# LitLeo/3m-asr-inference

Hardware: AMD Instinct MI355X
Metric: encoder frames/sec, 18Lx32e Conformer-MoE, 206-frame utterance (higher is better)
Workload: dtype f32; 1 GPU; 18-layer 32-expert fp32 (v_mfma_f32_16x16x4_f32), batch=1x206 frames per GPU, all experts local (BASELINE.json configs[1]); layers=18, experts=32, frames=206, batch_per_gpu=1, parallelism=replicas x1, streams_per_gpu=4, hip_graph=True, kernels_per_forward=262, fold_pos_proj=True, routing=balanced, route_mode=staged, packed_rows=False, fork_embed=auto

## Files before the change

### 3m-asr-inference_amd/csrc/conv.hip

```cpp
#include "common.h"
#include "kernels.h"

namespace m3 {

struct DwCausal {
  int causal = 0;
  const float* left = nullptr;
  long left_b_stride = 0; int left_t_stride = 0;
  const int32_t* step = nullptr;
  long half = 0;
  const int32_t* chunk_len = nullptr;
  int max_chunks = 0;
};

template <int KT, bool CAUSAL, bool SLOTS = false, bool GLU_IN = false>
__device__ __forceinline__ void dwconv_ln_silu_body(const float* __restrict__ z, const float* __restrict__ w_kc,
                                                    const float* __restrict__ bias, const float* __restrict__ gamma,
                                                    const float* __restrict__ beta, float eps, int T, int D, int K,
                                                    float* __restrict__ out, int out_bf16, const int32_t* __restrict__ pad_of,
                                                    const int32_t* __restrict__ row0, const int32_t* __restrict__ row_len,
                                                    int n_rows, const DwCausal& cs, const int row, const int ldz = 0) {
  static_assert(!GLU_IN || (!CAUSAL && !SLOTS), "GLU on load: the symmetric conv only");
  __shared__ float red[2][16];
  asm volatile("" ::"s"(z), "s"(w_kc), "s"(bias), "s"(gamma), "s"(beta), "s"(eps), "s"(T), "s"(D), "s"(K), "s"(out), "s"(out_bf16),
               "s"(pad_of), "s"(row0), "s"(row_len), "s"(n_rows));
  const int c = threadIdx.x * 4;
  const bool live = c < D;
  const size_t zs = GLU_IN ? (size_t)ldz : (size_t)D;
  const float* leftp = cs.left;
  if (CAUSAL && cs.step != nullptr) {
    int par;
    if (SLOTS) {
      const int sb = row >= n_rows ? (row - n_rows) / (K - 1) : row / T;
      const int pos = cs.step[sb];
      if (row >= n_rows && !stream_slot_live(cs.chunk_len[sb], pos, cs.max_chunks)) return;
      par = pos & 1;
    } else {
      par = *cs.step & 1;
    }
    leftp = cs.left + (size_t)par * cs.half;
    if (row >= n_rows) {
      const int i = row - n_rows, b = i / (K - 1), ci = i - b * (K - 1);
      const int s = ci + min(max(cs.chunk_len[b], 0), T);
      const float* src = s < K - 1 ? leftp + (size_t)b * cs.left_b_stride + (size_t)s * cs.left_t_stride
                                   : z + ((size_t)b * T + (s - (K - 1))) * D;
      float* dst = const_cast<float*>(cs.left) + (size_t)(par ^ 1) * cs.half + (size_t)b * cs.left_b_stride + (size_t)ci * cs.left_t_stride;
      if (live) stg4(dst + c, ldg4(src + c));
      return;
    }
  }
  int b = row / T, t = row % T, len = T;
  size_t r0 = (size_t)b * T, rpad = 0;
  if (pad_of != nullptr) {
    const int pr = pad_of[row];
    if (pr < 0) return;
    b = pr / T;
    t = pr - b * T;
    len = row_len[b];
    r0 = (size_t)row0[b];
    rpad = (size_t)row0[n_rows / T];
  }
  const int pad = CAUSAL ? K - 1 : (K - 1) / 2;
  if (CAUSAL) leftp += (size_t)b * cs.left_b_stride + (size_t)(K - 1) * cs.left_t_stride;
  const int lane = threadIdx.x & 63, wave = threadIdx.x >> 6, nwaves = (blockDim.x + 63) >> 6;
  f32x4 v = f32x4{0.f, 0.f, 0.f, 0.f};
  if (live) {
    v = ldg4(bias + c);
    for (int k0 = 0; k0 < K; k0 += KT) {
      f32x4 zz[KT], ww[KT], gg[GLU_IN ? KT : 1];
      float on[KT];
#pragma unroll
      for (int kk = 0; kk < KT; ++kk) {
        const int k = min(k0 + kk, K - 1);
        const int tt = t + k - pad;
        const int tc = min(max(tt, 0), T - 1);
        const float* src = z + (tc < len ? r0 + tc : rpad) * zs;
        if (CAUSAL) {
          on[kk] = (k0 + kk < K) ? 1.f : 0.f;
          if (tt < 0) src = leftp + (long)tt * cs.left_t_stride;
        } else {
          on[kk] = (k0 + kk < K && tt >= 0 && tt < T) ? 1.f : 0.f;
        }
        zz[kk] = ldg4(src + c);
        if (GLU_IN) gg[kk] = ldg4(src + D + c);
        ww[kk] = ldg4(w_kc + (size_t)k * D + c);
      }
      if (GLU_IN) {
        __builtin_amdgcn_sched_barrier(0);
#pragma unroll
        for (int kk = 0; kk < KT; ++kk)
#pragma unroll
          for (int j = 0; j < 4; ++j) zz[kk][j] = zz[kk][j] * sigmoidf(gg[kk][j]);
      }
#pragma unroll
      for (int kk = 0; kk < KT; ++kk)
#pragma unroll
        for (int j = 0; j < 4; ++j) v[j] = fmaf(zz[kk][j] * on[kk], ww[kk][j], v[j]);
    }
  }
  if (gamma != nullptr) {
    float s = live ? (v[0] + v[1]) + (v[2] + v[3]) : 0.f;
    s = wave_sum(s);
    if (lane == 0) red[0][wave] = s;
    __syncthreads();
    float tot = 0.f;
    for (int w = 0; w < nwaves; ++w) tot += red[0][w];
    const float mean = tot / (float)D;
    float q = 0.f;
    if (live) {
#pragma unroll
      for (int j = 0; j < 4; ++j) {
        const float d = v[j] - mean;
        q += d * d;
      }
    }
    q = wave_sum(q);
    if (lane == 0) red[1][wave] = q;
    __syncthreads();
    float qt = 0.f;
    for (int w = 0; w < nwaves; ++w) qt += red[1][w];
    const float rstd = rsqrtf(qt / (float)D + eps);
    if (live) {
      const f32x4 g = ldg4(gamma + c), be = ldg4(beta + c);
#pragma unroll
      for (int j = 0; j < 4; ++j) v[j] = (v[j] - mean) * rstd * g[j] + be[j];
    }
  }
  if (live) {
#pragma unroll
    for (int j = 0; j < 4; ++j) v[j] = silu(v[j]);
    if (out_bf16) {
      bf16x4 h;
#pragma unroll
      for (int j = 0; j < 4; ++j) h[j] = (bf16_t)v[j];
      *reinterpret_cast<bf16x4*>(reinterpret_cast<bf16_t*>(out) + (size_t)row * D + c) = h;
    } else {
      stg4(out + (size_t)row * D + c, v);
    }
  }
}

template <int KT, bool CAUSAL, bool SLOTS = false, bool GLU_IN = false>
__global__ __launch_bounds__(GLU_IN ? 256 : 1024) void dwconv_ln_silu_kernel(const float* __restrict__ z, const float* __restrict__ w_kc,
                                                              const float* __restrict__ bias,
                                                              const float* __restrict__ gamma,
                                                              const float* __restrict__ beta, float eps, int T,
                                                              int D, int K, float* __restrict__ out, int out_bf16,
                                                              const int32_t* __restrict__ pad_of,
                                                              const int32_t* __restrict__ row0,
                                                              const int32_t* __restrict__ row_len, int n_rows, DwCausal cs, int ldz) {
  dwconv_ln_silu_body<KT, CAUSAL, SLOTS, GLU_IN>(z, w_kc, bias, gamma, beta, eps, T, D, K, out, out_bf16, pad_of, row0, row_len, n_rows, cs,
                                                 (int)blockIdx.x, ldz);
}
struct DwKernArgs {
  const float *z, *w_kc, *bias, *gamma, *beta; float eps; int T, D, K; float* out; int out_bf16;
  const int32_t *pad_of, *row0, *row_len; int n_rows; DwCausal cs; int ldz;
};
template <int KT, bool CAUSAL, bool GLU_IN = false>
__global__ __launch_bounds__(GLU_IN ? 256 : 1024) void dwconv_ln_silu_dual_kernel(const DwKernArgs a, const DwKernArgs b) {
  if ((int)blockIdx.x < a.n_rows)
    dwconv_ln_silu_body<KT, CAUSAL, false, GLU_IN>(a.z, a.w_kc, a.bias, a.gamma, a.beta, a.eps, a.T, a.D, a.K, a.out, a.out_bf16, a.pad_of, a.row0,
                                                   a.row_len, a.n_rows, a.cs, (int)blockIdx.x, a.ldz);
  else
    dwconv_ln_silu_body<KT, CAUSAL, false, GLU_IN>(b.z, b.w_kc, b.bias, b.gamma, b.beta, b.eps, b.T, b.D, b.K, b.out, b.out_bf16, b.pad_of, b.row0,
                                                   b.row_len, b.n_rows, b.cs, (int)blockIdx.x - a.n_rows, b.ldz);
}

static int launch_dwconv_impl(const float* z, const float* w_kc, const float* bias, const float* gamma, const float* beta, float eps,
                              int B, int T, int D, int K, float* out, hipStream_t stream, int out_bf16, const int32_t* pad_of,
                              const int32_t* row0, const int32_t* row_len, const DwCausal& cs, bool slots = false, int glu_ldz = 0) {
  M3_REQUIRE(glu_ldz == 0 || dwconv_glu_in_supports(D, K, cs.causal != 0 || slots, out_bf16, glu_ldz),
             "dwconv (GLU on load): needs the symmetric fp32 conv, K <= 15, 256 <= channels <= 1024, ldz=%d a multiple of 4 and >= %d", glu_ldz, 2 * D);
  M3_REQUIRE(!slots || (cs.causal && cs.step != nullptr && cs.max_chunks > 0), "dwconv (slot mode): needs the streaming causal form");
  M3_REQUIRE((D & 3) == 0 && D <= 4096, "dwconv: channels=%d must be a multiple of 4 (<=4096)", D);
  M3_REQUIRE(cs.causal || (K & 1) == 1, "dwconv: kernel size %d must be odd (non-causal)", K);
  M3_REQUIRE(!cs.causal || (cs.left != nullptr && K >= 2), "dwconv (causal): the frames left of frame 0 must be supplied (left_fill / cache)");
  const int rows = B * T;
  if (rows == 0) return 0;
  const int threads = (int)align_up(D / 4, 64);
  const int grid = rows + (cs.step != nullptr ? B * (K - 1) : 0);
#define M3_DW_CASE(KT_, C_)                                                                                                  \
  hipLaunchKernelGGL((dwconv_ln_silu_kernel<KT_, C_>), dim3(grid), dim3(threads), 0, stream, z, w_kc, bias, gamma, beta, eps, T, \
                     D, K, out, out_bf16, pad_of, row0, row_len, rows, cs, 0)
#define M3_DW_SLOTS(KT_)                                                                                                        \
  hipLaunchKernelGGL((dwconv_ln_silu_kernel<KT_, true, true>), dim3(grid), dim3(threads), 0, stream, z, w_kc, bias, gamma, beta, eps, \
                     T, D, K, out, out_bf16, pad_of, row0, row_len, rows, cs, 0)
  if (glu_ldz)
    hipLaunchKernelGGL((dwconv_ln_silu_kernel<15, false, false, true>), dim3(grid), dim3(threads), 0, stream, z, w_kc, bias, gamma, beta, eps, T,
                       D, K, out, out_bf16, pad_of, row0, row_len, rows, cs, glu_ldz);
  else if (slots) { if (K <= 15) M3_DW_SLOTS(15); else M3_DW_SLOTS(8); }
  else if (K <= 15) { if (cs.causal) M3_DW_CASE(15, true); else M3_DW_CASE(15, false); }
  else { if (cs.causal) M3_DW_CASE(8, true); else M3_DW_CASE(8, false); }
#undef M3_DW_SLOTS
#undef M3_DW_CASE
  M3_LAUNCH_CHECK();
  return 0;
}

int launch_dwconv_ln_silu(const float* z, const float* w_kc, const float* bias, const float* gamma,
                          const float* beta, float eps, int B, int T, int D, int K, float* out, hipStream_t stream, int out_bf16,
                          const int32_t* pad_of, const int32_t* row0, const int32_t* row_len, const float* causal_left_fill) {
  DwCausal cs;
  if (causal_left_fill != nullptr) { cs.causal = 1; cs.left = causal_left_fill; }
  return launch_dwconv_impl(z, w_kc, bias, gamma, beta, eps, B, T, D, K, out, stream, out_bf16, pad_of, row0, row_len, cs);
}

bool dwconv_glu_in_supports(int D, int K, bool causal_or_stream, int out_bf16, int ldz) {
  return !causal_or_stream && !out_bf16 && (K & 1) == 1 && K <= 15 && D >= 256 && D <= 1024 && (D & 3) == 0 && ldz >= 2 * D && (ldz & 3) == 0;
}

int launch_dwconv_ln_silu_args(const DwArgs& a, hipStream_t stream) {
  if (a.glu_ldz) {
    M3_REQUIRE(a.causal_left_fill == nullptr, "dwconv (GLU on load): the symmetric conv only");
    return launch_dwconv_impl(a.z, a.w_kc, a.bias, a.gamma, a.beta, a.eps, a.B, a.T, a.D, a.K, a.out, stream, a.out_bf16, a.pad_of, a.row0, a.row_len,
                              DwCausal{}, false, a.glu_ldz);
  }
  return launch_dwconv_ln_silu(a.z, a.w_kc, a.bias, a.gamma, a.beta, a.eps, a.B, a.T, a.D, a.K, a.out, stream, a.out_bf16, a.pad_of, a.row0,
                               a.row_len, a.causal_left_fill);
}
bool dwconv_dual_fusable(const DwArgs& a, const DwArgs& b) {
  if ((a.glu_ldz != 0) != (b.glu_ldz != 0)) return false;
  if (a.glu_ldz && !(dwconv_glu_in_supports(a.D, a.K, a.causal_left_fill != nullptr, a.out_bf16, a.glu_ldz) &&
                     dwconv_glu_in_supports(b.D, b.K, b.causal_left_fill != nullptr, b.out_bf16, b.glu_ldz)))
    return false;
  return a.D == b.D && a.K == b.K && (a.causal_left_fill != nullptr) == (b.causal_left_fill != nullptr) && a.B * a.T > 0 && b.B * b.T > 0 &&
         (a.D & 3) == 0 && a.D <= 4096 && (a.causal_left_fill != nullptr || (a.K & 1) == 1);
}
int launch_dwconv_ln_silu_dual(const DwArgs& a, const DwArgs& b, hipStream_t stream) {
  M3_REQUIRE(dwconv_dual_fusable(a, b), "dwconv dual: the two problems do not share an instantiation");
  auto pack = [](const DwArgs& q) {
    DwKernArgs k;
    k.z = q.z; k.w_kc = q.w_kc; k.bias = q.bias; k.gamma = q.gamma; k.beta = q.beta; k.eps = q.eps; k.T = q.T; k.D = q.D; k.K = q.K;
    k.out = q.out; k.out_bf16 = q.out_bf16; k.pad_of = q.pad_of; k.row0 = q.row0; k.row_len = q.row_len; k.n_rows = q.B * q.T;
    if (q.causal_left_fill != nullptr) { k.cs.causal = 1; k.cs.left = q.causal_left_fill; }
    k.ldz = q.glu_ldz;
    return k;
  };
  const DwKernArgs ka = pack(a), kb = pack(b);
  const int threads = (int)align_up(a.D / 4, 64), grid = ka.n_rows + kb.n_rows;
  const bool causal = a.causal_left_fill != nullptr;
#define M3_DWD_CASE(KT_, C_) hipLaunchKernelGGL((dwconv_ln_silu_dual_kernel<KT_, C_>), dim3(grid), dim3(threads), 0, stream, ka, kb)
  if (a.glu_ldz) hipLaunchKernelGGL((dwconv_ln_silu_dual_kernel<15, false, true>), dim3(grid), dim3(threads), 0, stream, ka, kb);
  else if (a.K <= 15) { if (causal) M3_DWD_CASE(15, true); else M3_DWD_CASE(15, false); }
  else { if (causal) M3_DWD_CASE(8, true); else M3_DWD_CASE(8, false); }
#undef M3_DWD_CASE
  M3_LAUNCH_CHECK();
  return 0;
}

int launch_dwconv_ln_silu_stream(const float* z, const float* w_kc, const float* bias, const float* gamma, const float* beta,
                                 float eps, int B, int T, int D, int K, float* out, float* cache_pair, const int32_t* step,
                                 const int32_t* chunk_len, hipStream_t stream, int out_bf16, int slot_max_chunks) {
  M3_REQUIRE(cache_pair && step && chunk_len, "dwconv (stream): null state");
  DwCausal cs;
  cs.causal = 1; cs.left = cache_pair; cs.left_b_stride = (long)(K - 1) * D; cs.left_t_stride = D;
  cs.step = step; cs.half = (long)B * (K - 1) * D; cs.chunk_len = chunk_len;
  cs.max_chunks = slot_max_chunks > 0 ? slot_max_chunks : 0;
  return launch_dwconv_impl(z, w_kc, bias, gamma, beta, eps, B, T, D, K, out, stream, out_bf16, nullptr, nullptr, nullptr, cs,
                            slot_max_chunks >= 0);
}

__device__ __forceinline__ void conv1_relu_body(const float* __restrict__ feat, const float* __restrict__ w9c,
                                                const float* __restrict__ bias, const float* __restrict__ cmvn_mean,
                                                const float* __restrict__ cmvn_istd, int T, int idim, int T1, int F1, int C,
                                                float* __restrict__ out, int relu, int out_bf16, const int32_t* __restrict__ feat_len,
                                                int32_t* __restrict__ lens_out, int B, const int row) {
  extern __shared__ float xs[];
  if (feat_len != nullptr && row == 0 && blockIdx.y == 0)
    for (int i = threadIdx.x; i < B; i += blockDim.x) lens_out[i] = ((feat_len[i] - 3) / 2 + 1 - 3) / 2 + 1;
  const int b = row / T1, t1 = row - b * T1;
  const float* src = feat + ((size_t)b * T + 2 * t1) * idim;
  for (int i = threadIdx.x; i < 3 * idim; i += blockDim.x) {
    float xv = src[i];
    if (cmvn_mean != nullptr) {
      const int f = i % idim;
      xv = (xv - cmvn_mean[f]) * cmvn_istd[f];
    }
    xs[i] = xv;
  }
  const int c = threadIdx.x * 4;
  const bool live = c < C;
  f32x4 w[9], bv = f32x4{0.f, 0.f, 0.f, 0.f};
  if (live) {
    bv = ldg4(bias + c);
#pragma unroll
    for (int k = 0; k < 9; ++k) w[k] = ldg4(w9c + (size_t)k * C + c);
  }
  __syncthreads();
  if (!live) return;
  const size_t obase = (size_t)row * F1 * C + c;
  const int fchunk = (F1 + gridDim.y - 1) / gridDim.y;
  const int f_lo = blockIdx.y * fchunk, f_hi = min(F1, f_lo + fchunk);
  for (int f1 = f_lo; f1 < f_hi; ++f1) {
    f32x4 acc = bv;
#pragma unroll
    for (int kh = 0; kh < 3; ++kh)
#pragma unroll
      for (int kw = 0; kw < 3; ++kw) {
        const float xv = xs[kh * idim + 2 * f1 + kw];
#pragma unroll
        for (int j = 0; j < 4; ++j) acc[j] = fmaf(xv, w[kh * 3 + kw][j], acc[j]);
      }
#pragma unroll
    for (int j = 0; j < 4; ++j) acc[j] = relu ? fmaxf(acc[j], 0.f) : acc[j];
    if (out_bf16) {
      bf16x4 h;
#pragma unroll
      for (int j = 0; j < 4; ++j) h[j] = (bf16_t)acc[j];
      *reinterpret_cast<bf16x4*>(reinterpret_cast<bf16_t*>(out) + obase + (size_t)f1 * C) = h;
    } else {
      stg4(out + obase + (size_t)f1 * C, acc);
    }
  }
}

__global__ __launch_bounds__(256) void conv1_relu_kernel(const float* __restrict__ feat, const float* __restrict__ w9c,
                                                         const float* __restrict__ bias,
                                                         const float* __restrict__ cmvn_mean,
                                                         const float* __restrict__ cmvn_istd, int T, int idim, int T1,
                                                         int F1, int C, float* __restrict__ out, int relu, int out_bf16,
                                                         const int32_t* __restrict__ feat_len, int32_t* __restrict__ lens_out, int B) {
  conv1_relu_body(feat, w9c, bias, cmvn_mean, cmvn_istd, T, idim, T1, F1, C, out, relu, out_bf16, feat_len, lens_out, B, (int)blockIdx.x);
}
struct Conv1KernArgs {
  const float *feat, *w9c, *bias, *cmvn_mean, *cmvn_istd; int C; float* out; int relu, out_bf16; const int32_t* feat_len; int32_t* lens_out;
};
__global__ __launch_bounds__(256) void conv1_relu_dual_kernel(const Conv1KernArgs a, const Conv1KernArgs b, int T, int idim, int T1, int F1,
                                                              int B, int rows, int n0) {
  const int id = (int)blockIdx.x;
  if (id < n0) {
    if (id < rows)
      conv1_relu_body(a.feat, a.w9c, a.bias, a.cmvn_mean, a.cmvn_istd, T, idim, T1, F1, a.C, a.out, a.relu, a.out_bf16, a.feat_len, a.lens_out, B, id);
  } else {
    conv1_relu_body(b.feat, b.w9c, b.bias, b.cmvn_mean, b.cmvn_istd, T, idim, T1, F1, b.C, b.out, b.relu, b.out_bf16, b.feat_len, b.lens_out, B, id - n0);
  }
}

static int conv1_fsplit(int rows) { return rows >= 2048 ? 1 : (rows >= 512 ? 2 : 5); }

int launch_conv1_relu(const float* feat, const float* w9c, const float* bias, const float* cmvn_mean,
                      const float* cmvn_istd, int B, int T, int idim, int C, float* out, hipStream_t stream, int relu, int out_bf16,
                      const int32_t* feat_len, int32_t* lens_out) {
  M3_REQUIRE(T >= 3 && idim >= 3, "subsampling: input (T=%d, idim=%d) shorter than the 3x3 kernel", T, idim);
  M3_REQUIRE((C & 3) == 0 && C <= 1024, "subsampling: channels=%d must be a multiple of 4 (<= 1024)", C);
  const int T1 = (T - 3) / 2 + 1, F1 = (idim - 3) / 2 + 1;
  if (B * T1 == 0) return 0;
  const int threads = (int)align_up(C / 4, 64);
  const int fsplit = conv1_fsplit(B * T1);
  hipLaunchKernelGGL(conv1_relu_kernel, dim3(B * T1, fsplit), dim3(threads), 3 * idim * sizeof(float), stream,
                     feat, w9c, bias, cmvn_mean, cmvn_istd, T, idim, T1, F1, C, out, relu, out_bf16, feat_len, lens_out, B);
  M3_LAUNCH_CHECK();
  return 0;
}

int launch_conv1_relu_args(const Conv1Args& a, hipStream_t stream) {
  return launch_conv1_relu(a.feat, a.w9c, a.bias, a.cmvn_mean, a.cmvn_istd, a.B, a.T, a.idim, a.C, a.out, stream, a.relu, a.out_bf16, a.feat_len,
                           a.lens_out);
}
bool conv1_dual_fusable(const Conv1Args& a, const Conv1Args& b) {
  auto ok = [](const Conv1Args& q) { return q.T >= 3 && q.idim >= 3 && (q.C & 3) == 0 && q.C > 0 && q.C <= 1024; };
  return ok(a) && ok(b) && a.B == b.B && a.T == b.T && a.idim == b.idim && a.B * ((a.T - 3) / 2 + 1) > 0 && a.out != b.out;
}
int launch_conv1_relu_dual(const Conv1Args& a, const Conv1Args& b, hipStream_t stream) {
  M3_REQUIRE(conv1_dual_fusable(a, b), "subsampling conv1 dual: the two problems do not share an input shape");
  const int T1 = (a.T - 3) / 2 + 1, F1 = (a.idim - 3) / 2 + 1, rows = a.B * T1;
  auto pack = [](const Conv1Args& q) {
    return Conv1KernArgs{q.feat, q.w9c, q.bias, q.cmvn_mean, q.cmvn_istd, q.C, q.out, q.relu, q.out_bf16, q.feat_len, q.lens_out};
  };
  const int threads = (int)align_up((a.C > b.C ? a.C : b.C) / 4, 64);
  const int n0 = (int)align_up((size_t)rows, 8);
  hipLaunchKernelGGL(conv1_relu_dual_kernel, dim3(n0 + rows, conv1_fsplit(rows)), dim3(threads), 3 * a.idim * sizeof(float), stream, pack(a), pack(b),
                     a.T, a.idim, T1, F1, a.B, rows, n0);
  M3_LAUNCH_CHECK();
  return 0;
}

__global__ void depthwise_conv1d_nct_kernel(const float* __restrict__ x, const float* __restrict__ w,
                                            const float* __restrict__ bias, int C, int T, int To, int K, int pad,
                                            float* __restrict__ y, size_t n) {
  for (size_t i = (size_t)blockIdx.x * blockDim.x + threadIdx.x; i < n; i += (size_t)gridDim.x * blockDim.x) {
    const int t = (int)(i % To);
    const size_t bc = i / To;
    const int c = (int)(bc % C);
    const float* xr = x + bc * T;
    float acc = bias ? bias[c] : 0.f;
    for (int k = 0; k < K; ++k) {
      const int tt = t + k - pad;
      if (tt >= 0 && tt < T) acc = fmaf(xr[tt], w[(size_t)c * K + k], acc);
    }
    y[i] = acc;
  }
}

int launch_depthwise_conv1d_nct(const float* x, const float* w, const float* bias, int B, int C, int T, int K,
                                int pad, float* y, hipStream_t stream) {
// ... 31 lines not shown
```

### 3m-asr-inference_amd/csrc/engine.hip

```cpp
#include <assert.h>
#include <math.h>
#include <stdlib.h>
#include <string.h>

#include <functional>
#include <memory>
#include <string>
#include <unordered_map>
#include <vector>

#include "../../include/m3asr.h"
#include "common.h"
#include "kernels.h"

namespace m3 {
struct MoeWorkspace {
  int32_t* mapping; int32_t* acc; int32_t* pos; float* slab; size_t bytes;
};
MoeWorkspace carve_moe_workspace(void* base, int S, int E, int D, int F);
}

using namespace m3;

namespace {

struct Norm { const float* g = nullptr; const float* b = nullptr; };
struct Lin { const float* w = nullptr; const float* b = nullptr; const float* wsum = nullptr; const float* wbeta = nullptr; };

struct BlockW {
  Norm n_ffm, n_mha, n_conv, n_ff, n_final, n_cnn;
  Lin mac1, mac2, qkv, pos, out, pw1, pw2, ff1, ff2;
  const float* pos_u = nullptr; const float* pos_v = nullptr;
  const float* dw_w = nullptr; const float* dw_b = nullptr;
  const float* left_fill = nullptr;
  Lin router;
  Lin router_x;
  const float *ew1 = nullptr, *eb1 = nullptr, *ew2 = nullptr, *eb2 = nullptr;
  const float *es1 = nullptr, *es2 = nullptr;
  float h_scale = 0.f;
};

struct SubW { const float* c1w; const float* c1b; const float* c2w; const float* c2b; Lin out; };

enum class FuseKind { None, Gemm, Dwconv, Attention, Conv1, SplitK };

struct Stage {
  std::string name;
  std::function<int(hipStream_t)> run;
  m3_stage_info info;
  bool reads_embed = false;
  FuseKind fuse_kind = FuseKind::None;
  GemmParams gemm; GemmPlan gemm_plan; float* gemm_ws = nullptr;
  Conv1Args c1;
  DwArgs dw;
  AttArgs att;
};

m3_stage_info stage_info(const char* kernel, int launches, double bytes, double flops, bool per_row = true) {
  m3_stage_info i;
  i.kernel = kernel; i.launches = launches; i.per_row = per_row ? 1 : 0; i.alg_bytes = bytes; i.flops = flops;
  return i;
}

struct Buf { void* ptr; size_t bytes; };

struct BindKey {
  int B = 0, T = 0;
  const float* feat = nullptr; const int32_t* feat_len = nullptr; float* logits = nullptr;
  void* ws = nullptr; size_t ws_bytes = 0;
  int ep_cap = 0;
  void* sstate = nullptr; int s_hist = 0, s_maxf = 0;
  bool s_slots = false;
  bool operator==(const BindKey& o) const {
    return B == o.B && T == o.T && feat == o.feat && feat_len == o.feat_len && logits == o.logits && ws == o.ws &&
           ws_bytes == o.ws_bytes && ep_cap == o.ep_cap && sstate == o.sstate && s_hist == o.s_hist && s_maxf == o.s_maxf &&
           s_slots == o.s_slots;
  }
};

}

struct m3_engine {
  m3_engine_config cfg;
  std::unordered_map<std::string, m3_weight_entry> table;
  std::vector<std::string> names;
  SubW sub_e, sub_m;
  std::vector<BlockW> eblocks, mblocks;
  Norm e_after, m_after;
  Lin out_linear;
  const float* pe = nullptr;
  int64_t pe_rows = 0;
  const float* pos_all = nullptr;
  const float* cmvn_mean = nullptr; const float* cmvn_istd = nullptr;
  const float* output_bias = nullptr;
  const float* router_e_all = nullptr;

  struct Bound {
    BindKey key;
    int Tp = 0, S = 0;
    bool a16 = false;
    bool dma = false;
    bool packed = false;
    bool xn_skipped = false;
    int fork_first = -1, fork_mid = -1, join_at = -1;
    std::shared_ptr<float> pfold;
    std::vector<Stage> stages;
    std::unordered_map<std::string, Buf> buffers;
    int n_kernels = 0;
    hipGraphExec_t graph_exec = nullptr;
    bool graph_valid = false;
    uint64_t last_use = 0;
    bool matches(const BindKey& k) const { return !stages.empty() && key == k; }
  };
  Bound cur;
  std::vector<Bound> parked;
  uint64_t use_clock = 0;
  int n_captures = 0;
  int ep_capacity = 0;
  hipStream_t side = nullptr;
  hipEvent_t ev_fork = nullptr, ev_join = nullptr;
  std::unordered_map<int, std::weak_ptr<float>> pfold_by_tp;
};

namespace {

struct Switches {
  int gate_index_max_rows;
  bool self_route;
  bool hfuse;
  int router_min_rows;
  bool router_xq;
  bool router_skip_xn;
  bool fused8_adapt;
  bool glu_defer;
  bool front_pair;
};
const Switches& switches() {
  static const Switches sw = [] {
    auto num = [](const char* name, int dflt) { const char* v = getenv(name); return v ? atoi(v) : dflt; };
    Switches w;
    w.gate_index_max_rows = num("M3_GATE_INDEX_MAX_ROWS", 512);
    w.self_route = num("M3_SELF_ROUTE", 1) != 0;
    w.hfuse = num("M3_HFUSE", 1) != 0;
    w.router_min_rows = num("M3_ROUTER_MIN_ROWS", 2048);
    w.router_xq = num("M3_ROUTER_XQ", 1) != 0;
    w.router_skip_xn = num("M3_ROUTER_SKIP_XN", 0) != 0;
    w.fused8_adapt = num("M3_FUSED8_ADAPT", 0) != 0;
    w.glu_defer = num("M3_GLU_DEFER", 1) != 0;
    w.front_pair = num("M3_FRONT_PAIR", 1) != 0;
    return w;
  }();
  return sw;
}

bool lookup(const m3_engine* e, const std::string& name, int64_t numel, const float** out, int dtype = M3_F32) {
  auto it = e->table.find(name);
  if (it == e->table.end()) {
    set_error("engine: weight '%s' missing from the plan", name.c_str());
    return false;
  }
  if (numel >= 0 && it->second.numel != numel) {
    set_error("engine: weight '%s' has %lld elements, expected %lld", name.c_str(), (long long)it->second.numel,
              (long long)numel);
    return false;
  }
  if (it->second.dtype != dtype) {
    set_error("engine: weight '%s' has dtype %d, the engine (weight_dtype=%d) expects %d", name.c_str(),
              (int)it->second.dtype, (int)e->cfg.weight_dtype, dtype);
    return false;
  }
  *out = (const float*)it->second.data;
  return true;
}

#define GET(dst, name, numel) \
  do { if (!lookup(e, (name), (numel), &(dst))) return false; } while (0)
#define GETW(dst, name, numel) \
  do { if (!lookup(e, (name), (numel), &(dst), e->cfg.weight_dtype == M3_F32 ? M3_F32 : M3_BF16)) return false; } while (0)
#define GETE(dst, name, numel) \
  do { if (!lookup(e, (name), (numel), &(dst), e->cfg.weight_dtype)) return false; } while (0)

bool load_norm(const m3_engine* e, const std::string& p, int d, Norm* n) {
  GET(n->g, p + "weight", d);
  GET(n->b, p + "bias", d);
  return true;
}
bool load_lin(const m3_engine* e, const std::string& p, int64_t n_out, int64_t n_in, bool bias, Lin* l) {
  GETW(l->w, p + "weight", n_out * n_in);
  if (bias) GET(l->b, p + "bias", n_out);
  return true;
}
bool load_lin_ln(const m3_engine* e, const std::string& p, int64_t n_out, int64_t n_in, bool wbeta, Lin* l,
                 bool fp32_only = false) {
  if (fp32_only) {
    GET(l->w, p + "ln.weight", n_out * n_in);
  } else {
    GETW(l->w, p + "ln.weight", n_out * n_in);
  }
  GET(l->b, p + "ln.bias", n_out);
  GET(l->wsum, p + "ln.wsum", n_out);
  if (wbeta) GET(l->wbeta, p + "ln.wbeta", n_out);
  return true;
}

bool load_block(const m3_engine* e, const std::string& p, int D, int F, int K, bool cnn_ln, bool moe, int De, BlockW* b, bool causal) {
  const m3_engine_config& c = e->cfg;
  if (!load_norm(e, p + "norm_final.", D, &b->n_final)) return false;
  if (moe && !load_norm(e, p + "norm_ff.", D, &b->n_ff)) return false;
  if (!load_lin_ln(e, p + "feed_forward_macaron.w_1.", F, D, false, &b->mac1) ||
      !load_lin(e, p + "feed_forward_macaron.w_2.", D, F, true, &b->mac2) ||
      !load_lin_ln(e, p + "self_attn.qkv.", 3 * D, D, false, &b->qkv) ||
      !load_lin(e, p + "self_attn.linear_out.", D, D, true, &b->out) ||
      !load_lin_ln(e, p + "conv_module.pointwise_conv1.", 2 * D, D, true, &b->pw1) ||
      !load_lin(e, p + "conv_module.pointwise_conv2.", D, D, true, &b->pw2))
    return false;
  GET(b->pos_u, p + "self_attn.pos_bias_u", D);
  GET(b->pos_v, p + "self_attn.pos_bias_v", D);
  GET(b->dw_w, p + "conv_module.depthwise_conv.weight_kc", (int64_t)K * D);
  GET(b->dw_b, p + "conv_module.depthwise_conv.bias", D);
  if (cnn_ln && !load_norm(e, p + "conv_module.norm.", D, &b->n_cnn)) return false;
  if (causal) GET(b->left_fill, p + "conv_module.left_fill", D);
  if (!moe) {
    if (!load_lin_ln(e, p + "feed_forward.w_1.", F, D, false, &b->ff1) ||
        !load_lin(e, p + "feed_forward.w_2.", D, F, true, &b->ff2))
      return false;
  } else {
    const int world = c.ep_world_size > 0 ? c.ep_world_size : 1;
    const int64_t Etot = (int64_t)c.num_experts * world;
    GET(b->router.w, p + "feed_forward.router_weights_t", Etot * (D + De));
    if (c.router_with_bias) GET(b->router.b, p + "feed_forward.router_bias", Etot);
    if (c.fuse_route && !load_lin_ln(e, p + "feed_forward.router_x.", Etot, D, false, &b->router_x, true)) return false;
    const int64_t E = c.num_experts;
    GETE(b->ew1, p + "feed_forward.experts.w_1.weight", E * F * D);
    if (c.weight_dtype == M3_FP8) {
      GET(b->es1, p + "feed_forward.experts.w_1.scale", E * F);
      GET(b->es2, p + "feed_forward.experts.w_2.scale", E * D);
      if (c.fp8_activations) {
        const float* hs = nullptr;
        GET(hs, p + "feed_forward.experts.h_scale", 1);
        if (hipMemcpy(&b->h_scale, hs, sizeof(float), hipMemcpyDeviceToHost) != hipSuccess || !(b->h_scale > 0.f)) {
          set_error("engine: '%sfeed_forward.experts.h_scale' must hold one positive number", p.c_str());
          return false;
        }
      }
    }
    GET(b->eb1, p + "feed_forward.experts.w_1.bias", E * F);
    GETE(b->ew2, p + "feed_forward.experts.w_2.weight_sliced", E * D * F);
    GET(b->eb2, p + "feed_forward.experts.w_2.bias", E * D);
  }
  return true;
}

bool load_sub(const m3_engine* e, const std::string& p, int D, int idim, SubW* s) {
  const int F2 = ((idim - 1) / 2 - 1) / 2;
  GET(s->c1w, p + "conv.0.weight_9c", 9 * (int64_t)D);
  GET(s->c1b, p + "conv.0.bias", D);
  GETW(s->c2w, p + "conv.2.weight_ohwi", 9 * (int64_t)D * D);
  GET(s->c2b, p + "conv.2.bias", D);
  return load_lin(e, p + "out.0.", D, (int64_t)D * F2, true, &s->out);
}
#undef GET
#undef GETW
#undef GETE

inline int sub_len(int t) { return ((t - 3) / 2 + 1 - 3) / 2 + 1; }

struct Carver {
  char* base; size_t off = 0;
  explicit Carver(void* b) : base((char*)b) {}
  template <typename T> T* take(size_t n) {
    T* p = (T*)(base ? base + off : nullptr);
    off += align_up(n * sizeof(T), 256);
    return p;
  }
};

struct Plan {
  int32_t* lens;
  float *c1, *c2, *x, *emb, *h1, *qkv, *pbuf, *ctx, *glu, *dw, *xn, *rl, *eall;
  void* xb;
  int32_t* moe_fs;
  unsigned char* xq; float* xq_scale;
  float* xstats;
  int32_t* gate_idx; float* gate_val;
  void* moe_ws; size_t moe_ws_bytes;
  float* splitk; size_t splitk_bytes;
  float* taps;
  float* pfold;
  int32_t *row0, *pad_of; float* xpad; void* xbpad; float* lpk;
  int32_t *ep_acc, *ep_mapping, *ep_pos, *ep_map_send, *ep_gate_recv, *ep_overflow; float *wire_a, *wire_b; int ep_cap, ep_rows;
  bool fork;
  bool hfuse;
  float *e_c1, *e_c2, *e_x, *e_h1, *e_qkv, *e_ctx, *e_glu, *e_dw, *e_xpad, *e_splitk, *e_xstats; void *e_xb, *e_xbpad;
  size_t bytes;
};

bool use_fork_embed(const m3_engine_config& c, int B, int S) { return c.fork_embed > 0 && !c.debug_taps; }
bool use_packed_rows(const m3_engine_config& c, int B) {
  if (c.packed_rows < 0 || (c.packed_rows == 0 && B <= 1)) return false;
  return !c.debug_taps && c.fuse_route == 0 && B <= 1024;
}

bool use_hfuse(const m3_engine_config& c, int B, int S) {
  return switches().hfuse && !c.debug_taps && c.weight_dtype == M3_F32 && c.embed_blocks > 0 && c.num_blocks > 0 && S <= 128 && c.fork_embed <= 0 &&
         !use_packed_rows(c, B);
}

Plan make_plan(const m3_engine_config& c, void* base, int B, int T, int ep_capacity = 0) {
  Plan p;
  Carver cv(base);
  const int Tp = sub_len(T), S = B * Tp;
  const int T1 = (T - 3) / 2 + 1, F1 = (c.input_dim - 3) / 2 + 1, F2 = (F1 - 3) / 2 + 1;
  const int D = c.attention_dim > c.embed_dim ? c.attention_dim : c.embed_dim;
  const int F = c.hidden_units > c.embed_linear_units ? c.hidden_units : c.embed_linear_units;
  const int world = c.ep_world_size > 0 ? c.ep_world_size : 1;
  const int Etot = c.num_experts * world;
  p.lens = cv.take<int32_t>(B);
  p.c1 = cv.take<float>((size_t)B * T1 * F1 * D);
  p.c2 = cv.take<float>((size_t)S * F2 * D);
  p.x = cv.take<float>((size_t)S * D);
  p.emb = cv.take<float>((size_t)S * D);
  p.xb = cv.take<uint16_t>((size_t)S * D);
  p.xstats = cv.take<float>((size_t)S * 2 * kXbStatParts);
  p.h1 = cv.take<float>((size_t)S * F);
  p.qkv = cv.take<float>((size_t)S * 3 * D);
  p.pbuf = cv.take<float>((size_t)Tp * D * (c.num_blocks + c.embed_blocks));
  p.ctx = cv.take<float>((size_t)S * D);
  const size_t glu_floats = (size_t)S * D * (switches().glu_defer && c.weight_dtype == M3_F32 && D >= 256 ? 2 : 1);
  p.glu = cv.take<float>(glu_floats);
  p.dw = cv.take<float>((size_t)S * D);
  p.xn = cv.take<float>((size_t)S * D);
  p.xq = nullptr; p.xq_scale = nullptr; p.moe_fs = nullptr;
  if (c.weight_dtype == M3_FP8) p.moe_fs = cv.take<int32_t>(64);
  if (c.weight_dtype == M3_FP8 && D == 512) {
    p.xq = cv.take<unsigned char>((size_t)S * D);
    p.xq_scale = cv.take<float>((size_t)S);
  }
  p.rl = cv.take<float>((size_t)S * Etot);
  p.eall = cv.take<float>((size_t)S * Etot * c.num_blocks);
  p.gate_idx = cv.take<int32_t>((size_t)c.num_blocks * S);
  p.gate_val = cv.take<float>((size_t)c.num_blocks * S);
  const bool ep = world > 1 || c.ep_stages > 0;
  p.ep_cap = ep ? (ep_capacity > 0 ? ep_capacity : S) : 0;
  p.ep_rows = ep ? world * (p.ep_cap + 1) : 0;
  p.moe_ws_bytes = carve_moe_workspace(nullptr, ep ? p.ep_rows : S, c.num_experts, c.attention_dim, c.hidden_units).bytes;
  p.moe_ws = cv.take<char>(p.moe_ws_bytes * (size_t)(c.debug_taps ? c.num_blocks : 1));
  p.ep_acc = p.ep_mapping = p.ep_pos = p.ep_map_send = p.ep_gate_recv = p.ep_overflow = nullptr; p.wire_a = p.wire_b = nullptr;
  if (ep) {
    p.ep_overflow = cv.take<int32_t>(64);
    p.ep_acc = cv.take<int32_t>((size_t)Etot + 1);
    p.ep_mapping = cv.take<int32_t>(S);
    p.ep_pos = cv.take<int32_t>(S);
    p.ep_map_send = cv.take<int32_t>(S);
    p.ep_gate_recv = cv.take<int32_t>(p.ep_rows);
    p.wire_a = cv.take<float>((size_t)p.ep_rows * c.attention_dim);
    p.wire_b = cv.take<float>((size_t)p.ep_rows * c.attention_dim);
  }
  {
    size_t n1 = 0, n2 = 0;
    if (c.weight_dtype == M3_F32) {
      GemmParams g;
      g.mode = GEMM_A_CONV3X3S2; g.lda = 4; g.conv_C = D; g.M = S * F2; g.N = D; g.K = 9 * D; g.ldy = D;
      n1 = plan_gemm(g, SIZE_MAX).ws_bytes;
      GemmParams l;
      l.lda = F2 * D; l.M = S; l.N = D; l.K = F2 * D; l.ldy = D;
      n2 = plan_gemm(l, SIZE_MAX).ws_bytes;
    }
    p.splitk_bytes = n1 > n2 ? n1 : n2;
    p.splitk = p.splitk_bytes ? cv.take<float>(p.splitk_bytes / sizeof(float)) : nullptr;
  }
  p.taps = c.debug_taps ? cv.take<float>((size_t)(c.num_blocks + c.embed_blocks) * S * D) : nullptr;
  p.pfold = nullptr;
  p.row0 = p.pad_of = nullptr; p.xpad = p.lpk = nullptr; p.xbpad = nullptr;
  if (use_packed_rows(c, B)) {
    p.row0 = cv.take<int32_t>(B + 1);
    p.pad_of = cv.take<int32_t>(S);
    p.xpad = cv.take<float>((size_t)S * D);
    p.xbpad = cv.take<uint16_t>((size_t)S * D);
    p.lpk = cv.take<float>((size_t)S * c.output_dim);
  }
  p.fork = use_fork_embed(c, B, S);
  p.hfuse = !p.fork && use_hfuse(c, B, S);
  p.e_c1 = p.c1; p.e_c2 = p.c2; p.e_x = p.x; p.e_h1 = p.h1; p.e_qkv = p.qkv; p.e_ctx = p.ctx; p.e_glu = p.glu; p.e_dw = p.dw;
  p.e_xb = p.xb; p.e_xpad = p.xpad; p.e_xbpad = p.xbpad; p.e_splitk = p.splitk; p.e_xstats = p.xstats;
  if (p.fork || p.hfuse) {
    p.e_c1 = cv.take<float>((size_t)B * T1 * F1 * D);
    p.e_c2 = cv.take<float>((size_t)S * F2 * D);
    p.e_x = cv.take<float>((size_t)S * D);
    p.e_xb = cv.take<uint16_t>((size_t)S * D);
    p.e_xstats = cv.take<float>((size_t)S * 2 * kXbStatParts);
    p.e_h1 = cv.take<float>((size_t)S * F);
    p.e_qkv = cv.take<float>((size_t)S * 3 * D);
    p.e_ctx = cv.take<float>((size_t)S * D);
    p.e_glu = cv.take<float>(glu_floats);
    p.e_dw = cv.take<float>((size_t)S * D);
    if (p.splitk_bytes) p.e_splitk = cv.take<float>(p.splitk_bytes / sizeof(float));
    if (use_packed_rows(c, B)) {
      p.e_xpad = cv.take<float>((size_t)S * D);
      p.e_xbpad = cv.take<uint16_t>((size_t)S * D);
    }
  }
  p.bytes = cv.off;
  return p;
}

struct StreamState {
  int32_t* step = nullptr;
  std::vector<float*> kv, conv;
  int32_t *slot_pos = nullptr, *slot_status = nullptr, *slot_frames = nullptr;
  size_t bytes = 0;
};
StreamState carve_stream_state(const m3_engine_config& c, void* base, int B, int hist) {
  Carver cv(base);
  StreamState st;
  st.step = cv.take<int32_t>(64);
  const int nb = c.embed_blocks + c.num_blocks, D = c.attention_dim, K = c.cnn_module_kernel;
  for (int i = 0; i < nb; ++i) st.kv.push_back(cv.take<float>((size_t)B * hist * 2 * D));
  for (int i = 0; i < nb; ++i) st.conv.push_back(cv.take<float>((size_t)2 * B * (K - 1) * D));
  st.slot_pos = cv.take<int32_t>((size_t)3 * B);
  st.slot_status = st.slot_pos ? st.slot_pos + B : nullptr;
  st.slot_frames = st.slot_pos ? st.slot_pos + 2 * B : nullptr;
  st.bytes = cv.off;
  return st;
}

Plan embed_view(const Plan& pl) {
  Plan q = pl;
  q.c1 = pl.e_c1; q.c2 = pl.e_c2; q.x = pl.e_x; q.h1 = pl.e_h1; q.qkv = pl.e_qkv; q.ctx = pl.e_ctx; q.glu = pl.e_glu; q.dw = pl.e_dw;
  q.xb = pl.e_xb; q.xpad = pl.e_xpad; q.xbpad = pl.e_xbpad; q.splitk = pl.e_splitk; q.xstats = pl.e_xstats;
  return q;
}

enum class RouterForm {
  Gemm,
  Kernel,
  Fused,
  Split,
};
enum class GateForm {
  RouterTail,
  GateIndex,
  Top1Index,
  InExpert,
  InRoute,
};
struct MoeRoute {
  RouterForm router = RouterForm::Gemm;
  GateForm gate = GateForm::Top1Index;
  bool ep = false;
  bool router_top1 = false;
  bool use_xq = false;
  bool skip_xn = false;
  bool fs_dev = false;
  bool needs_e_all = false;
  bool norm_in_expert() const { return router == RouterForm::Fused || router == RouterForm::Split; }
};

static ExpertWeights expert_weights(const m3_engine_config& c, const BlockW& w) {
  if (c.weight_dtype == M3_F32) return ExpertWeights::F32;
  if (c.weight_dtype == M3_BF16) return ExpertWeights::BF16;
  return w.h_scale > 0.f ? ExpertWeights::FP8A8 : ExpertWeights::FP8;
}

MoeRoute choose_moe_route(const m3_engine_config& c, int S, const BlockW& w, const Plan& pl) {
  const Switches& sw = switches();
  const int world = c.ep_world_size > 0 ? c.ep_world_size : 1;
  const int E = c.num_experts, Etot = E * world, D = c.attention_dim, De = c.embed_dim, F = c.hidden_units;
  const bool one_wg_experts = Etot == 8 || Etot == 16 || Etot == 32 || Etot == 64;
  const bool self_routing = sw.self_route && c.weight_dtype == M3_F32 && expert_ffn_f32_self_routing(S, Etot) &&
                            plan_expert_ffn(ExpertWeights::F32, S, E, D, F).kernel == ExpertKernel::SlabF32;
  MoeRoute r;
  r.ep = world > 1 || c.ep_stages > 0;
  if (c.fuse_route == 2 && world == 1 && S < 1024 && one_wg_experts) {
    r.router = RouterForm::Split;
    r.gate = self_routing ? GateForm::InExpert : GateForm::GateIndex;
  } else if (c.fuse_route == 1 && world == 1 && S <= 256 && (E == 16 || E == 32 || E == 64)) {
    r.router = RouterForm::Fused;
    r.gate = GateForm::InRoute;
  } else {
    r.router = moe_router_supports(De, D, Etot) && S >= sw.router_min_rows ? RouterForm::Kernel : RouterForm::Gemm;
    r.router_top1 = r.router == RouterForm::Kernel && moe_router_fuses_top1(Etot) && S > sw.gate_index_max_rows;
    if (self_routing && c.fuse_route == 0 && !r.ep) r.gate = GateForm::InExpert;
    else if (S <= sw.gate_index_max_rows && one_wg_experts) r.gate = GateForm::GateIndex;
    else r.gate = r.router_top1 ? GateForm::RouterTail : GateForm::Top1Index;
  }
  const bool fused8 = !r.ep && plan_expert_ffn(expert_weights(c, w), S, E, D, F).kernel == ExpertKernel::FusedFp8;
  r.use_xq = r.router == RouterForm::Kernel && sw.router_xq && fused8 && pl.xq != nullptr;
  r.skip_xn = r.use_xq && sw.router_skip_xn && !c.debug_taps;
  r.fs_dev = sw.fused8_adapt && fused8 && pl.moe_fs != nullptr && !c.debug_taps;
  r.needs_e_all = r.norm_in_expert();
  return r;
}

struct StageBuilder {
  const m3_engine& eng;
  Plan pl;
  m3_engine::Bound& bd;
  StreamState st;
  bool lens_in_conv1 = false;
  const float *tail_ln_g = nullptr, *tail_ln_b = nullptr; float tail_ln_eps = 0.f; float* tail_ln_out = nullptr;
  float* splitk_ws = nullptr; size_t splitk_bytes = 0;
};

}

static void add_stage(StageBuilder& sb, const std::string& name, int kernels, std::function<int(hipStream_t)> fn,
                      m3_stage_info info = stage_info("", 0, 0.0, 0.0)) {
  info.launches = kernels;
  sb.bd.stages.push_back(Stage{name, std::move(fn), info});
  sb.bd.n_kernels += kernels;
}

static m3_stage_info gemm_info(const GemmParams& p, const GemmPlan& plan) {
  const bool glu = p.act == ACT_GLU;
  const double M = p.M, N = p.N, K = p.K, Nout = glu ? N / 2 : N;
  const double wsz = p.w_bf16 ? 2 : 4, asz = p.a_bf16 ? 2 : 4, ysz = p.y_bf16 ? 2 : 4;
  double a_bytes = M * K * asz;
  if (p.mode == GEMM_A_CONV3X3S2)
    a_bytes = (double)(p.M / (p.conv_T2 * p.conv_F2)) * p.conv_T1 * p.conv_F1 * p.conv_C * asz;
  double bytes = N * K * wsz + a_bytes + M * Nout * ysz;
  if (p.resid) bytes += M * Nout * 4;
  if (p.Yb) bytes += M * Nout * 2;
  if (p.ln_out) bytes += M * (K - p.K1) * 4;
  return stage_info(plan.label, 1, bytes, 2.0 * M * N * K, p.mode != GEMM_A_CONV3X3S2);
}

static void add_gemm(StageBuilder& sb, const std::string& name, GemmParams p, bool fp32_weights = false) {
  p.w_bf16 = (!fp32_weights && sb.eng.cfg.weight_dtype != M3_F32) ? 1 : 0;
  float* ws = sb.splitk_ws;
  const GemmPlan plan = plan_gemm(p, ws != nullptr ? sb.splitk_bytes : 0);
  add_stage(sb, name, plan.launches ? plan.launches : 1, [plan, p, ws](hipStream_t s) { return launch_gemm(plan, p, ws, s); }, gemm_info(p, plan));
  if (plan.launches == 1) {
    sb.bd.stages.back().fuse_kind = FuseKind::Gemm;
    sb.bd.stages.back().gemm = p;
    sb.bd.stages.back().gemm_plan = plan;
  } else if (plan.kernel == GemmKernel::SplitKF32 && plan.launches == 2) {
    sb.bd.stages.back().gemm = p;
    sb.bd.stages.back().gemm_plan = plan;
    sb.bd.stages.back().gemm_ws = ws;
  }
}

static bool stages_fusable(const Stage& a, const Stage& b) {
  if (a.fuse_kind == FuseKind::None || a.fuse_kind != b.fuse_kind) return false;
  if (a.fuse_kind == FuseKind::Gemm) return gemm_dual_fusable(a.gemm_plan, b.gemm_plan);
  if (a.fuse_kind == FuseKind::Dwconv) return dwconv_dual_fusable(a.dw, b.dw);
  if (a.fuse_kind == FuseKind::Attention) return relpos_attention_dual_fusable(a.att, b.att);
  if (a.fuse_kind == FuseKind::Conv1) return conv1_dual_fusable(a.c1, b.c1);
  if (a.fuse_kind == FuseKind::SplitK) return gemm_splitk_dual_fusable(a.gemm_plan, b.gemm_plan) && a.gemm_ws != b.gemm_ws;
  return false;
}
static Stage fused_stage(const Stage& a, const Stage& b, bool reduce_half = false) {
  Stage d;
  d.name = reduce_half ? a.name + ".reduce+" + b.name + ".reduce" : a.name + "+" + b.name;
  const char* label = "";
  if (a.fuse_kind == FuseKind::Conv1) {
    const Conv1Args pa = a.c1, pb = b.c1;
    d.run = [pa, pb](hipStream_t s) { return launch_conv1_relu_dual(pa, pb, s); };
    label = "conv1_relu_dual_kernel";
  } else if (a.fuse_kind == FuseKind::SplitK) {
    const GemmParams pa = a.gemm, pb = b.gemm;
    const GemmPlan qa = a.gemm_plan, qb = b.gemm_plan;
    float* const wa = a.gemm_ws; float* const wb = b.gemm_ws;
    const int which = reduce_half ? 2 : 1;
    d.run = [qa, pa, wa, qb, pb, wb, which](hipStream_t s) { return launch_gemm_f32_splitk_dual(qa, pa, wa, qb, pb, wb, s, which); };
    label = "gemm_f32_splitk_dual_kernel";
  } else if (a.fuse_kind == FuseKind::Gemm) {
    const GemmParams pa = a.gemm, pb = b.gemm;
    const GemmPlan qa = a.gemm_plan, qb = b.gemm_plan;
    d.run = [qa, pa, qb, pb](hipStream_t s) { return launch_gemm_f32_dual(qa, pa, qb, pb, s); };
    label = "gemm_f32_dual_kernel";
  } else if (a.fuse_kind == FuseKind::Dwconv) {
    const DwArgs pa = a.dw, pb = b.dw;
    d.run = [pa, pb](hipStream_t s) { return launch_dwconv_ln_silu_dual(pa, pb, s); };
    label = "dwconv_ln_silu_dual_kernel";
  } else {
    const AttArgs pa = a.att, pb = b.att;
    d.run = [pa, pb](hipStream_t s) { return launch_relpos_attention_dual(pa, pb, s); };
    label = "relpos_attention_dual_kernel";
  }
  d.info = reduce_half ? stage_info(label, 1, 0.0, 0.0, a.info.per_row != 0)
                       : stage_info(label, 1, a.info.alg_bytes + b.info.alg_bytes, a.info.flops + b.info.flops, a.info.per_row != 0);
  return d;
}
static void fuse_independent_pairs(StageBuilder& sb, int first, int mid, int join) {
  if (first < 0 || mid <= first + 1 || join <= mid) return;
  std::vector<Stage>& st = sb.bd.stages;
  std::vector<Stage> out(st.begin(), st.begin() + first);
  std::vector<Stage> pending;
  int i = first, saved = 0;
  for (int m = mid; m < join; ++m) {
    assert(!st[m].reads_embed);
    int partner = -1;
    if (st[m].fuse_kind != FuseKind::None)
      for (int k = st[m].fuse_kind == FuseKind::Conv1 ? i : std::max(i, first + 1); k < mid; ++k)
        if (stages_fusable(st[k], st[m])) { partner = k; break; }
    if (partner < 0) { pending.push_back(st[m]); continue; }
    for (; i < partner; ++i) out.push_back(st[i]);
    for (Stage& q : pending) out.push_back(q);
    pending.clear();
    out.push_back(fused_stage(st[partner], st[m]));
    saved += st[partner].info.launches + st[m].info.launches - 1;
    if (st[m].fuse_kind == FuseKind::SplitK) {
      out.push_back(fused_stage(st[partner], st[m], true));
      saved -= 1;
    }
    i = partner + 1;
  }
  for (; i < mid; ++i) out.push_back(st[i]);
  for (Stage& q : pending) out.push_back(q);
  for (int k = join; k < (int)st.size(); ++k) out.push_back(st[k]);
  st.swap(out);
  sb.bd.n_kernels -= saved;
}

static int embed_join(const std::vector<Stage>& st, int from) {
  for (int i = from; i < (int)st.size(); ++i)
    if (st[i].reads_embed) return i;
  return -1;
}

static void build_subsample(StageBuilder& sb, const std::string& pfx, const SubW& w, int D, const Plan& pl, float* xout) {
  const m3_engine_config& c = sb.eng.cfg;
  const int B = sb.bd.key.B, T = sb.bd.key.T;
  const int T1 = (T - 3) / 2 + 1, F1 = (c.input_dim - 3) / 2 + 1, F2 = (F1 - 3) / 2 + 1, T2 = (T1 - 3) / 2 + 1;
  const float* feat = sb.bd.key.feat;
  float* c1 = pl.c1; float* c2 = pl.c2;
  const int idim = c.input_dim;
  const float* cm = sb.eng.cmvn_mean; const float* ci = sb.eng.cmvn_istd;
  const bool a16 = sb.bd.a16;
  const int32_t* flen = sb.lens_in_conv1 ? sb.bd.key.feat_len : nullptr;
  int32_t* lens_out = pl.lens;
  sb.lens_in_conv1 = false;
  Conv1Args ca;
  ca.feat = feat; ca.w9c = w.c1w; ca.bias = w.c1b; ca.cmvn_mean = cm; ca.cmvn_istd = ci; ca.B = B; ca.T = T; ca.idim = idim; ca.C = D; ca.out = c1;
  ca.relu = 1; ca.out_bf16 = a16; ca.feat_len = flen; ca.lens_out = lens_out;
  add_stage(sb, pfx + "conv1", 1, [ca](hipStream_t s) { return launch_conv1_relu_args(ca, s); },
            stage_info("conv1_relu_kernel", 1, (double)B * T * idim * 4 + (double)B * T1 * F1 * D * (a16 ? 2 : 4), 18.0 * B * T1 * F1 * D, false));
  const size_t conv1_at = sb.bd.stages.size() - 1;
  GemmParams g;
  g.a_bf16 = a16; g.y_bf16 = a16;
  g.mode = GEMM_A_CONV3X3S2; g.A = c1; g.lda = 4;
  g.conv_T1 = T1; g.conv_F1 = F1; g.conv_T2 = T2; g.conv_F2 = F2; g.conv_C = D;
  g.W = w.c2w; g.bias = w.c2b; g.Y = c2; g.ldy = D; g.M = B * T2 * F2; g.N = D; g.K = 9 * D; g.act = ACT_RELU;
  if (sb.bd.packed) g.conv_len = pl.lens;
  add_gemm(sb, pfx + "conv2", g);
  const bool pairable = switches().front_pair && !a16 && !sb.bd.packed && sb.bd.stages.back().gemm_plan.kernel == GemmKernel::SplitKF32 &&
                        sb.bd.stages.back().gemm_ws != nullptr;
  if (pairable) {
    sb.bd.stages[conv1_at].fuse_kind = FuseKind::Conv1;
    sb.bd.stages[conv1_at].c1 = ca;
    sb.bd.stages.back().fuse_kind = FuseKind::SplitK;
  }
  const bool packed = sb.bd.packed;
  GemmParams l;
  l.A = c2; l.lda = F2 * D; l.W = w.out.w; l.bias = w.out.b; l.Y = packed ? pl.xpad : xout; l.ldy = D;
  l.M = B * T2; l.N = D; l.K = F2 * D; l.alpha = sqrtf((float)D);
  l.a_bf16 = a16;
  if (a16) { l.Yb = packed ? pl.xbpad : pl.xb; l.ldyb = D; }
  add_gemm(sb, pfx + "linear", l);
  if (pairable && sb.bd.stages.back().gemm_ws != nullptr) sb.bd.stages.back().fuse_kind = FuseKind::SplitK;
  if (packed) {
    const float* xpad = pl.xpad; const void* xbpad = pl.xbpad; void* xb = pl.xb; const int32_t* pad_of = pl.pad_of;
    const int S = B * T2;
    add_stage(sb, pfx + "pack", a16 ? 2 : 1, [=](hipStream_t s) {
      if (int rc = launch_local_gather(xpad, pad_of, S, D * 4, xout, s)) return rc;
      return a16 ? launch_local_gather(xbpad, pad_of, S, D * 2, xb, s) : 0;
    }, stage_info("row_permute_kernel", 1, (double)S * D * (a16 ? 12 : 8) + 4.0 * S, 0.0));
  }
  if (sb.bd.dma) {
    const void* xbv = pl.xb; float* xs = pl.xstats;
    const int S = B * T2;
    add_stage(sb, pfx + "row_stats", 1, [=](hipStream_t s) { return launch_row_stats_bf16(xbv, S, D, xs, s); },
              stage_info("row_stats_bf16_kernel", 1, (double)S * D * 2 + 32.0 * S, 3.0 * S * D));
  }
}

struct MoeLayer {
  std::string pfx;
  const BlockW* w;
  int S, Tp, D, F, De, E, Etot, world;
  float eps;
  float *x, *xn, *rl;
  int32_t* gidx; float* gval;
  const float* gv;
  const int32_t *lens, *live_len; int live_rpb;
  const int32_t* pdev;
  const float* eall; int ld_eall;
  void* xb_out; float* xstats_out;
  void* ws; MoeWorkspace mw;
};

static void add_moe_router(StageBuilder& sb, const MoeLayer& m, const MoeRoute& r, const Plan& pl) {
  const BlockW& w = *m.w;
  const int S = m.S, D = m.D, De = m.De, E = m.E, Etot = m.Etot;
  if (r.router == RouterForm::Fused) {
    add_stage(sb, m.pfx + "moe_route", 1, [m](hipStream_t s) {
      const BlockW& w = *m.w;
      return launch_moe_route(m.x, m.D, m.D, w.router_x.w, w.router_x.wsum, w.router_x.b, m.eall, m.ld_eall, m.eps, m.lens, m.Tp,
                              m.S, m.E, m.gidx, m.gval, m.mw.mapping, m.mw.acc, m.mw.pos, s);
    }, stage_info("moe_route_kernel", 1, (double)E * D * 4 + (double)S * (D + E) * 4 + 16.0 * S, 2.0 * S * E * D));
  } else if (r.router == RouterForm::Kernel) {
    void* xq = r.use_xq ? pl.xq : nullptr; float* xqs = r.use_xq ? pl.xq_scale : nullptr;
    float* xn_out = r.skip_xn ? nullptr : m.xn;
    if (r.skip_xn) sb.bd.xn_skipped = true;
    int32_t* gidx = r.router_top1 ? m.gidx : nullptr; float* gval = r.router_top1 ? m.gval : nullptr;
    const float* emb = pl.emb;
    add_stage(sb, m.pfx + "moe_router", 1, [=](hipStream_t s) {
      const BlockW& w = *m.w;
      return launch_moe_router(emb, m.De, m.De, m.x, m.D, m.D, w.router.w, w.router.b, w.n_ff.g, w.n_ff.b, m.eps, xn_out, m.D, m.rl,
                               m.Etot, m.S, m.Etot, m.pdev, s, gidx, gval, m.live_len, m.live_rpb, xq, xqs);
    }, stage_info("moe_router_kernel", 1, (double)Etot * (De + D) * 4 + (double)S * (De + 2 * D + Etot) * 4, 2.0 * S * Etot * (De + D)));
  } else {
    GemmParams g;
    g.Y = m.rl; g.ldy = Etot; g.M = S; g.N = Etot; g.m_dev = m.pdev;
    if (r.router == RouterForm::Split) {
      g.A = m.x; g.lda = D; g.W = w.router_x.w; g.bias = w.router_x.b; g.ln_wsum = w.router_x.wsum; g.ln_eps = m.eps; g.K = D;
      g.resid = m.eall; g.ldr = m.ld_eall;
    } else {
      g.mode = GEMM_A_CONCAT2; g.A = pl.emb; g.lda = De; g.K1 = De; g.A2 = m.x; g.lda2 = D; g.K = De + D;
      g.W = w.router.w; g.bias = w.router.b;
      g.ln_gamma = w.n_ff.g; g.ln_beta = w.n_ff.b; g.ln_eps = m.eps; g.ln_on_a2 = 1; g.ln_out = m.xn; g.ld_ln_out = D;
    }
    add_gemm(sb, m.pfx + "moe_router", g, true);
  }
  sb.bd.stages.back().reads_embed = true;
}

static void add_moe_gate_index(StageBuilder& sb, const MoeLayer& m, int32_t* map, int32_t* acc, int32_t* pos) {
  add_stage(sb, m.pfx + "moe_gate_index", 1, [=](hipStream_t s) {
    return launch_moe_gate_index(m.rl, m.Etot, m.live_len, m.live_rpb, m.S, m.gidx, m.gval, map, acc, pos, s);
  }, stage_info("moe_index_kernel", 1, (double)m.S * (m.Etot * 4 + 16) + 4.0 * (m.Etot + 1), 0.0));
}

static void add_moe_top1(StageBuilder& sb, const MoeLayer& m) {
  add_stage(sb, m.pfx + "moe_top1", 1, [m](hipStream_t s) {
    return launch_softmax_top1(m.rl, m.Etot, m.live_len, m.live_rpb, m.S, m.Etot, m.gidx, m.gval, s);
  }, stage_info("softmax_top1_kernel", 1, (double)m.S * (m.Etot * 4 + 8), 0.0));
}

static void add_moe_local_index(StageBuilder& sb, const MoeLayer& m) {
  add_stage(sb, m.pfx + "moe_local.index", 1, [m](hipStream_t s) {
    return launch_moe_index(m.gidx, m.S, m.E, m.mw.mapping, m.mw.acc, m.mw.pos, s);
  }, stage_info("moe_index_kernel", 1, 12.0 * m.S + 4.0 * (m.E + 1), 0.0));
}

static ExpertFfnArgs expert_args(const BlockW& w, const float* x, const MoeWorkspace& mw, int D) {
  ExpertFfnArgs a{};
  a.x = x; a.ldx = D; a.pos = mw.pos; a.acc_hist = mw.acc; a.w1 = w.ew1; a.w2 = w.ew2; a.s1 = w.es1; a.s2 = w.es2; a.b1 = w.eb1;
  a.w2_sliced = 1; a.h_scale = w.h_scale; a.slab = mw.slab;
  return a;
}

static void add_moe_local_expert(StageBuilder& sb, const MoeLayer& m, const MoeRoute& r, const ExpertFfnPlan& f, const Plan& pl) {
  const bool norm = r.norm_in_expert();
  const float* xin = norm ? m.x : m.xn;
  const bool self_route = r.gate == GateForm::InExpert;
  const void* xq = r.use_xq ? pl.xq : nullptr; const float* xqs = r.use_xq ? pl.xq_scale : nullptr;
  int32_t* fs = r.fs_dev ? pl.moe_fs : nullptr;
  add_stage(sb, m.pfx + "moe_local.expert", f.launches, [=](hipStream_t s) {
    const BlockW& w = *m.w;
    const float* ln_g = norm ? w.n_ff.g : nullptr; const float* ln_b = norm ? w.n_ff.b : nullptr; const float ln_eps = norm ? m.eps : 0.f;
    if (self_route)
      return launch_expert_route_ffn_f32(xin, m.D, m.rl, m.live_len, m.live_rpb, m.S, m.E, m.D, m.F, w.ew1, w.eb1, w.ew2, 1, w.eb2,
                                         m.mw.slab, m.gidx, m.gval, m.mw.mapping, m.mw.acc, m.mw.pos, s, ln_g, ln_b, ln_eps);
    ExpertFfnArgs a = expert_args(w, xin, m.mw, m.D);
    a.ln_gamma = ln_g; a.ln_beta = ln_b; a.ln_eps = ln_eps; a.xq = xq; a.xq_scale = xqs; a.fs_dev = fs;
    return launch_expert_ffn(f, m.S, m.E, m.D, m.F, a, s);
  }, stage_info(f.label, 1, -1.0, 4.0 * m.D * m.F * m.S));
}

static void add_moe_local_combine(StageBuilder& sb, const MoeLayer& m, const MoeRoute& r, const ExpertFfnPlan& f, const Plan& pl) {
  const bool self_route = r.gate == GateForm::InExpert;
  const int32_t* cmap = self_route ? nullptr : m.mw.mapping;
  const float* cb2 = self_route ? nullptr : m.w->eb2;
  const int32_t* fs = r.fs_dev ? pl.moe_fs : nullptr;
  const double S = m.S, D = m.D;
  add_stage(sb, m.pfx + "moe_local.combine", 1, [=](hipStream_t s) {
    const BlockW& w = *m.w;
    return launch_moe_combine(f.rows(m.mw.slab), fs ? kExpertFusedFp8MaxSplit : f.slices, cmap, m.gidx, m.gv, cb2, m.x, 0.5f, w.n_final.g, w.n_final.b, m.eps, m.x,
                              m.S, m.D, s, m.xb_out, m.xstats_out, fs);
  }, stage_info("moe_combine_kernel", 1, S * D * 4 * (f.slices + 2) + (m.xb_out ? 2.0 * S * D : 0.0), S * D * (f.slices + 10)));
}

static void add_moe_ep(StageBuilder& sb, const MoeLayer& m, const MoeRoute& r, const Plan& pl) {
  const int S = m.S, E = m.E, Etot = m.Etot, D = m.D, F = m.F, world = m.world;
  const int cap = pl.ep_cap, R = pl.ep_rows;
  int32_t *g_acc = pl.ep_acc, *g_map = pl.ep_mapping, *g_pos = pl.ep_pos, *map_send = pl.ep_map_send, *gate_recv = pl.ep_gate_recv;
  int32_t* ep_overflow = pl.ep_overflow;
  float *wire_a = pl.wire_a, *wire_b = pl.wire_b;
  const MoeWorkspace rw = carve_moe_workspace(m.ws, R, E, D, F);
  if (r.gate == GateForm::GateIndex) add_moe_gate_index(sb, m, g_map, g_acc, g_pos);
  if (r.gate == GateForm::Top1Index) add_moe_top1(sb, m);
  const bool one_launch = r.gate == GateForm::GateIndex;
  const int32_t* gidx = m.gidx; const float* xn = m.xn;
  add_stage(sb, m.pfx + "moe_ep.send", one_launch ? 1 : 2, [=](hipStream_t s) {
    if (!one_launch)
      if (int rc = launch_moe_index(gidx, S, Etot, g_map, g_acc, g_pos, s)) return rc;
    return launch_ep_send_rows(gidx, g_map, g_acc, S, world, E, cap, map_send, xn, wire_a, D * 4, s, ep_overflow);
  }, stage_info("ep_send_rows_kernel", 1, (double)S * D * 8 + 24.0 * S, 0.0));
  auto exchange = [=, &sb](const char* name) {
    if (world == 1) add_stage(sb, m.pfx + name, 0, [=](hipStream_t s) {
      M3_CHECK_HIP(hipMemcpyAsync(wire_b, wire_a, (size_t)R * D * 4, hipMemcpyDeviceToDevice, s));
      return 0;
    });
  };
  exchange("moe_ep.exchange1");
  const ExpertFfnPlan f = plan_expert_ffn(expert_weights(sb.eng.cfg, *m.w), R, E, D, F, EXPERT_SCATTER_ROWS);
  const bool scatter2 = f.kernel == ExpertKernel::TiledBf16;
  const BlockW* wp = m.w;
  add_stage(sb, m.pfx + "moe_ep.expert", (scatter2 ? 2 : 3) + f.launches, [=](hipStream_t s) {
    const BlockW& w = *wp;
    if (int rc = launch_ep_recv_gate(wire_b, world, E, cap, D * 4, gate_recv, s)) return rc;
    if (int rc = launch_moe_index(gate_recv, R, E, rw.mapping, rw.acc, rw.pos, s)) return rc;
    ExpertFfnArgs a = expert_args(w, wire_b, rw, D);
    if (scatter2) { a.b2 = w.eb2; a.y_scatter = wire_a; }
    if (int rc = launch_expert_ffn(f, R, E, D, F, a, s)) return rc;
    if (scatter2) return 0;
    return launch_moe_combine(f.rows(rw.slab), f.slices, rw.mapping, gate_recv, nullptr, w.eb2, nullptr, 1.f, nullptr, nullptr, 0.f, wire_a, R, D, s);
  }, stage_info(f.label, 1, -1.0, 4.0 * D * F * S));
  exchange("moe_ep.exchange2");
  add_stage(sb, m.pfx + "moe_ep.combine", 1, [=](hipStream_t s) {
    const BlockW& w = *wp;
    return launch_moe_combine(wire_b, 1, map_send, nullptr, m.gv, nullptr, m.x, 0.5f, w.n_final.g, w.n_final.b, m.eps, m.x, S, D, s,
                              m.xb_out, m.xstats_out);
  }, stage_info("moe_combine_kernel", 1, (double)S * D * 12 + (m.xb_out ? 2.0 * S * D : 0.0), (double)S * D * 11));
  sb.bd.buffers["ep.wire_a"] = Buf{wire_a, (size_t)R * D * 4};
  sb.bd.buffers["ep.wire_b"] = Buf{wire_b, (size_t)R * D * 4};
}

static void build_block(StageBuilder& sb, const std::string& pfx, const BlockW& w, int D, int F, int H, int K, bool cnn_ln,
                        bool moe, int layer, int tap_index, const Plan& pl, bool causal) {
  auto add_gemm = [&](StageBuilder&, const std::string& name, GemmParams g, bool fp32_weights = false) {
    if (sb.bd.packed) g.m_dev = pl.row0 + sb.bd.key.B;
    ::add_gemm(sb, name, g, fp32_weights);
  };
  const m3_engine_config& c = sb.eng.cfg;
  const BindKey& key = sb.bd.key;
  const int B = key.B, Tp = sb.bd.Tp, S = sb.bd.S;
  const bool streaming = key.sstate != nullptr;
  const int32_t* step = key.s_slots ? sb.st.slot_pos : sb.st.step;
  const int slot_chunks = key.s_slots ? key.s_maxf / Tp : -1;
  float* x = pl.x;
  const int32_t* lens = pl.lens;
  const float eps = 1e-12f;

  const bool a16 = sb.bd.a16;
  void* xb = pl.xb;
  const bool dma = sb.bd.dma;
  float* xstats = pl.xstats;
  auto from_xb = [&](GemmParams& g) {
    if (a16) { g.A = (const float*)xb; g.a_bf16 = 1; }
    if (dma) { g.ln_stats = xstats; g.ln_stat_parts = kXbStatParts; }
  };
  auto also_xb = [&](GemmParams& g) {
    if (a16) { g.Yb = xb; g.ldyb = D; }
    if (dma) g.Yb_stats = xstats;
  };
  const bool packed = sb.bd.packed;
  const int32_t* row0 = packed ? pl.row0 : nullptr;
  const int32_t* pad_of = packed ? pl.pad_of : nullptr;
  const int32_t* pdev = packed ? pl.row0 + B : nullptr;
  const int32_t* live_len = packed ? pdev : lens;
  const int live_rpb = packed ? S : Tp;
  {
    GemmParams g;
    g.A = x; g.lda = D; g.W = w.mac1.w; g.bias = w.mac1.b; g.Y = pl.h1; g.ldy = F; g.M = S; g.N = F; g.K = D;
    g.ln_wsum = w.mac1.wsum; g.ln_eps = eps; g.act = ACT_SILU;
    from_xb(g); g.y_bf16 = a16;
    add_gemm(sb, pfx + "ffn_macaron.w1", g);
    GemmParams h;
    h.A = pl.h1; h.lda = F; h.W = w.mac2.w; h.bias = w.mac2.b; h.Y = x; h.ldy = D; h.M = S; h.N = D; h.K = F;
    h.alpha = 0.5f; h.resid = x; h.ldr = D;
    h.a_bf16 = a16; also_xb(h);
    add_gemm(sb, pfx + "ffn_macaron.w2", h);
  }
  {
    GemmParams g;
    g.A = x; g.lda = D; g.W = w.qkv.w; g.bias = w.qkv.b; g.Y = pl.qkv; g.ldy = 3 * D; g.M = S; g.N = 3 * D; g.K = D;
    g.ln_wsum = w.qkv.wsum; g.ln_eps = eps;
    from_xb(g);
    const bool att16 = a16 && relpos_attention_bf16_supports(Tp, D / H);
    g.y_bf16 = att16;
    add_gemm(sb, pfx + "att.qkv", g);
    const int ldp = (c.num_blocks + c.embed_blocks) * D;
    const float* pmat = pl.pbuf + (size_t)tap_index * D;
    const float* qkv = pl.qkv; float* ctx = pl.ctx;
    const float* pu = w.pos_u; const float* pv = w.pos_v;
    const int dk = D / H;
    const float scale = 1.f / sqrtf((float)dk);
    const int chunk = c.static_chunk_size, left_chunks = c.num_left_chunks;
    if (streaming) {
      float* hist = sb.st.kv[tap_index]; const int cap = key.s_hist;
      add_stage(sb, pfx + "att.core", 1, [=](hipStream_t s) {
        return launch_relpos_attention_stream(qkv, 3 * D, hist, cap, pmat, ldp, pu, pv, lens, step, B, Tp, H, dk, scale, ctx, D, left_chunks, s,
                                              slot_chunks);
      }, stage_info("relpos_attention_stream_kernel", 1, (double)S * D * 24 + (double)Tp * D * 4, 6.0 * Tp * D * S));
    } else
    {
    add_stage(sb, pfx + "att.core", 1, [=](hipStream_t s) {
      if (att16) return launch_relpos_attention_bf16(qkv, 3 * D, pmat, ldp, pu, pv, lens, B, Tp, H, dk, scale, ctx, D, s, row0, chunk, left_chunks);
      return launch_relpos_attention(qkv, 3 * D, pmat, ldp, pu, pv, lens, B, Tp, H, dk, scale, ctx, D, s, a16, row0, chunk, left_chunks);
    }, stage_info(att16 ? "relpos_attention_bf16_kernel" : "relpos_attention_kernel", 1,
                  (double)S * D * (att16 ? 8 : (12 + (a16 ? 2 : 4))) + (double)Tp * D * 4, 6.0 * Tp * D * S));
    if (!att16) {
      AttArgs aa;
      aa.qkv = qkv; aa.ldq = 3 * D; aa.pmat = pmat; aa.ldp = ldp; aa.pos_u = pu; aa.pos_v = pv; aa.row_len = lens; aa.B = B; aa.T = Tp; aa.H = H;
      aa.dk = dk; aa.scale = scale; aa.out = ctx; aa.ldo = D; aa.out_bf16 = a16; aa.row0 = row0; aa.chunk = chunk; aa.left_chunks = left_chunks;
      sb.bd.stages.back().fuse_kind = FuseKind::Attention;
      sb.bd.stages.back().att = aa;
    }
    }
    GemmParams o;
    o.A = pl.ctx; o.lda = D; o.W = w.out.w; o.bias = w.out.b; o.Y = x; o.ldy = D; o.M = S; o.N = D; o.K = D;
    o.resid = x; o.ldr = D;
    o.a_bf16 = a16; also_xb(o);
    add_gemm(sb, pfx + "att.out", o);
  }
  {
    GemmParams g;
    g.A = x; g.lda = D; g.W = w.pw1.w; g.bias = w.pw1.b; g.Y = pl.glu; g.ldy = D; g.M = S; g.N = 2 * D; g.K = D;
    g.ln_wsum = w.pw1.wsum; g.ln_wbeta = w.pw1.wbeta; g.ln_eps = eps; g.act = ACT_GLU;
    g.row_len = live_len; g.rows_per_batch = live_rpb; g.mask_in = 1;
    from_xb(g);
    bool glu_deferred = false;
    if (switches().glu_defer && c.weight_dtype == M3_F32 && !a16 && !causal && !streaming &&
        dwconv_glu_in_supports(D, K, false, 0, 2 * D)) {
      GemmParams r = g;
      r.act = ACT_NONE; r.ldy = 2 * D;
      const GemmPlan rp = plan_gemm(r, 0);
      if (rp.launches == 1 && rp.kernel == GemmKernel::SkinnyF32 && rp.mt == 1) { g = r; glu_deferred = true; }
    }
    add_gemm(sb, pfx + "conv.pw1_glu", g);
    const float* glu = pl.glu; float* dw = pl.dw;
    const float* dww = w.dw_w; const float* dwb = w.dw_b;
    const float* ng = cnn_ln ? w.n_cnn.g : nullptr; const float* nb = cnn_ln ? w.n_cnn.b : nullptr;
    const float* lfill = causal ? w.left_fill : nullptr;
    if (streaming) {
      float* cpair = sb.st.conv[tap_index];
      add_stage(sb, pfx + "conv.dw_ln_silu", 1, [=](hipStream_t s) {
        return launch_dwconv_ln_silu_stream(glu, dww, dwb, ng, nb, 1e-5f, B, Tp, D, K, dw, cpair, step, lens, s, a16, slot_chunks);
      }, stage_info("dwconv_ln_silu_kernel", 1, (double)S * D * 8 + (double)K * D * 4 + 8.0 * B * (K - 1) * D, 2.0 * K * D * S));
    } else
    {
      DwArgs da;
      da.z = glu; da.w_kc = dww; da.bias = dwb; da.gamma = ng; da.beta = nb; da.eps = 1e-5f; da.B = B; da.T = Tp; da.D = D; da.K = K;
      da.out = dw; da.out_bf16 = a16; da.pad_of = pad_of; da.row0 = row0; da.row_len = lens; da.causal_left_fill = lfill;
      da.glu_ldz = glu_deferred ? 2 * D : 0;
      add_stage(sb, pfx + "conv.dw_ln_silu", 1, [da](hipStream_t s) { return launch_dwconv_ln_silu_args(da, s); },
                stage_info("dwconv_ln_silu_kernel", 1, (double)S * D * ((glu_deferred ? 8 : 4) + (a16 ? 2 : 4)) + (double)K * D * 4, 2.0 * K * D * S));
      sb.bd.stages.back().fuse_kind = FuseKind::Dwconv;
      sb.bd.stages.back().dw = da;
    }
    GemmParams h;
    h.A = pl.dw; h.lda = D; h.W = w.pw2.w; h.bias = w.pw2.b; h.Y = x; h.ldy = D; h.M = S; h.N = D; h.K = D;
    h.row_len = live_len; h.rows_per_batch = live_rpb; h.mask_out = 1; h.resid = x; h.ldr = D;
    h.a_bf16 = a16; also_xb(h);
    add_gemm(sb, pfx + "conv.pw2", h);
  }
  if (!moe) {
    GemmParams g;
    g.A = x; g.lda = D; g.W = w.ff1.w; g.bias = w.ff1.b; g.Y = pl.h1; g.ldy = F; g.M = S; g.N = F; g.K = D;
    g.ln_wsum = w.ff1.wsum; g.ln_eps = eps; g.act = ACT_SILU;
    from_xb(g); g.y_bf16 = a16;
    add_gemm(sb, pfx + "ffn.w1", g);
    GemmParams h;
    h.A = pl.h1; h.lda = F; h.W = w.ff2.w; h.bias = w.ff2.b; h.Y = x; h.ldy = D; h.M = S; h.N = D; h.K = F;
    h.alpha = 0.5f; h.resid = x; h.ldr = D;
    h.a_bf16 = a16;
    add_gemm(sb, pfx + "ffn.w2", h);
    const float* fg = w.n_final.g; const float* fb = w.n_final.b;
    void* xbo = a16 ? xb : nullptr;
    float* xso = dma ? xstats : nullptr;
    const float* g2 = sb.tail_ln_g; const float* b2 = sb.tail_ln_b; float* y2 = sb.tail_ln_out;
    const float eps2 = sb.tail_ln_eps;
    sb.tail_ln_g = nullptr;
    add_stage(sb, pfx + "norm_final", 1, [=](hipStream_t s) { return launch_layernorm(x, fg, fb, eps, x, S, D, s, xbo, xso, g2, b2, eps2, y2); },
              stage_info("layernorm_kernel", 1, (double)S * D * (a16 ? 10 : 8) + (g2 ? 4.0 * S * D : 0.0), (g2 ? 16.0 : 8.0) * S * D));
  } else {
    MoeLayer m;
    m.pfx = pfx; m.w = &w; m.S = S; m.Tp = Tp; m.D = D; m.F = F; m.De = c.embed_dim; m.E = c.num_experts;
    m.world = c.ep_world_size > 0 ? c.ep_world_size : 1; m.Etot = m.E * m.world; m.eps = eps;
    m.x = x; m.xn = pl.xn; m.rl = pl.rl;
    m.gidx = pl.gate_idx + (size_t)layer * S; m.gval = pl.gate_val + (size_t)layer * S;
    m.gv = c.keep_expert_output ? nullptr : m.gval;
    m.lens = lens; m.live_len = live_len; m.live_rpb = live_rpb; m.pdev = pdev;
    m.eall = pl.eall + (size_t)layer * m.E; m.ld_eall = c.num_blocks * m.E;
    m.xb_out = a16 ? xb : nullptr; m.xstats_out = dma ? xstats : nullptr;
    m.ws = (char*)pl.moe_ws + (c.debug_taps ? (size_t)layer * pl.moe_ws_bytes : 0);
    m.mw = carve_moe_workspace(m.ws, S, m.E, D, F);
    const MoeRoute r = choose_moe_route(c, S, w, pl);
    add_moe_router(sb, m, r, pl);
    if (r.ep) {
      add_moe_ep(sb, m, r, pl);
    } else {
      if (r.gate == GateForm::GateIndex) add_moe_gate_index(sb, m, m.mw.mapping, m.mw.acc, m.mw.pos);
      if (r.gate == GateForm::Top1Index) add_moe_top1(sb, m);
      if (r.gate == GateForm::Top1Index || r.gate == GateForm::RouterTail) add_moe_local_index(sb, m);
      const ExpertFfnPlan f = plan_expert_ffn(expert_weights(c, w), S, m.E, D, F, r.norm_in_expert() ? EXPERT_NORM_IN_KERNEL : 0);
      add_moe_local_expert(sb, m, r, f, pl);
      add_moe_local_combine(sb, m, r, f, pl);
    }
    const std::string b = pfx.substr(0, pfx.size() - 1);
    sb.bd.buffers[b + ".gate_idx"] = Buf{m.gidx, (size_t)S * 4};
    sb.bd.buffers[b + ".gate_value"] = Buf{m.gval, (size_t)S * 4};
    sb.bd.buffers[b + ".mapping"] = Buf{m.mw.mapping, (size_t)S * 4};
    sb.bd.buffers[b + ".acc_histogram"] = Buf{m.mw.acc, (size_t)(m.E + 1) * 4};
  }
  if (c.debug_taps) {
    float* tap = pl.taps + (size_t)tap_index * S * D;
    add_stage(sb, pfx + "tap", 0, [=](hipStream_t s) {
      M3_CHECK_HIP(hipMemcpyAsync(tap, x, (size_t)S * D * sizeof(float), hipMemcpyDeviceToDevice, s));
      return 0;
    });
    sb.bd.buffers[pfx.substr(0, pfx.size() - 1) + ".out"] = Buf{tap, (size_t)S * D * 4};
  }
}

extern "C" {

int m3_engine_output_frames(int T) { return T >= 7 ? sub_len(T) : 0; }

m3_engine* m3_engine_create(const m3_engine_config* config, const m3_weight_entry* table, int n_entries) {
  if (!config || !table || n_entries <= 0) {
    set_error("engine_create: null config / weight table");
    return nullptr;
  }
  m3_engine* e = new m3_engine;
  e->cfg = *config;
  const m3_engine_config& c = e->cfg;
  auto fail = [&](const char* msg) -> m3_engine* {
    if (msg) set_error("%s", msg);
    delete e;
    return nullptr;
  };
  if (c.attention_dim % c.attention_heads || c.embed_dim % c.embed_heads) return fail("engine_create: dim % heads != 0");
  if (c.attention_dim % 16 || c.embed_dim % 16 || c.hidden_units % 64 || c.embed_linear_units % 16)
    return fail("engine_create: dims must be multiples of 16 (hidden_units of 64)");
  if (c.embed_dim != c.attention_dim) return fail("engine_create: embed_dim != attention_dim is not supported");
  if (c.weight_dtype != M3_F32 && c.weight_dtype != M3_BF16 && c.weight_dtype != M3_FP8)
    return fail("engine_create: weight_dtype must be f32, bf16 or fp8");
  if (c.weight_dtype == M3_FP8 && (c.attention_dim % 64 || c.hidden_units % 64))
    return fail("engine_create: fp8 experts need attention_dim and hidden_units that are multiples of 64");
  if (c.fp8_activations && c.weight_dtype != M3_FP8) return fail("engine_create: fp8_activations needs weight_dtype fp8");
  if (c.ep_stages > 0 && c.fuse_route) return fail("engine_create: ep_stages needs the staged route (fuse_route = 0)");
  if (c.ep_world_size > 1 && (c.ep_rank < 0 || c.ep_rank >= c.ep_world_size)) return fail("engine_create: ep_rank outside [0, ep_world_size)");
  if (c.weight_dtype != M3_F32) {
    if (c.fuse_route) return fail("engine_create: fuse_route is fp32-only");
    if (c.attention_dim % 32 || c.hidden_units % 64 || c.embed_linear_units % 32)
      return fail("engine_create: bf16 weights need dims that are multiples of 32");
  }
  e->names.reserve(n_entries);
  for (int i = 0; i < n_entries; ++i) {
    if (!table[i].name || !table[i].data) return fail("engine_create: null weight entry");
    e->names.emplace_back(table[i].name);
    m3_weight_entry w = table[i];
    w.name = nullptr;
    e->table[e->names.back()] = w;
  }
  const int D = c.attention_dim, De = c.embed_dim, K = c.cnn_module_kernel;
  if (!load_sub(e, "embed.subsampling.", De, c.input_dim, &e->sub_e) || !load_sub(e, "subsampling.", D, c.input_dim, &e->sub_m))
    return fail(nullptr);
  if (!load_norm(e, "embed.after_norm.", De, &e->e_after) ||
      !load_lin_ln(e, "out_linear.", c.output_dim, D, false, &e->out_linear))
    return fail(nullptr);
  {
    auto m = e->table.find("cmvn.mean"), v = e->table.find("cmvn.istd"), ob = e->table.find("output_bias");
    if ((m == e->table.end()) != (v == e->table.end())) return fail("engine_create: cmvn.mean and cmvn.istd go together");
    if (m != e->table.end()) {
      if (m->second.numel != c.input_dim || v->second.numel != c.input_dim) return fail("engine_create: cmvn vectors must have input_dim entries");
      e->cmvn_mean = (const float*)m->second.data;
      e->cmvn_istd = (const float*)v->second.data;
    }
    if (ob != e->table.end()) {
      if (ob->second.numel != c.output_dim) return fail("engine_create: output_bias must have output_dim entries");
      e->output_bias = (const float*)ob->second.data;
    }
  }
  {
    auto it = e->table.find("pe");
    if (it == e->table.end() || it->second.numel % D) return fail("engine_create: positional table 'pe' missing");
    e->pe = (const float*)it->second.data;
    e->pe_rows = it->second.numel / D;
  }
  if (!lookup(e, "pos_all.weight", (int64_t)(c.embed_blocks + c.num_blocks) * D * D, &e->pos_all,
              c.weight_dtype == M3_F32 ? M3_F32 : M3_BF16))
    return fail(nullptr);
  if (c.fuse_route && !lookup(e, "router_e_all.weight", (int64_t)c.num_blocks * c.num_experts * De, &e->router_e_all))
    return fail(nullptr);
  e->eblocks.resize(c.embed_blocks);
  for (int i = 0; i < c.embed_blocks; ++i)
    if (!load_block(e, "embed.blocks." + std::to_string(i) + ".", De, c.embed_linear_units, K, c.embed_cnn_layer_norm,
                    false, De, &e->eblocks[i], c.embed_causal > 0))
      return fail(nullptr);
  e->mblocks.resize(c.num_blocks);
  for (int i = 0; i < c.num_blocks; ++i)
    if (!load_block(e, "blocks." + std::to_string(i) + ".", D, c.hidden_units, K, c.cnn_layer_norm, true, De,
                    &e->mblocks[i], c.causal > 0))
      return fail(nullptr);
  return e;
}

void m3_engine_destroy(m3_engine* engine) {
  if (!engine) return;
  if (engine->ev_fork) (void)hipEventDestroy(engine->ev_fork);
  if (engine->ev_join) (void)hipEventDestroy(engine->ev_join);
  if (engine->side) (void)hipStreamDestroy(engine->side);
  if (engine->cur.graph_exec) (void)hipGraphExecDestroy(engine->cur.graph_exec);
  for (auto& b : engine->parked)
    if (b.graph_exec) (void)hipGraphExecDestroy(b.graph_exec);
  delete engine;
}

size_t m3_engine_workspace_size(const m3_engine* engine, int B, int T) {
  if (!engine || B <= 0 || T < 7) return 0;
  return make_plan(engine->cfg, nullptr, B, T, engine->ep_capacity).bytes;
}

static int init_engine_kernels() {
  int (*const inits[])() = {init_expert_ffn_kernels, init_expert_ffn_bf16_kernels, init_expert_ffn_w8_kernels, init_gemm_bf16_tiled_kernels,
                            init_expert_ffn_f32_tiled_kernels, init_expert_ffn_fused_fp8_kernels, init_gemm_f32_tiled_kernels,
                            init_gemm_bf16_dma_kernels, init_expert_gemm_g256_kernels, init_moe_router_kernels,
                            init_relpos_attention_bf16_kernels, init_gemm_f32_splitk_kernels};
  for (auto init : inits)
    if (int rc = init()) return rc;
  return 0;
}

static int build_binding(m3_engine* e, const BindKey& k, m3_engine::Bound& bd) {
  M3_REQUIRE(k.feat && k.feat_len && k.logits && k.ws, "engine_prepare: null argument");
  const int B = k.B, T = k.T;
  M3_REQUIRE(B > 0 && T >= 7, "engine_prepare: need B > 0 and T >= 7 frames (got B=%d T=%d)", B, T);
  const m3_engine_config& c = e->cfg;
  const int Tp = sub_len(T);
  M3_REQUIRE(Tp < e->pe_rows, "engine_prepare: T'=%d exceeds the positional table (%lld rows)", Tp,
             (long long)e->pe_rows);
  if (int rc = init_engine_kernels()) return rc;
  const bool streaming = k.sstate != nullptr;
  StageBuilder sb{*e, make_plan(c, k.ws, B, T, k.ep_cap), bd,
                  streaming ? carve_stream_state(c, k.sstate, B, k.s_hist) : StreamState()};
  Plan& pl = sb.pl;
  M3_REQUIRE(k.ws_bytes >= pl.bytes, "engine_prepare: workspace %zu bytes < required %zu", k.ws_bytes, pl.bytes);
  const int32_t* feat_len = k.feat_len; float* logits = k.logits;
  bd.key = k; bd.Tp = Tp; bd.S = B * Tp;
  sb.splitk_ws = pl.splitk; sb.splitk_bytes = pl.splitk_bytes;
  {
    GemmParams t;
    t.M = B * Tp; t.N = c.attention_dim; t.K = c.attention_dim; t.w_bf16 = 1;
    bd.a16 = c.weight_dtype != M3_F32 && c.bf16_activations >= 0 && !c.debug_taps && c.embed_dim == c.attention_dim &&
             (c.embed_linear_units % 128) == 0 && (c.hidden_units % 128) == 0 && plan_gemm(t, 0).kernel == GemmKernel::TiledBf16;
  }
  {
    GemmParams t;
    t.M = B * Tp; t.N = c.attention_dim; t.K = c.attention_dim; t.lda = c.attention_dim; t.w_bf16 = 1; t.a_bf16 = 1;
    bd.dma = bd.a16 && c.attention_dim == 128 * kXbStatParts && plan_gemm(t, 0).kernel == GemmKernel::DmaBf16;
  }
  bd.packed = use_packed_rows(c, B);
  if (streaming) {
    bd.a16 = bd.dma = bd.packed = false;
  }
  const int S = bd.S, D = c.attention_dim, De = c.embed_dim;

  if (pl.ep_overflow != nullptr) {
    int32_t* ovf = pl.ep_overflow;
    add_stage(sb, "ep.reset", 0, [=](hipStream_t s) {
      M3_CHECK_HIP(hipMemsetAsync(ovf, 0, sizeof(int32_t), s));
      return 0;
    });
    bd.buffers["ep.overflow"] = Buf{ovf, sizeof(int32_t)};
  }
  {
    int32_t* lens = pl.lens;
    if (bd.packed) {
      int32_t* row0 = pl.row0; int32_t* pad_of = pl.pad_of;
      add_stage(sb, "pack_plan", 1, [=](hipStream_t s) { return launch_pack_plan(lens, B, Tp, row0, pad_of, s, feat_len); },
                stage_info("pack_plan_kernel", 1, 12.0 * B + 4.0 * B * Tp, 0.0, false));
    } else if (pl.fork || (!c.fold_pos_proj && !streaming)) {
      add_stage(sb, "lens", 1, [=](hipStream_t s) { return launch_subsample_lens(feat_len, B, lens, s); },
                stage_info("subsample_lens_kernel", 1, 8.0 * B, 0.0, false));
    } else {
      sb.lens_in_conv1 = true;
    }
  }
  {
    const int nb = c.num_blocks + c.embed_blocks;
    GemmParams pp;
    const int Tpos = streaming ? k.s_maxf : Tp;
    pp.A = e->pe; pp.lda = D; pp.W = e->pos_all; pp.Y = pl.pbuf; pp.ldy = nb * D; pp.M = Tpos; pp.N = nb * D; pp.K = D;
    if (c.fold_pos_proj || streaming) {
      auto known = e->pfold_by_tp.find(Tpos);
      std::shared_ptr<float> pf = known != e->pfold_by_tp.end() ? known->second.lock() : nullptr;
      if (!pf) {
        float* dev = nullptr;
        M3_CHECK_HIP(hipMalloc((void**)&dev, (size_t)Tpos * nb * D * sizeof(float)));
        pf = std::shared_ptr<float>(dev, [](float* q) { (void)hipFree(q); });
        pp.Y = dev;
        pp.w_bf16 = c.weight_dtype != M3_F32;
        if (int rc = launch_gemm(plan_gemm(pp, 0), pp, nullptr, nullptr)) return rc;
        M3_CHECK_HIP(hipStreamSynchronize(nullptr));
        for (auto it = e->pfold_by_tp.begin(); it != e->pfold_by_tp.end();)
          it = it->second.expired() ? e->pfold_by_tp.erase(it) : std::next(it);
        e->pfold_by_tp[Tpos] = pf;
      }
      bd.pfold = pf;
      pl.pbuf = pf.get();
    } else {
      add_gemm(sb, "pos_all", pp);
    }
  }
  const Plan ple = embed_view(pl);
  const int embed_start = (int)bd.stages.size();
  sb.splitk_ws = ple.splitk;
  build_subsample(sb, "embed.subsample.", e->sub_e, De, ple, ple.x);
  for (int i = 0; i < c.embed_blocks; ++i) {
    if (i + 1 == c.embed_blocks) {
      sb.tail_ln_g = e->e_after.g; sb.tail_ln_b = e->e_after.b; sb.tail_ln_eps = 1e-12f; sb.tail_ln_out = pl.emb;
    }
    build_block(sb, "embed.blocks." + std::to_string(i) + ".", e->eblocks[i], De, c.embed_linear_units, c.embed_heads,
                c.cnn_module_kernel, c.embed_cnn_layer_norm, false, i, i, ple, c.embed_causal > 0);
  }
  sb.splitk_ws = pl.splitk;
  if (c.embed_blocks == 0) {
    float* x = ple.x; float* emb = pl.emb;
    const float* g = e->e_after.g; const float* b = e->e_after.b;
    add_stage(sb, "embed.after_norm", 1, [=](hipStream_t s) { return launch_layernorm(x, g, b, 1e-12f, emb, S, De, s); },
              stage_info("layernorm_kernel", 1, 8.0 * S * De, 8.0 * S * De));
  }
  if (choose_moe_route(c, S, e->mblocks.empty() ? BlockW() : e->mblocks[0], pl).needs_e_all) {
    GemmParams g;
    g.A = pl.emb; g.lda = De; g.W = e->router_e_all; g.Y = pl.eall; g.ldy = c.num_blocks * c.num_experts;
    g.M = S; g.N = c.num_blocks * c.num_experts; g.K = De;
    add_gemm(sb, "router_e_all", g, true);
    bd.stages.back().reads_embed = true;
  }
  const int main_start = (int)bd.stages.size();
  build_subsample(sb, "subsample.", e->sub_m, D, pl, pl.x);
  for (int i = 0; i < c.num_blocks; ++i)
    build_block(sb, "blocks." + std::to_string(i) + ".", e->mblocks[i], D, c.hidden_units, c.attention_heads,
                c.cnn_module_kernel, c.cnn_layer_norm, true, i, c.embed_blocks + i, pl, c.causal > 0);
  {
    GemmParams g;
    g.A = pl.x; g.lda = D; g.W = e->out_linear.w; g.bias = e->out_linear.b; g.Y = logits; g.ldy = c.output_dim;
    g.M = S; g.N = c.output_dim; g.K = D;
    g.ln_wsum = e->out_linear.wsum; g.ln_eps = 1e-12f;
    if (bd.a16) { g.A = (const float*)pl.xb; g.a_bf16 = 1; }
    if (bd.dma) { g.ln_stats = pl.xstats; g.ln_stat_parts = kXbStatParts; }
    float* lout = logits;
    if (bd.packed) {
      lout = pl.lpk;
      g.Y = lout;
      g.m_dev = pl.row0 + B;
    }
    add_gemm(sb, "logits", g);
    const float* ob = e->output_bias;
    const int V = c.output_dim;
    if (c.log_softmax_out) {
      add_stage(sb, "log_softmax", 1, [=](hipStream_t s) { return launch_log_softmax_bias(lout, ob, lout, (size_t)S, V, s); },
                stage_info("log_softmax_bias_kernel", 1, 8.0 * S * V, 4.0 * S * V));
    }
    if (bd.packed) {
      const int32_t* row0 = pl.row0;
      add_stage(sb, "unpack", 1, [=](hipStream_t s) { return launch_unpack_rows(lout, row0, B, Tp, V, logits, s); },
                stage_info("unpack_rows_kernel", 1, 8.0 * S * V, 0.0, false));
    }
  }
  const int join = embed_join(bd.stages, main_start);
  if (pl.fork && join >= 0 && c.num_blocks >= 1) {
    bd.fork_first = embed_start; bd.fork_mid = main_start; bd.join_at = join;
  }
  if (pl.hfuse && !streaming && join > 0) fuse_independent_pairs(sb, embed_start, main_start, join);
  if (streaming) {
    const StreamState& st = sb.st;
    int32_t* step = st.step;
    if (k.s_slots) {
      int32_t *pos = st.slot_pos, *status = st.slot_status, *frames = st.slot_frames;
      const int32_t* lens = pl.lens; const int max_chunks = k.s_maxf / Tp;
      add_stage(sb, "stream.advance", 1, [=](hipStream_t s) { return launch_advance_slots(pos, status, frames, lens, B, Tp, max_chunks, s); },
                stage_info("advance_slots_kernel", 1, 20.0 * B, 0.0, false));
    } else
    add_stage(sb, "stream.advance", 1, [=](hipStream_t s) { return launch_advance_counter(step, 1, s); },
              stage_info("advance_counter_kernel", 1, 8.0, 0.0, false));
  }
  bd.buffers["x"] = Buf{pl.x, (size_t)S * D * 4};
  bd.buffers["dw"] = Buf{pl.dw, (size_t)S * D * 4};
  if (!bd.xn_skipped) bd.buffers["xn"] = Buf{pl.xn, (size_t)S * D * 4};
  if (pl.xq != nullptr) {
    bd.buffers["xq"] = Buf{pl.xq, (size_t)S * D};
    bd.buffers["xq_scale"] = Buf{pl.xq_scale, (size_t)S * 4};
  }
  bd.buffers["embed"] = Buf{pl.emb, (size_t)S * De * 4};
  if (bd.a16) bd.buffers["xb"] = Buf{pl.xb, (size_t)S * D * 2};
  bd.buffers["lens"] = Buf{pl.lens, (size_t)B * 4};
  if (bd.packed) bd.buffers["row0"] = Buf{pl.row0, (size_t)(B + 1) * 4};
  if (pl.ep_rows) bd.buffers["ep.gate_recv"] = Buf{pl.ep_gate_recv, (size_t)pl.ep_rows * 4};
  bd.buffers["router_logits"] = Buf{pl.rl, (size_t)S * c.num_experts * (c.ep_world_size > 0 ? c.ep_world_size : 1) * 4};

  return 0;
}

static int find_parked(const m3_engine* e, const BindKey& k) {
  for (size_t i = 0; i < e->parked.size(); ++i)
    if (e->parked[i].matches(k)) return (int)i;
  return -1;
}

static int shape_cache_capacity(const m3_engine* e) { return e->cfg.shape_cache > 0 ? e->cfg.shape_cache : (e->cfg.shape_cache < 0 ? 0 : 7); }

static int park_victim(const m3_engine* e) {
  if (e->parked.empty() || (int)e->parked.size() < shape_cache_capacity(e)) return -1;
  size_t lru = 0;
  for (size_t i = 1; i < e->parked.size(); ++i)
    if (e->parked[i].last_use < e->parked[lru].last_use) lru = i;
  return (int)lru;
}

static void park_current(m3_engine* e) {
  if (e->cur.stages.empty()) return;
  if (shape_cache_capacity(e) > 0) {
    const int victim = park_victim(e);
    if (victim >= 0) {
      if (e->parked[victim].graph_exec) (void)hipGraphExecDestroy(e->parked[victim].graph_exec);
      e->parked.erase(e->parked.begin() + victim);
    }
    e->parked.push_back(std::move(e->cur));
  } else if (e->cur.graph_exec) {
    (void)hipGraphExecDestroy(e->cur.graph_exec);
  }
  e->cur = m3_engine::Bound();
}

static int bind(m3_engine* e, const BindKey& k) {
  if (!e->cur.matches(k)) {
    int hit = find_parked(e, k);
    if (hit >= 0 && !e->cur.stages.empty() && hit == park_victim(e)) hit = -1;
    m3_engine::Bound fresh;
    if (hit < 0)
      if (int rc = build_binding(e, k, fresh)) return rc;
    park_current(e);
    if (hit >= 0) {
      hit = find_parked(e, k);
      fresh = std::move(e->parked[hit]);
      e->parked.erase(e->parked.begin() + hit);
    }
    e->cur = std::move(fresh);
  }
  e->cur.last_use = ++e->use_clock;
  return 0;
}

static BindKey forward_key(const m3_engine* e, const float* feat, const int32_t* feat_len, int B, int T, float* logits,
                           void* workspace, size_t workspace_bytes) {
  BindKey k;
  k.B = B; k.T = T; k.feat = feat; k.feat_len = feat_len; k.logits = logits; k.ws = workspace; k.ws_bytes = workspace_bytes;
  k.ep_cap = e->ep_capacity;
  return k;
}

int m3_engine_prepare(m3_engine* e, const float* feat, const int32_t* feat_len, int B, int T, float* logits,
                      void* workspace, size_t workspace_bytes) {
  M3_REQUIRE(e != nullptr, "engine_prepare: null argument");
  if (int rc = bind(e, forward_key(e, feat, feat_len, B, T, logits, workspace, workspace_bytes))) return rc;
  return (int)e->cur.stages.size();
}

int m3_engine_set_ep_capacity(m3_engine* engine, int rows_per_chunk) {
  M3_REQUIRE(engine != nullptr && rows_per_chunk >= 0, "engine_set_ep_capacity: bad argument");
  engine->ep_capacity = rows_per_chunk;
  return 0;
}

int m3_engine_num_stages(const m3_engine* engine) { return engine ? (int)engine->cur.stages.size() : 0; }
const char* m3_engine_stage_name(const m3_engine* engine, int index) {
  if (!engine || index < 0 || index >= (int)engine->cur.stages.size()) return nullptr;
  return engine->cur.stages[index].name.c_str();
}
int m3_engine_num_captures(const m3_engine* engine) { return engine ? engine->n_captures : 0; }
int m3_engine_stage_info(const m3_engine* engine, int index, m3_stage_info* info) {
  M3_REQUIRE(engine && info, "engine_stage_info: null argument");
  M3_REQUIRE(index >= 0 && index < (int)engine->cur.stages.size(), "engine_stage_info: no stage %d", index);
  *info = engine->cur.stages[index].info;
  return 0;
}
int m3_engine_num_kernels(const m3_engine* engine) { return engine ? engine->cur.n_kernels : 0; }

int m3_engine_run(m3_engine* engine, int first_stage, int last_stage, m3_stream stream) {
  M3_REQUIRE(engine && !engine->cur.stages.empty(), "engine_run: engine not prepared");
  M3_REQUIRE(first_stage >= 0 && last_stage <= (int)engine->cur.stages.size() && first_stage <= last_stage,
             "engine_run: bad stage range [%d,%d)", first_stage, last_stage);
  for (int i = first_stage; i < last_stage; ++i)
    if (int rc = engine->cur.stages[i].run((hipStream_t)stream)) return rc;
  return 0;
}

int m3_engine_buffer(const m3_engine* engine, const char* name, void** ptr, size_t* bytes) {
  M3_REQUIRE(engine && name && ptr && bytes, "engine_buffer: null argument");
  auto it = engine->cur.buffers.find(name);
  M3_REQUIRE(it != engine->cur.buffers.end(), "engine_buffer: no buffer named '%s' for the bound shape", name);
  *ptr = it->second.ptr;
  *bytes = it->second.bytes;
  return 0;
}

static int capture_graph(m3_engine* e, hipStream_t stream, const char* who) {
  m3_engine::Bound& b = e->cur;
  M3_REQUIRE(stream != nullptr, "%s: graph capture needs a non-default stream", who);
  if (b.graph_exec) {
    (void)hipGraphExecDestroy(b.graph_exec);
    b.graph_exec = nullptr;
  }
  hipGraph_t graph = nullptr;
  const m3_stream stream_ = (m3_stream)stream;
  const int n_st = (int)b.stages.size();
  const bool fork = b.fork_first >= 0 && b.fork_mid > b.fork_first && b.join_at > b.fork_mid;
  if (fork && e->side == nullptr) {
    M3_CHECK_HIP(hipStreamCreateWithFlags(&e->side, hipStreamNonBlocking));
    M3_CHECK_HIP(hipEventCreateWithFlags(&e->ev_fork, hipEventDisableTiming));
    M3_CHECK_HIP(hipEventCreateWithFlags(&e->ev_join, hipEventDisableTiming));
  }
  M3_CHECK_HIP(hipStreamBeginCapture(stream, hipStreamCaptureModeThreadLocal));
  int rc = 0;
  if (!fork) {
    rc = m3_engine_run(e, 0, n_st, stream_);
  } else {
    hipError_t he = hipSuccess;
    rc = m3_engine_run(e, 0, b.fork_first, stream_);
    if (!rc && (he = hipEventRecord(e->ev_fork, stream)) != hipSuccess) rc = -1;
    if (!rc && (he = hipStreamWaitEvent(e->side, e->ev_fork, 0)) != hipSuccess) rc = -1;
    if (!rc) rc = m3_engine_run(e, b.fork_first, b.fork_mid, (m3_stream)e->side);
    if (!rc) rc = m3_engine_run(e, b.fork_mid, b.join_at, stream_);
    if (!rc && (he = hipEventRecord(e->ev_join, e->side)) != hipSuccess) rc = -1;
    if (!rc && (he = hipStreamWaitEvent(stream, e->ev_join, 0)) != hipSuccess) rc = -1;
    if (!rc) rc = m3_engine_run(e, b.join_at, n_st, stream_);
    if (he != hipSuccess) set_error("%s: forked capture failed: %s", who, hipGetErrorString(he));
  }
  hipError_t ce = hipStreamEndCapture(stream, &graph);
  if (rc) {
    if (graph) (void)hipGraphDestroy(graph);
    return rc;
  }
  M3_CHECK_HIP(ce);
  M3_CHECK_HIP(hipGraphInstantiate(&b.graph_exec, graph, nullptr, nullptr, 0));
  M3_CHECK_HIP(hipGraphDestroy(graph));
  b.graph_valid = true;
  ++e->n_captures;
  return 0;
}

static int run_current(m3_engine* e, int use_graph, m3_stream stream_, const char* who) {
  if (!use_graph) return m3_engine_run(e, 0, (int)e->cur.stages.size(), stream_);
  hipStream_t stream = (hipStream_t)stream_;
  if (!e->cur.graph_valid)
    if (int rc = capture_graph(e, stream, who)) return rc;
  M3_CHECK_HIP(hipGraphLaunch(e->cur.graph_exec, stream));
  return 0;
}

int m3_engine_forward(m3_engine* e, const float* feat, const int32_t* feat_len, int B, int T, float* logits,
                      void* workspace, size_t workspace_bytes, int use_graph, m3_stream stream_) {
  M3_REQUIRE(e != nullptr, "engine_forward: null engine");
  if (int rc = bind(e, forward_key(e, feat, feat_len, B, T, logits, workspace, workspace_bytes))) return rc;
  M3_REQUIRE(e->cfg.ep_world_size <= 1, "engine_forward: an expert-parallel engine (ep_world_size = %d) is run stage-wise, with the "
             "all-to-all between its moe_ep.* stages (m3asr/ep.py)", (int)e->cfg.ep_world_size);
  return run_current(e, use_graph, stream_, "engine_forward");
}


static int stream_check(const m3_engine* e, const m3_stream_desc* d) {
  M3_REQUIRE(e != nullptr && d != nullptr, "engine stream: null argument");
  const m3_engine_config& c = e->cfg;
  M3_REQUIRE(c.static_chunk_size > 0, "engine stream: the engine was built without static_chunk_size (the chunk length in output frames)");
  M3_REQUIRE(c.causal > 0 && c.embed_causal > 0, "engine stream: both encoders need causal conv modules (a symmetric depthwise conv "
             "looks %d frames into the future)", (int)(c.cnn_module_kernel - 1) / 2);
  M3_REQUIRE(c.ep_world_size <= 1 && c.ep_stages <= 0 && c.fork_embed <= 0, "engine stream: expert-parallel stages / forked capture are not available chunk by chunk");
  M3_REQUIRE(d->B > 0 && d->max_frames >= c.static_chunk_size && d->max_frames < e->pe_rows,
             "engine stream: need B > 0 and chunk <= max_frames < %lld positions (got B=%d max_frames=%d)", (long long)e->pe_rows, d->B, d->max_frames);
  const int need = c.num_left_chunks < 0 ? d->max_frames : (c.num_left_chunks + 1) * c.static_chunk_size;
  M3_REQUIRE(d->history_frames >= need, "engine stream: history_frames=%d < %d (%s)", d->history_frames, need,
             c.num_left_chunks < 0 ? "all left chunks are visible: the history must hold the whole stream" : "(num_left_chunks + 1) chunks");
  return 0;
}

static int stream_state(const m3_engine* e, const m3_stream_desc* d, const void* state, size_t state_bytes, const char* who,
                        StreamState* st) {
  if (int rc = stream_check(e, d)) return rc;
  *st = carve_stream_state(e->cfg, const_cast<void*>(state), d->B, d->history_frames);
  M3_REQUIRE(state != nullptr && state_bytes >= st->bytes, "%s: state %zu bytes < required %zu", who, state_bytes, st->bytes);
  return 0;
}

int m3_engine_chunk_input_frames(const m3_engine* engine) {
  return engine && engine->cfg.static_chunk_size > 0 ? 4 * engine->cfg.static_chunk_size + 3 : 0;
}

size_t m3_engine_stream_state_size(const m3_engine* engine, const m3_stream_desc* desc) {
  if (stream_check(engine, desc)) return 0;
  return carve_stream_state(engine->cfg, nullptr, desc->B, desc->history_frames).bytes;
}

int m3_engine_stream_reset(m3_engine* e, const m3_stream_desc* desc, void* state, size_t state_bytes, m3_stream stream_) {
  StreamState st;
  if (int rc = stream_state(e, desc, state, state_bytes, "engine_stream_reset", &st)) return rc;
  const m3_engine_config& c = e->cfg;
  hipStream_t stream = (hipStream_t)stream_;
  M3_CHECK_HIP(hipMemsetAsync(st.step, 0, 64 * sizeof(int32_t), stream));
  M3_CHECK_HIP(hipMemsetAsync(st.slot_pos, 0, (size_t)3 * desc->B * sizeof(int32_t), stream));
  const int K = c.cnn_module_kernel, D = c.attention_dim, nb = c.embed_blocks + c.num_blocks;
  for (int i = 0; i < nb; ++i) {
    const BlockW& w = i < c.embed_blocks ? e->eblocks[i] : e->mblocks[i - c.embed_blocks];
    if (int rc = launch_fill_rows(w.left_fill, D, st.conv[i], (size_t)2 * desc->B * (K - 1), stream)) return rc;
  }
  return 0;
}

static int run_chunk(m3_engine* e, const m3_stream_desc* desc, void* state, const float* feat_chunk, const int32_t* chunk_feat_len,
                     float* logits, void* workspace, size_t workspace_bytes, bool slots, int use_graph, m3_stream stream_) {
  BindKey k = forward_key(e, feat_chunk, chunk_feat_len, desc->B, 4 * e->cfg.static_chunk_size + 3, logits, workspace, workspace_bytes);
  k.sstate = state; k.s_hist = desc->history_frames; k.s_maxf = desc->max_frames; k.s_slots = slots;
  if (int rc = bind(e, k)) return rc;
  return run_current(e, use_graph, stream_, "engine_forward_chunk");
}

int m3_engine_forward_chunk(m3_engine* e, const m3_stream_desc* desc, void* state, size_t state_bytes, const float* feat_chunk,
                            const int32_t* chunk_feat_len, float* logits, void* workspace, size_t workspace_bytes, int chunk_index,
                            int use_graph, m3_stream stream_) {
  StreamState st;
  if (int rc = stream_state(e, desc, state, state_bytes, "engine_forward_chunk", &st)) return rc;
  M3_REQUIRE(chunk_index >= 0 && (long)(chunk_index + 1) * e->cfg.static_chunk_size <= desc->max_frames,
             "engine_forward_chunk: chunk %d ends past max_frames=%d (the stream is longer than the state was sized for)", chunk_index, desc->max_frames);
  return run_chunk(e, desc, state, feat_chunk, chunk_feat_len, logits, workspace, workspace_bytes, false, use_graph, stream_);
}

int m3_engine_forward_chunk_slots(m3_engine* e, const m3_stream_desc* desc, void* state, size_t state_bytes, const float* feat_chunk,
                                  const int32_t* chunk_feat_len, float* logits, void* workspace, size_t workspace_bytes,
                                  int use_graph, m3_stream stream_) {
  StreamState st;
  if (int rc = stream_state(e, desc, state, state_bytes, "engine_forward_chunk_slots", &st)) return rc;
  return run_chunk(e, desc, state, feat_chunk, chunk_feat_len, logits, workspace, workspace_bytes, true, use_graph, stream_);
}

int m3_engine_stream_reset_slots(m3_engine* e, const m3_stream_desc* desc, void* state, size_t state_bytes, const int32_t* slots,
                                 int n, m3_stream stream_) {
  StreamState st;
  if (int rc = stream_state(e, desc, state, state_bytes, "engine_stream_reset_slots", &st)) return rc;
  const m3_engine_config& c = e->cfg;
  M3_REQUIRE(n >= 0 && (n == 0 || slots != nullptr), "engine_stream_reset_slots: bad slot list (n=%d)", n);
  const int nb = c.embed_blocks + c.num_blocks;
  M3_REQUIRE(nb <= kMaxStreamBlocks, "engine_stream_reset_slots: %d blocks > %d", nb, kMaxStreamBlocks);
  SlotResetArgs a;
  a.pos = st.slot_pos; a.status = st.slot_status; a.frames = st.slot_frames; a.slots = slots; a.n = n;
  a.B = desc->B; a.K = c.cnn_module_kernel; a.D = c.attention_dim; a.n_blocks = nb;
  for (int i = 0; i < kMaxStreamBlocks; ++i) { a.conv[i] = nullptr; a.fill[i] = nullptr; }
  for (int i = 0; i < nb; ++i) {
    a.conv[i] = st.conv[i];
    a.fill[i] = (i < c.embed_blocks ? e->eblocks[i] : e->mblocks[i - c.embed_blocks]).left_fill;
  }
  return launch_reset_slots(a, (hipStream_t)stream_);
}

int m3_engine_stream_positions(m3_engine* e, const m3_stream_desc* desc, const void* state, size_t state_bytes, int32_t* frames,
                               m3_stream stream_) {
  StreamState st;
  if (int rc = stream_state(e, desc, state, state_bytes, "engine_stream_positions", &st)) return rc;
  M3_REQUIRE(frames != nullptr, "engine_stream_positions: null pointer");
  return launch_slot_positions(st.slot_status, st.slot_frames, desc->B, frames, (hipStream_t)stream_);
}

}
```

### 3m-asr-inference_amd/csrc/gemm.hip

```cpp
#include "common.h"
#include "gemm_epilogue.h"
#include "kernels.h"

#ifdef M3_GEMM_DIAG
#define M3_GDIAG(...) __VA_ARGS__
#else
#define M3_GDIAG(...)
#endif

namespace m3 {

M3_GDIAG(__device__ unsigned long long g_gemm_dbg[2048 * 8];)

enum { LN_NONE = GEMM_LN_NONE, LN_EPI = GEMM_LN_EPI, LN_PRO = GEMM_LN_PRO };

template <int MT, bool GLU, int NW, bool CONV, int LN, int NBUF>
__device__ __forceinline__ void gemm_f32_body(const GemmParams& p, const int bid) {
  constexpr int NT = GLU ? 2 : 1;
  constexpr int G = gemm_group_steps(MT, NT, NW);
  constexpr int RW = (16 * MT) / NW;
  static_assert(RW >= 1, "more waves than rows");
  __shared__ float red[NW][MT * NT][256];
  __shared__ float stats[16 * MT][2];
  __shared__ float rsum[LN == LN_EPI ? NW : 1][16 * MT][2];
  __shared__ __attribute__((aligned(16))) float ln_g[LN == LN_PRO ? 1024 : 4], ln_b[LN == LN_PRO ? 1024 : 4];

  M3_GDIAG(unsigned long long dg[8]; dg[0] = __builtin_amdgcn_s_memtime();)
  asm volatile("" ::"s"(p.A), "s"(p.lda), "s"(p.W), "s"(p.bias), "s"(p.Y), "s"(p.ldy), "s"(p.M), "s"(p.N), "s"(p.K), "s"(p.mode),
               "s"(p.n_tiles), "s"(p.m_tiles), "s"(p.xcd_swizzle), "s"(p.m_dev), "s"(p.resid), "s"(p.ldr), "s"(p.act), "s"(p.alpha),
               "s"(p.mask_in), "s"(p.mask_out), "s"(p.row_len), "s"(p.rows_per_batch));
  if (LN == LN_EPI) asm volatile("" ::"s"(p.ln_wsum), "s"(p.ln_wbeta), "s"(p.ln_eps));
  if (LN == LN_PRO) asm volatile("" ::"s"(p.ln_gamma), "s"(p.ln_beta), "s"(p.ln_eps), "s"(p.ln_out), "s"(p.ld_ln_out), "s"(p.ln_on_a2));
  if (!CONV) asm volatile("" ::"s"(p.A2), "s"(p.lda2), "s"(p.K1));
  if (CONV) asm volatile("" ::"s"(p.conv_T1), "s"(p.conv_F1), "s"(p.conv_T2), "s"(p.conv_F2), "s"(p.conv_C));
  const int lane = threadIdx.x & 63, wave = threadIdx.x >> 6;
  const int col = lane & 15, kq = lane >> 4;
  const int Nout = GLU ? (p.N >> 1) : p.N;

  int n_tile, m_tile;
  {
    const int id = bid;
    if (p.xcd_swizzle) {
      const int j = id >> 3;
      m_tile = j % p.m_tiles;
      n_tile = (j / p.m_tiles) * 8 + (id & 7);
    } else {
      n_tile = id % p.n_tiles;
      m_tile = id / p.n_tiles;
    }
  }
  const int n0 = n_tile * 16;
  const int m0 = m_tile * (16 * MT);
  if (p.m_dev != nullptr && m0 > *p.m_dev) return;
  const int ln_k0 = p.ln_on_a2 ? p.K1 : 0;
  const int Kl = p.K - ln_k0;

  const float* arow[MT];
  const float* arow2[MT];
#pragma unroll
  for (int mt = 0; mt < MT; ++mt) {
    const int m = min(m0 + 16 * mt + col, p.M - 1);
    arow2[mt] = nullptr;
    if (CONV) {
      const int f2 = m % p.conv_F2;
      const int t2 = (m / p.conv_F2) % p.conv_T2;
      const int b = m / (p.conv_F2 * p.conv_T2);
      arow[mt] = p.A + ((size_t)(b * p.conv_T1 + 2 * t2) * p.conv_F1 + 2 * f2) * p.conv_C + 4 * kq;
    } else {
      arow[mt] = p.A + (size_t)m * p.lda + 4 * kq;
      if (p.mode == GEMM_A_CONCAT2) arow2[mt] = p.A2 + (size_t)m * p.lda2 + 4 * kq;
    }
  }
  const float* wrow[NT];
#pragma unroll
  for (int t = 0; t < NT; ++t)
    wrow[t] = p.W + (size_t)min(n0 + t * Nout + col, p.N - 1) * p.K + 4 * kq;

  f32x4 acc[MT][NT];
#pragma unroll
  for (int mt = 0; mt < MT; ++mt)
#pragma unroll
    for (int t = 0; t < NT; ++t) acc[mt][t] = f32x4{0.f, 0.f, 0.f, 0.f};
  constexpr bool DUAL = MT * NT <= 2;
  f32x4 acc2[MT][NT];
#pragma unroll
  for (int mt = 0; mt < MT; ++mt)
#pragma unroll
    for (int t = 0; t < NT; ++t) acc2[mt][t] = f32x4{0.f, 0.f, 0.f, 0.f};
  float s1[MT], s2[MT];
#pragma unroll
  for (int mt = 0; mt < MT; ++mt) s1[mt] = s2[mt] = 0.f;

  const int nsteps = p.K >> 4;
  auto a_offset = [&](int k) -> int {
    if (CONV) {
      const int seg = k / p.conv_C, c = k - seg * p.conv_C;
      const int kh = seg / 3, kw = seg - kh * 3;
      return (kh * p.conv_F1 + kw) * p.conv_C + c;
    }
    return k;
  };

  f32x4 wbuf[NBUF][G][NT], abuf[NBUF][G][MT];
  auto load_group = [&](int g, int buf) {
#pragma unroll
    for (int i = 0; i < G; ++i) {
      const int s = min(wave + NW * (G * g + i), nsteps - 1);
      const int k = s << 4;
#pragma unroll
      for (int t = 0; t < NT; ++t) wbuf[buf][i][t] = ldg4_w(wrow[t] + k);
      const bool second = !CONV && p.mode == GEMM_A_CONCAT2 && k >= p.K1;
      const int off = second ? (k - p.K1) : a_offset(k);
#pragma unroll
      for (int mt = 0; mt < MT; ++mt) abuf[buf][i][mt] = ldg4((second ? arow2[mt] : arow[mt]) + off);
    }
  };

  const int ngroups = (nsteps + NW * G - 1) / (NW * G);
  M3_GDIAG(dg[1] = __builtin_amdgcn_s_memtime();)
  load_group(0, 0);
  M3_GDIAG(dg[2] = __builtin_amdgcn_s_memtime();)
  const int ep_mt = wave;
  const bool is_ep = wave < MT;
  const int ep_n = n0 + col;
  float bias0 = 0.f, bias1 = 0.f, wsum0 = 0.f, wsum1 = 0.f, wbeta0 = 0.f, wbeta1 = 0.f, res[4] = {0.f, 0.f, 0.f, 0.f};
  if (is_ep && ep_n < Nout) {
    if (p.bias) {
      bias0 = p.bias[ep_n];
      if (GLU) bias1 = p.bias[ep_n + Nout];
    }
    if (LN == LN_EPI) {
      wsum0 = p.ln_wsum[ep_n];
      if (GLU) wsum1 = p.ln_wsum[ep_n + Nout];
      if (p.mask_in) {
        wbeta0 = p.ln_wbeta[ep_n];
        if (GLU) wbeta1 = p.ln_wbeta[ep_n + Nout];
      }
    }
    if (p.resid) {
#pragma unroll
      for (int r = 0; r < 4; ++r) {
        const int m = min(m0 + 16 * ep_mt + 4 * kq + r, p.M - 1);
        res[r] = p.resid[(size_t)m * p.ldr + ep_n];
      }
    }
  }
  bool pad4[4] = {false, false, false, false};
  if (is_ep && (p.mask_in || p.mask_out)) {
#pragma unroll
    for (int r = 0; r < 4; ++r) {
      const int m = min(m0 + 16 * ep_mt + 4 * kq + r, p.M - 1);
      pad4[r] = gemm_row_padded(p, m);
    }
  }


  float a_mean[MT], a_rstd[MT];
  float* ln_out_row[MT];
#pragma unroll
  for (int mt = 0; mt < MT; ++mt) {
    a_mean[mt] = 0.f;
    a_rstd[mt] = 1.f;
    ln_out_row[mt] = nullptr;
  }
  if (LN == LN_PRO) {
    const float* lnA = p.ln_on_a2 ? p.A2 : p.A;
    const int ldl = p.ln_on_a2 ? p.lda2 : p.lda;
    for (int k = threadIdx.x * 4; k < Kl; k += 256 * NW) {
      *reinterpret_cast<f32x4*>(&ln_g[k]) = ldg4(p.ln_gamma + k);
      *reinterpret_cast<f32x4*>(&ln_b[k]) = ldg4(p.ln_beta + k);
    }
    const int q = lane >> 4, l16 = lane & 15;
    const int nj = (Kl + 63) >> 6;
    for (int c = 0; c < (RW + 3) / 4; ++c) {
      const int rloc = wave * RW + 4 * c + q;
      const bool row_on = (4 * c + q) < RW;
      const int m = min(m0 + min(rloc, 16 * MT - 1), p.M - 1);
      const float* row = lnA + (size_t)m * ldl;
      f32x4 v[16];
#pragma unroll
      for (int j = 0; j < 16; ++j) {
        const int k = 4 * (l16 + 16 * j);
        const f32x4 t = ldg4(row + min(k, Kl - 4));
        const bool in = j < nj && k < Kl;
        v[j] = f32x4{in ? t[0] : 0.f, in ? t[1] : 0.f, in ? t[2] : 0.f, in ? t[3] : 0.f};
      }
      float sum = 0.f;
#pragma unroll
      for (int j = 0; j < 16; ++j) sum += (v[j][0] + v[j][1]) + (v[j][2] + v[j][3]);
      const float mean = group16_sum(sum) / (float)Kl;
      float sq = 0.f;
#pragma unroll
      for (int j = 0; j < 16; ++j) {
        const int k = 4 * (l16 + 16 * j);
        const float on = (j < nj && k < Kl) ? 1.f : 0.f;
#pragma unroll
        for (int e = 0; e < 4; ++e) {
          const float d = (v[j][e] - mean) * on;
          sq += d * d;
        }
      }
      const float var = group16_sum(sq) / (float)Kl;
      if (row_on && l16 == 0) {
        stats[rloc][0] = mean;
        stats[rloc][1] = rsqrtf(var + p.ln_eps);
      }
    }
    __syncthreads();
#pragma unroll
    for (int mt = 0; mt < MT; ++mt) {
      a_mean[mt] = stats[16 * mt + col][0];
      a_rstd[mt] = stats[16 * mt + col][1];
      const int m = m0 + 16 * mt + col;
      if (p.ln_out != nullptr && n_tile == 0 && m < p.M) ln_out_row[mt] = p.ln_out + (size_t)m * p.ld_ln_out + 4 * kq;
    }
  }

  auto compute_group = [&](int g, int buf) {
#pragma unroll
    for (int i = 0; i < G; ++i) {
      const int s = wave + NW * (G * g + i);
      if (s < nsteps) {
        const int k = s << 4;
        const bool in_ln = k >= ln_k0;
        f32x4 g4, b4;
        if (LN == LN_PRO && in_ln) {
          g4 = *reinterpret_cast<const f32x4*>(&ln_g[(k - ln_k0) + 4 * kq]);
          b4 = *reinterpret_cast<const f32x4*>(&ln_b[(k - ln_k0) + 4 * kq]);
        }
#pragma unroll
        for (int mt = 0; mt < MT; ++mt) {
          f32x4 a = abuf[buf][i][mt];
          if (LN == LN_PRO && in_ln) {
#pragma unroll
            for (int j = 0; j < 4; ++j) a[j] = (a[j] - a_mean[mt]) * a_rstd[mt] * g4[j] + b4[j];
            if (ln_out_row[mt] != nullptr) stg4(ln_out_row[mt] + (k - ln_k0), a);
          }
          if (LN == LN_EPI && in_ln) {
            s1[mt] += (a[0] + a[1]) + (a[2] + a[3]);
            s2[mt] += (a[0] * a[0] + a[1] * a[1]) + (a[2] * a[2] + a[3] * a[3]);
          }
#pragma unroll
          for (int t = 0; t < NT; ++t) {
            if (DUAL) {
#pragma unroll
              for (int j = 0; j < 4; j += 2) {
                acc[mt][t] = mfma16(a[j], wbuf[buf][i][t][j], acc[mt][t]);
                acc2[mt][t] = mfma16(a[j + 1], wbuf[buf][i][t][j + 1], acc2[mt][t]);
              }
            } else {
#pragma unroll
              for (int j = 0; j < 4; ++j) acc[mt][t] = mfma16(a[j], wbuf[buf][i][t][j], acc[mt][t]);
            }
          }
        }
      }
    }
  };

  M3_GDIAG(asm volatile("s_waitcnt vmcnt(0)" ::: "memory"); dg[3] = __builtin_amdgcn_s_memtime();)
  if (NBUF == 1) {
    compute_group(0, 0);
  } else {
    for (int g = 0; g < ngroups; g += 2) {
      if (g + 1 < ngroups) load_group(g + 1, NBUF - 1);
      compute_group(g, 0);
      if (g + 1 < ngroups) {
        if (g + 2 < ngroups) load_group(g + 2, 0);
        compute_group(g + 1, NBUF - 1);
      }
    }
  }

  if (DUAL) {
#pragma unroll
    for (int mt = 0; mt < MT; ++mt)
#pragma unroll
      for (int t = 0; t < NT; ++t) acc[mt][t] += acc2[mt][t];
  }
  M3_GDIAG(asm volatile("s_nop 15\n\ts_nop 15" ::: "memory"); dg[4] = __builtin_amdgcn_s_memtime();)
#pragma unroll
  for (int mt = 0; mt < MT; ++mt)
#pragma unroll
    for (int t = 0; t < NT; ++t)
#pragma unroll
      for (int r = 0; r < 4; ++r) red[wave][mt * NT + t][r * 64 + lane] = acc[mt][t][r];
  if (LN == LN_EPI) {
#pragma unroll
    for (int mt = 0; mt < MT; ++mt) {
      float a1 = s1[mt], a2 = s2[mt];
      a1 += __shfl_xor(a1, 16, 64);
      a2 += __shfl_xor(a2, 16, 64);
      a1 += __shfl_xor(a1, 32, 64);
      a2 += __shfl_xor(a2, 32, 64);
      if (kq == 0) {
        rsum[wave][16 * mt + col][0] = a1;
        rsum[wave][16 * mt + col][1] = a2;
      }
    }
  }
  __syncthreads();
  M3_GDIAG(dg[5] = __builtin_amdgcn_s_memtime();)

  if (is_ep) {
    const int mt = ep_mt;
    f32x4 v[NT];
#pragma unroll
    for (int t = 0; t < NT; ++t)
#pragma unroll
      for (int r = 0; r < 4; ++r) {
        float sum = 0.f;
#pragma unroll
        for (int w = 0; w < NW; w += 4)
          sum += (red[w][mt * NT + t][r * 64 + lane] + red[w + 1][mt * NT + t][r * 64 + lane]) +
                 (red[w + 2][mt * NT + t][r * 64 + lane] + red[w + 3][mt * NT + t][r * 64 + lane]);
        v[t][r] = sum;
      }
    if (ep_n < Nout) {
#pragma unroll
      for (int r = 0; r < 4; ++r) {
        const int row = 16 * mt + 4 * kq + r;
        const int m = m0 + row;
        if (m >= p.M) continue;
        float y0 = v[0][r], y1 = v[NT - 1][r];
        const bool pad = pad4[r];
        if (LN != LN_EPI && p.mask_in && pad) y0 = y1 = 0.f;
        float mean = 0.f, rstd = 1.f;
        if (LN == LN_EPI) {
          float t1 = 0.f, t2 = 0.f;
#pragma unroll
          for (int w = 0; w < NW; ++w) {
            t1 += rsum[w][row][0];
            t2 += rsum[w][row][1];
          }
          ln_mean_rstd(t1, t2, Kl, p.ln_eps, mean, rstd);
        }
        p.Y[(size_t)m * p.ldy + ep_n] =
            gemm_epilogue<GLU, LN == LN_EPI>(y0, y1, bias0, bias1, wsum0, wsum1, wbeta0, wbeta1, mean, rstd, pad, res[r], p);
      }
    }
  }
  M3_GDIAG(dg[6] = __builtin_amdgcn_s_memtime();
           asm volatile("s_waitcnt vmcnt(0)" ::: "memory");
           dg[7] = __builtin_amdgcn_s_memtime();
           if (lane == 0 && wave == 0 && bid < 2048) {
             unsigned long long* o = g_gemm_dbg + (size_t)bid * 8;
             for (int i = 0; i < 8; ++i) o[i] = dg[i];
             const unsigned hw = __builtin_amdgcn_s_getreg((31 << 11) | 4), xcc = __builtin_amdgcn_s_getreg((31 << 11) | 20);
             o[7] = (dg[7] & 0xffffffffffull) | ((unsigned long long)(hw & 0xffff) << 40) | ((unsigned long long)(xcc & 0xf) << 56);
           })
}

template <int MT, bool GLU, int NW, bool CONV, int LN, int NBUF>
__global__ __launch_bounds__(64 * NW) void gemm_f32_kernel(const GemmParams p) {
  gemm_f32_body<MT, GLU, NW, CONV, LN, NBUF>(p, (int)blockIdx.x);
}
template <int MT, bool GLU, int NW, int LN>
__global__ __launch_bounds__(64 * NW) void gemm_f32_dual_kernel(const GemmParams p0, const GemmParams p1, const int n0) {
  if ((int)blockIdx.x < n0) {
    if ((int)blockIdx.x < p0.n_tiles * p0.m_tiles) gemm_f32_body<MT, GLU, NW, false, LN, 1>(p0, (int)blockIdx.x);
  } else {
    gemm_f32_body<MT, GLU, NW, false, LN, 1>(p1, (int)blockIdx.x - n0);
  }
}

int launch_gemm_f32_dual(const GemmPlan& pa, const GemmParams& a_in, const GemmPlan& pb, const GemmParams& b_in, hipStream_t stream) {
  M3_REQUIRE(gemm_dual_fusable(pa, pb), "gemm dual: the two problems do not share an instantiation");
  GemmParams q[2] = {a_in, b_in};
  const GemmPlan* const plans[2] = {&pa, &pb};
  for (int i = 0; i < 2; ++i) {
    q[i].n_tiles = plans[i]->n_tiles; q[i].m_tiles = plans[i]->m_tiles; q[i].xcd_swizzle = plans[i]->xcd_swizzle;
  }
  const int n0 = (int)align_up((size_t)q[0].n_tiles * q[0].m_tiles, 8);
  dim3 grid(n0 + q[1].n_tiles * q[1].m_tiles);
#define M3_DUAL(GLU_, NW_, LN_)                                                                                             \
  hipLaunchKernelGGL((gemm_f32_dual_kernel<1, GLU_, NW_, LN_>), grid, dim3(64 * NW_), 0, stream, q[0], q[1], n0)
  if (pa.glu) {
    if (pa.nw == 8) { if (pa.ln == LN_EPI) M3_DUAL(true, 8, LN_EPI); else M3_DUAL(true, 8, LN_NONE); }
    else { if (pa.ln == LN_EPI) M3_DUAL(true, 4, LN_EPI); else M3_DUAL(true, 4, LN_NONE); }
  } else {
    if (pa.nw == 8) { if (pa.ln == LN_EPI) M3_DUAL(false, 8, LN_EPI); else M3_DUAL(false, 8, LN_NONE); }
    else { if (pa.ln == LN_EPI) M3_DUAL(false, 4, LN_EPI); else M3_DUAL(false, 4, LN_NONE); }
  }
#undef M3_DUAL
  M3_LAUNCH_CHECK();
  return 0;
}

int launch_gemm_f32_skinny(const GemmPlan& plan, const GemmParams& pin, hipStream_t stream) {
  GemmParams p = pin;
  p.n_tiles = plan.n_tiles; p.m_tiles = plan.m_tiles; p.xcd_swizzle = plan.xcd_swizzle;
  dim3 grid(p.n_tiles * p.m_tiles);
  const int mt = plan.mt, nw = plan.nw, ln = plan.ln;

#define M3_GEMM_LAUNCH(MT_, GLU_, NW_, CONV_, LN_)                                                              \
  do {                                                                                                          \
    if (plan.nbuf == 1)                                                                                         \
      hipLaunchKernelGGL((gemm_f32_kernel<MT_, GLU_, NW_, CONV_, LN_, 1>), grid, dim3(64 * NW_), 0, stream, p); \
    else                                                                                                        \
      hipLaunchKernelGGL((gemm_f32_kernel<MT_, GLU_, NW_, CONV_, LN_, 2>), grid, dim3(64 * NW_), 0, stream, p); \
  } while (0)
#define M3_GEMM_MT(GLU_, NW_, CONV_, LN_)                                                              \
  do {                                                                                                 \
    if (mt == 1) M3_GEMM_LAUNCH(1, GLU_, NW_, CONV_, LN_);                                             \
    else if (mt == 2) M3_GEMM_LAUNCH(2, GLU_, NW_, CONV_, LN_);                                        \
    else M3_GEMM_LAUNCH(4, GLU_, NW_, CONV_, LN_);                                                     \
  } while (0)
#define M3_GEMM_LN(GLU_, NW_)                                                                          \
  do {                                                                                                 \
    if (ln == LN_EPI) M3_GEMM_MT(GLU_, NW_, false, LN_EPI);                                            \
    else if (ln == LN_PRO) M3_GEMM_MT(GLU_, NW_, false, LN_PRO);                                       \
    else M3_GEMM_MT(GLU_, NW_, false, LN_NONE);                                                        \
  } while (0)
  if (plan.conv) {
    if (nw == 16) M3_GEMM_MT(false, 16, true, LN_NONE); else if (nw == 8) M3_GEMM_MT(false, 8, true, LN_NONE);
    else M3_GEMM_MT(false, 4, true, LN_NONE);
  } else if (nw == 16) {
    M3_GEMM_MT(false, 16, false, LN_NONE);
  } else if (plan.glu) {
    if (nw == 8) M3_GEMM_LN(true, 8); else M3_GEMM_LN(true, 4);
  } else {
    if (nw == 8) M3_GEMM_LN(false, 8); else M3_GEMM_LN(false, 4);
  }
#undef M3_GEMM_LN
#undef M3_GEMM_MT
#undef M3_GEMM_LAUNCH
  M3_LAUNCH_CHECK();
  return 0;
}

}

#ifdef M3_GEMM_DIAG
extern "C" int m3_debug_gemm_read(void* dst, size_t bytes) {
  return (int)hipMemcpyFromSymbol(dst, HIP_SYMBOL(m3::g_gemm_dbg), bytes < sizeof(m3::g_gemm_dbg) ? bytes : sizeof(m3::g_gemm_dbg));
}
#endif
```

### 3m-asr-inference_amd/csrc/gemm_plan.hip

```cpp
#include <stdlib.h>

#include "common.h"
#include "kernels.h"

namespace m3 {

static int env_int(const char* name, int dflt) {
  const char* e = getenv(name);
  return e ? atoi(e) : dflt;
}

#define M3_PLAN_REQUIRE(cond, ...)                                  \
  do {                                                              \
    if (!(cond)) {                                                  \
      snprintf(plan.reason, sizeof(plan.reason), __VA_ARGS__);      \
      return false;                                                 \
    }                                                               \
  } while (0)

static bool operands_ok(const GemmParams& p, const char* who, GemmPlan& plan) {
  const int kmult = p.w_bf16 ? 32 : 16;
  M3_PLAN_REQUIRE(p.grp_acc == nullptr, "%s: grouped (per-expert) operands belong to the expert FFN's plan", who);
  M3_PLAN_REQUIRE(p.M > 0 && p.N > 0 && p.K > 0, "%s: empty problem M=%d N=%d K=%d", who, p.M, p.N, p.K);
  M3_PLAN_REQUIRE(p.K % kmult == 0, "%s: K=%d must be a multiple of %d", who, p.K, kmult);
  M3_PLAN_REQUIRE((p.lda & 3) == 0, "%s: lda=%d must be a multiple of 4", who, p.lda);
  M3_PLAN_REQUIRE(!plan.glu || (p.N & 1) == 0, "%s: GLU needs even N", who);
  if (plan.conv) {
    M3_PLAN_REQUIRE(p.conv_C % kmult == 0 && p.K == 9 * p.conv_C, "%s: conv mode needs K=9*C, C%%%d==0", who, kmult);
    M3_PLAN_REQUIRE(!plan.glu && plan.ln == GEMM_LN_NONE, "%s: conv mode supports neither GLU nor LayerNorm", who);
  }
  M3_PLAN_REQUIRE(!(p.ln_wsum && p.mask_in) || p.ln_wbeta, "%s: folded LayerNorm + input mask needs ln_wbeta", who);
  if (p.mask_in || p.mask_out) M3_PLAN_REQUIRE(p.row_len && p.rows_per_batch > 0, "%s: mask needs row_len", who);
  return true;
}

static int splitk_ranges(const GemmParams& p, size_t* ws_bytes) {
  if (p.w_bf16 || p.K < 4096 || (p.K & 63) || (p.N & 3) || (p.lda & 3) || (p.ldy & 3)) return 0;
  if (p.mode == GEMM_A_CONCAT2 || p.ln_wsum || p.ln_gamma || p.mask_in || p.mask_out || p.resid || p.act == ACT_GLU) return 0;
  if (p.mode == GEMM_A_CONV3X3S2 && (p.conv_C & 63)) return 0;
  const long tiles = (long)cdiv(p.M, 64) * cdiv(p.N, 64);
  if (tiles > 160) return 0;
  const int nsteps = p.K / 64;
  int splits = (int)(512 / tiles);
  if (splits > nsteps / 4) splits = nsteps / 4;
  if (splits < 2) return 0;
  splits = cdiv(nsteps, cdiv(nsteps, splits));
  *ws_bytes = (size_t)splits * p.M * p.N * sizeof(float);
  return splits;
}

static void tiled_grid(const GemmParams& p, GemmPlan& plan, int bm, int bn, int bk) {
  plan.bm = bm; plan.bn = bn; plan.bk = bk;
  plan.m_tiles = cdiv(p.M, bm);
  plan.n_tiles = plan.glu ? cdiv(p.N / 2, bn / 2) : cdiv(p.N, bn);
}

static void skinny_grid(const GemmParams& p, GemmPlan& plan, int Nout) {
  int mt = p.M <= 128 ? 1 : (p.M <= 512 ? 2 : 4);
  while (mt < 4 && 16 * mt < p.M && (long)cdiv(Nout, 16) * cdiv(p.M, 16 * mt) > 512) mt *= 2;
  while (!p.w_bf16 && mt > 1 && (long)cdiv(Nout, 16) * cdiv(p.M, 16 * mt) < 256) mt /= 2;
  plan.mt = mt;
  plan.n_tiles = cdiv(Nout, 16);
  plan.m_tiles = cdiv(p.M, 16 * mt);
  plan.xcd_swizzle = (plan.n_tiles % 8 == 0) ? 1 : 0;
  plan.nw = p.K >= 2048 ? 16 : (p.K >= 1024 ? 8 : 4);
  if (plan.nw == 16 && (plan.glu || mt == 4 || plan.ln != GEMM_LN_NONE)) plan.nw = 8;
  const int steps = p.w_bf16 ? (p.K >> 5) : (p.K >> 4);
  const int group = p.w_bf16 ? gemm16_group_steps(mt, plan.nw) : gemm_group_steps(mt, plan.glu ? 2 : 1, plan.nw);
  plan.nbuf = steps <= plan.nw * group ? 1 : 2;
}

static bool choose_form(const GemmParams& p, size_t ws_avail, GemmPlan& plan) {
  static const int tiled_min_rows = env_int("M3_TILED_MIN_ROWS", 384);
  static const int dma_min_rows = env_int("M3_DMA_MIN_ROWS", 4096);
  static const int thin_below = env_int("M3_TILED_THIN_BELOW", 0);
  const bool glu = plan.glu, conv = plan.conv, concat = p.mode == GEMM_A_CONCAT2;
  const int Nout = glu ? p.N / 2 : p.N;
  const long tiles64 = (long)cdiv(p.M, 64) * cdiv(Nout, 64);
  const bool long_batch = p.M >= tiled_min_rows && tiles64 >= 160 && !concat && p.ln_gamma == nullptr;
  const bool big = (long)cdiv(p.M, 128) * cdiv(p.N, 128) >= 200;

  size_t need = 0;
  if (const int splits = splitk_ranges(p, &need); splits >= 2 && ws_avail >= need) {
    plan.kernel = GemmKernel::SplitKF32; plan.label = "gemm_f32_splitk_kernel";
    plan.splits = splits; plan.ws_bytes = need;
    plan.bm = plan.bn = plan.bk = 64;
    plan.m_tiles = cdiv(p.M, 64); plan.n_tiles = cdiv(p.N, 64);
    return true;
  }
  if (p.w_bf16) {
    const char* who = "gemm_bf16w";
    M3_PLAN_REQUIRE(!concat, "%s: concat operands are fp32-only (the router stays fp32)", who);
    M3_PLAN_REQUIRE(p.ln_gamma == nullptr && p.ln_out == nullptr, "%s: only the folded LayerNorm (ln_wsum) is available with bf16 weights", who);
    if (plan.ln) M3_PLAN_REQUIRE(p.mode == GEMM_A_PLAIN && p.K <= 2047, "%s: LayerNorm needs plain A with K < 2048", who);
    const bool bf16_out_ok = (Nout & 3) == 0 && (p.ldy & 3) == 0 && (p.ldyb & 3) == 0;
    if (p.M >= dma_min_rows && p.a_bf16 && p.mode == GEMM_A_PLAIN && p.w_scale == nullptr && (p.K & 63) == 0 && (p.lda & 7) == 0 &&
        (p.ln_wsum == nullptr || p.ln_stats != nullptr) && ((size_t)(p.M - 1) * p.lda + p.K) * 2 < ((size_t)1 << 32) &&
        (size_t)p.N * p.K * 2 < ((size_t)1 << 32)) {
      M3_PLAN_REQUIRE(!(p.y_bf16 || p.Yb) || bf16_out_ok, "gemm_bf16_dma: bf16 output needs N %% 4 == 0");
      plan.kernel = GemmKernel::DmaBf16; plan.label = "gemm_bf16_dma_kernel";
      tiled_grid(p, plan, 128, 128, 64);
      plan.stages = (long)plan.m_tiles * plan.n_tiles <= device_cu_count() && p.K / 64 >= 4 ? 4 : 2;
      return true;
    }
    M3_PLAN_REQUIRE(p.Yb_stats == nullptr && p.ln_stats == nullptr,
                    "%s: y_copy_stats / ln_stats need the LDS-DMA kernel (M >= %d rows, bf16 A); this problem (M=%d) runs on another one",
                    who, dma_min_rows, p.M);
    if (long_batch && (p.K & 127) == 0 && (!conv || (p.conv_C & 127) == 0)) {
      if (p.a_bf16 && !conv) M3_PLAN_REQUIRE((p.lda & 7) == 0, "%s: bf16 A needs lda %% 8 == 0", who);
      M3_PLAN_REQUIRE(!(p.y_bf16 || p.Yb) || bf16_out_ok, "%s: bf16 output needs N %% 4 == 0", who);
      plan.kernel = GemmKernel::TiledBf16; plan.label = "gemm_bf16w_tiled_kernel";
      const bool thin = !big && !conv && (long)cdiv(p.M, 64) * cdiv(p.N, 64) < thin_below;
      if (big) tiled_grid(p, plan, 128, 128, 64); else tiled_grid(p, plan, thin ? 32 : 64, 64, 128);
      return true;
    }
    M3_PLAN_REQUIRE(!p.a_bf16 && !p.y_bf16 && p.Yb == nullptr, "%s: bf16 activations are a feature of the tiled kernel", who);
    plan.kernel = GemmKernel::SkinnyBf16; plan.label = "gemm_bf16w_kernel";
    skinny_grid(p, plan, Nout);
    return true;
  }
  const char* who = "gemm";
  if (concat) M3_PLAN_REQUIRE((p.K1 & 15) == 0 && p.A2 != nullptr && (p.lda2 & 3) == 0, "%s: bad concat operands", who);
  M3_PLAN_REQUIRE(!(p.ln_wsum && p.ln_gamma), "%s: folded (ln_wsum) and affine (ln_gamma) LayerNorm are exclusive", who);
  if (plan.ln != GEMM_LN_NONE) {
    M3_PLAN_REQUIRE(p.mode == GEMM_A_PLAIN || (concat && p.ln_on_a2), "%s: LayerNorm needs plain A (or the A2 half of a concat)", who);
    M3_PLAN_REQUIRE((p.ln_on_a2 ? p.K - p.K1 : p.K) <= 1024, "%s: LayerNorm supports rows up to 1024 wide", who);
    M3_PLAN_REQUIRE(p.K <= 2047, "%s: LayerNorm variants are built for K < 2048", who);
  }
  M3_PLAN_REQUIRE(!p.ln_on_a2 || concat, "%s: ln_on_a2 needs concat mode", who);
  M3_PLAN_REQUIRE(p.ln_out == nullptr || plan.ln == GEMM_LN_PRO, "%s: ln_out needs the affine LayerNorm prologue", who);
  if (long_batch && (p.K & 63) == 0 && (!conv || (p.conv_C & 63) == 0)) {
    plan.kernel = GemmKernel::TiledF32; plan.label = "gemm_f32_tiled_kernel";
    if (big) tiled_grid(p, plan, 128, 128, 32); else tiled_grid(p, plan, 64, 64, 64);
    return true;
  }
  plan.kernel = GemmKernel::SkinnyF32; plan.label = "gemm_f32_kernel";
  skinny_grid(p, plan, Nout);
  plan.dual_ok = plan.mt == 1 && (plan.nw == 4 || plan.nw == 8) && plan.nbuf == 1 && p.mode == GEMM_A_PLAIN &&
                 plan.ln != GEMM_LN_PRO && p.m_dev == nullptr;
  return true;
}

GemmPlan plan_gemm(const GemmParams& p, size_t workspace_bytes_available) {
  GemmPlan plan{};
  plan.kernel = p.w_bf16 ? GemmKernel::SkinnyBf16 : GemmKernel::SkinnyF32;
  plan.label = "";
  plan.glu = p.act == ACT_GLU; plan.conv = p.mode == GEMM_A_CONV3X3S2;
  plan.ln = p.ln_wsum ? GEMM_LN_EPI : (p.ln_gamma ? GEMM_LN_PRO : GEMM_LN_NONE);
  if (operands_ok(p, p.w_bf16 ? "gemm_bf16w" : "gemm", plan) && choose_form(p, workspace_bytes_available, plan))
    plan.launches = plan.kernel == GemmKernel::SplitKF32 ? 2 : 1;
  return plan;
}

bool gemm_dual_fusable(const GemmPlan& a, const GemmPlan& b) {
  return a.launches == 1 && b.launches == 1 && a.dual_ok && b.dual_ok && a.nw == b.nw && a.ln == b.ln && a.glu == b.glu;
}

int launch_gemm(const GemmPlan& plan, const GemmParams& p, float* ws, hipStream_t stream) {
  M3_REQUIRE(plan.launches > 0, "%s", plan.reason);
  switch (plan.kernel) {
    case GemmKernel::SkinnyF32: return launch_gemm_f32_skinny(plan, p, stream);
    case GemmKernel::SkinnyBf16: return launch_gemm_bf16w_skinny(plan, p, stream);
    case GemmKernel::TiledF32: return launch_gemm_f32_tiled(plan, p, stream);
    case GemmKernel::TiledBf16: return launch_gemm_bf16w_tiled(plan, p, stream);
    case GemmKernel::DmaBf16: return launch_gemm_bf16_dma(plan, p, stream);
    case GemmKernel::SplitKF32:
      M3_REQUIRE(ws != nullptr, "gemm split-K: the plan was made for a workspace of %zu bytes, none given", plan.ws_bytes);
      return launch_gemm_f32_splitk(plan, p, ws, stream);
  }
  return -2;
}

}
```

### 3m-asr-inference_amd/csrc/kernels.h

```cpp
#pragma once
#include <hip/hip_runtime.h>
#include <stdint.h>

#include "../../include/m3asr.h"

namespace m3 {

enum { ACT_NONE = 0, ACT_RELU = 1, ACT_SILU = 2, ACT_GLU = 3 };
enum { GEMM_A_PLAIN = 0, GEMM_A_CONCAT2 = 1, GEMM_A_CONV3X3S2 = 2 };

struct GemmParams {
  const float* A = nullptr; int lda = 0;
  const float* A2 = nullptr; int lda2 = 0; int K1 = 0;
  const float* W = nullptr;
  int w_bf16 = 0;
  const float* bias = nullptr;
  float* Y = nullptr; int ldy = 0;
  int M = 0, N = 0, K = 0;
  int mode = GEMM_A_PLAIN;
  const float* ln_gamma = nullptr; const float* ln_beta = nullptr; float ln_eps = 0.f;
  const float* ln_wsum = nullptr; const float* ln_wbeta = nullptr;
  int ln_on_a2 = 0;
  float* ln_out = nullptr; int ld_ln_out = 0;
  const int32_t* row_len = nullptr; int rows_per_batch = 0;
  int mask_in = 0, mask_out = 0;
  int conv_T1 = 0, conv_F1 = 0, conv_T2 = 0, conv_F2 = 0, conv_C = 0;
  int act = ACT_NONE;
  float alpha = 1.f;
  const float* resid = nullptr; int ldr = 0;
  const int32_t* grp_acc = nullptr; int grp_E = 0; const int32_t* grp_pos = nullptr; int w_sliced = 0;
  const float* w_scale = nullptr;
  int a_bf16 = 0, y_bf16 = 0; void* Yb = nullptr; int ldyb = 0;
  float* Yb_stats = nullptr; const float* ln_stats = nullptr; int ln_stat_parts = 0;
  const int32_t* m_dev = nullptr;
  const int32_t* y_rows = nullptr;
  const int32_t* conv_len = nullptr;
  int n_tiles = 0, m_tiles = 0, xcd_swizzle = 0;
};
enum { GEMM_LN_NONE = 0, GEMM_LN_EPI = 1, GEMM_LN_PRO = 2 };
enum class GemmKernel { SkinnyF32, SkinnyBf16, TiledF32, TiledBf16, DmaBf16, SplitKF32 };
struct GemmPlan {
  GemmKernel kernel;
  const char* label;
  int launches;
  bool glu, conv; int ln;
  int mt, nw, nbuf;
  bool dual_ok;
  int bm, bn, bk;
  int stages;
  int m_tiles, n_tiles, xcd_swizzle;
  int splits; size_t ws_bytes;
  char reason[192];
};
GemmPlan plan_gemm(const GemmParams& p, size_t workspace_bytes_available);
int launch_gemm(const GemmPlan& plan, const GemmParams& p, float* ws, hipStream_t stream);
bool gemm_dual_fusable(const GemmPlan& a, const GemmPlan& b);
int launch_gemm_f32_dual(const GemmPlan& pa, const GemmParams& a, const GemmPlan& pb, const GemmParams& b, hipStream_t stream);
constexpr int gemm_group_steps(int MT, int NT, int NW) {
  if (NW == 16) return MT == 1 ? (NT == 1 ? 4 : 2) : (MT == 2 ? 2 : 1);
  if (NW == 8) return MT == 1 ? 8 : (MT == 2 ? (NT == 1 ? 6 : 4) : (NT == 1 ? 3 : 2));
  return MT == 1 ? 8 : (MT == 2 ? 6 : 4);
}
constexpr int gemm16_group_steps(int MT, int NW) { return NW == 16 ? 2 : (MT == 4 ? 2 : 4); }
int launch_gemm_f32_skinny(const GemmPlan& plan, const GemmParams& p, hipStream_t stream);
int launch_gemm_bf16w_skinny(const GemmPlan& plan, const GemmParams& p, hipStream_t stream);
int launch_gemm_f32_tiled(const GemmPlan& plan, const GemmParams& p, hipStream_t stream);
int launch_gemm_bf16w_tiled(const GemmPlan& plan, const GemmParams& p, hipStream_t stream);
int launch_gemm_bf16_dma(const GemmPlan& plan, const GemmParams& p, hipStream_t stream);
int launch_gemm_f32_splitk(const GemmPlan& plan, const GemmParams& p, float* ws, hipStream_t stream);
bool gemm_splitk_dual_fusable(const GemmPlan& a, const GemmPlan& b);
int launch_gemm_f32_splitk_dual(const GemmPlan& pa, const GemmParams& a, float* ws_a, const GemmPlan& pb, const GemmParams& b, float* ws_b,
                                hipStream_t stream, int which = 3);
int init_gemm_f32_splitk_kernels();
int init_gemm_bf16_tiled_kernels();
int init_gemm_f32_tiled_kernels();
int init_gemm_bf16_dma_kernels();
constexpr int kXbStatParts = 4;
int launch_row_stats_bf16(const void* xb, int rows, int D, float* stats, hipStream_t stream);

int launch_moe_index(const int32_t* gate_idx, int S, int E, int32_t* mapping, int32_t* acc_hist,
                     int32_t* pos, hipStream_t stream);
int launch_moe_gate_index(const float* logits, int width, const int32_t* row_len, int rows_per_batch, int S,
                          int32_t* gate_idx, float* gate_value, int32_t* mapping, int32_t* acc_hist, int32_t* pos,
                          hipStream_t stream);
int launch_moe_route(const float* x, int ldx, int D, const float* wx, const float* wsum, const float* bias,
                     const float* eall, int ld_e, float ln_eps, const int32_t* row_len, int rows_per_batch, int S, int E,
                     int32_t* gate_idx, float* gate_value, int32_t* mapping, int32_t* acc_hist, int32_t* pos,
                     hipStream_t stream);
bool moe_router_supports(int De, int D, int N);
bool moe_router_fuses_top1(int N);
int init_moe_router_kernels();
int launch_moe_router(const float* emb, int lde, int De, const float* x, int ldx, int D, const float* W, const float* bias,
                      const float* gamma, const float* beta, float eps, float* xn, int ldxn, float* Y, int ldy, int M, int N,
                      const int32_t* m_dev, hipStream_t stream, int32_t* gate_idx = nullptr, float* gate_val = nullptr,
                      const int32_t* row_len = nullptr, int rows_per_batch = 0, void* xq = nullptr, float* xq_scale = nullptr);
int launch_local_scatter(const void* x, const int32_t* mapping, int S, int row_bytes, void* out, hipStream_t stream);
int launch_local_gather(const void* buf, const int32_t* mapping, int S, int row_bytes, void* out, hipStream_t stream);

int launch_ep_send_map(const int32_t* gate_idx, const int32_t* mapping, const int32_t* acc_hist, int S, int world, int e_loc,
                       int capacity, int32_t* map_send, void* wire, int row_bytes, hipStream_t stream, int32_t* overflow = nullptr);
int launch_ep_send_rows(const int32_t* gate_idx, const int32_t* mapping, const int32_t* acc_hist, int S, int world, int e_loc,
                        int capacity, int32_t* map_send, const void* x, void* wire, int row_bytes, hipStream_t stream, int32_t* overflow = nullptr);
int launch_ep_recv_gate(const void* wire, int world, int e_loc, int capacity, int row_bytes, int32_t* gate_recv,
                        hipStream_t stream);

#ifndef M3_EXPERT_SLICE
#define M3_EXPERT_SLICE 64
#endif
constexpr int kExpertSliceW16 = 64;
constexpr int kExpertSlice = M3_EXPERT_SLICE;
size_t expert_ffn_slab_bytes(int S, int D, int F);
enum class ExpertWeights { F32, BF16, FP8, FP8A8 };
enum class ExpertKernel { SlabF32, TiledF32, SlabBf16, TiledBf16, G256Bf16, SlabW8, TiledW8, FusedFp8 };
struct ExpertFfnPlan {
  ExpertWeights weights; ExpertKernel kernel;
  const char* label;
  int launches, slices;
  int fsplit;
  size_t h_off, rows_off, xb_off;
  float* rows(float* slab) const { return (float*)((char*)slab + rows_off); }
};
enum { EXPERT_NORM_IN_KERNEL = 1,
       EXPERT_SCATTER_ROWS = 2 };
ExpertFfnPlan plan_expert_ffn(ExpertWeights w, int S, int E, int D, int F, unsigned flags = 0);
struct ExpertFfnArgs { const float* x; int ldx; const int32_t *pos, *acc_hist; const void *w1, *w2; const float *s1, *s2, *b1, *b2;
                       int w2_sliced; float h_scale; float* slab; const float *ln_gamma, *ln_beta; float ln_eps;
                       const void* xq; const float* xq_scale; int32_t* fs_dev; float* y_scatter; };
int launch_expert_ffn(const ExpertFfnPlan& plan, int S, int E, int D, int F, const ExpertFfnArgs& a, hipStream_t stream);
int init_expert_ffn_kernels();
int launch_expert_ffn_f32_slab(const float* x, int ldx, const int32_t* pos, const int32_t* acc_hist, int S, int E,
                               int D, int F, const float* w1, const float* b1, const float* w2, int w2_sliced, float* slab,
                               const float* ln_gamma, const float* ln_beta, float ln_eps, hipStream_t stream);
int init_expert_ffn_f32_tiled_kernels();
int launch_expert_tiled_f32(const float* x, int ldx, const int32_t* pos, const int32_t* acc_hist, int S, int E,
                            int D, int F, const float* w1, const float* b1, const float* w2, int w2_sliced,
                            float* hbuf, float* ybuf, hipStream_t stream);
int init_expert_ffn_bf16_kernels();
int launch_expert_ffn_bf16w_slab(const float* x, int ldx, const int32_t* pos, const int32_t* acc_hist, int S, int E,
                                 int D, int F, const void* w1, const float* b1, const void* w2, int w2_sliced, float* slab,
                                 hipStream_t stream);
int init_expert_ffn_w8_kernels();
int launch_expert_ffn_w8_slab(const float* x, int ldx, const int32_t* pos, const int32_t* acc_hist, int S, int E, int D, int F,
                              const void* w1, const float* s1, const float* b1, const void* w2, const float* s2, int w2_sliced,
                              float* slab, hipStream_t stream);
constexpr int kExpertFusedFp8MaxSplit = 4;
int expert_ffn_fused_fp8_fsplit(int S, int E, int D, int F);
int init_expert_ffn_fused_fp8_kernels();
int launch_expert_ffn_fused_fp8(const float* x, int ldx, const int32_t* pos, const int32_t* acc_hist, int S, int E, int D, int F,
                                const void* w1, const float* s1, const float* b1, const void* w2, const float* s2, int w2_sliced,
                                float h_scale, int fsplit, float* ybuf, hipStream_t stream, const void* xq = nullptr,
                                const float* xq_scale = nullptr, int32_t* fs_dev = nullptr);
int launch_quantize_rows_e4m3(const float* x, int ldx, int S, int D, void* xq, float* scale, hipStream_t stream);
int launch_expert_tiled_w16(bool w_fp8, const float* x, int ldx, const int32_t* pos, const int32_t* acc_hist, int S, int E,
                            int D, int F, const void* w1, const float* s1, const float* b1, const void* w2, const float* s2,
                            int w2_sliced, void* hbuf, float* ybuf, hipStream_t stream, const float* b2 = nullptr,
                            float* y_scatter = nullptr);
bool expert_ffn_f32_self_routing(int S, int E);
int launch_expert_route_ffn_f32(const float* x, int ldx, const float* logits, const int32_t* row_len, int rows_per_batch, int S, int E,
                                int D, int F, const float* w1, const float* b1, const float* w2, int w2_sliced, const float* b2,
                                float* slab, int32_t* gate_idx, float* gate_value, int32_t* mapping, int32_t* acc_hist, int32_t* pos,
                                hipStream_t stream, const float* ln_gamma = nullptr, const float* ln_beta = nullptr, float ln_eps = 0.f);
bool expert_gemm_g256_takes(int S, int E, int D, int F);
int init_expert_gemm_g256_kernels();
int launch_rows_to_bf16(const float* x, int ldx, int S, int D, void* xb, hipStream_t stream);
int launch_expert_ffn_bf16_g256(const void* xb, int ldxb, const int32_t* pos, const int32_t* acc_hist, int S, int E, int D, int F,
                                const void* w1, const float* b1, const void* w2, int w2_sliced, void* hbuf, float* ybuf,
                                hipStream_t stream);
int launch_moe_combine(const float* slab, int n_slices, const int32_t* mapping, const int32_t* gate_idx,
                       const float* gate_value, const float* b2, const float* resid, float alpha,
                       const float* ln_gamma, const float* ln_beta, float ln_eps, float* out, int S, int D,
                       hipStream_t stream, void* out_bf16 = nullptr, float* out_stats = nullptr,
                       const int32_t* n_slices_dev = nullptr);

int launch_layernorm(const float* x, const float* gamma, const float* beta, float eps, float* y, int rows, int D,
                     hipStream_t stream, void* y_bf16 = nullptr, float* y_stats = nullptr, const float* gamma2 = nullptr,
                     const float* beta2 = nullptr, float eps2 = 0.f, float* y2 = nullptr);
int launch_softmax_top1(const float* logits, int ld, const int32_t* row_len, int rows_per_batch, int S, int E,
                        int32_t* idx, float* value, hipStream_t stream);
int launch_att_masked_softmax(const float* scores, const int32_t* len, int B, int H, int T1, int T2, float scale,
                              float* out, hipStream_t stream);
int launch_masked_fill(const float* x, const int32_t* len, int B, int C, int T, float fill, float* y,
                       hipStream_t stream);
int launch_glu(const float* x, int outer, int C, int inner, float* y, hipStream_t stream);
int launch_scale(const float* x, float scale, float* y, size_t n, hipStream_t stream);
int launch_mask_conv2d_sample(const int32_t* len_in, int B, int left_padding, int stride, int32_t* len_out,
                              hipStream_t stream);
int launch_subsample_lens(const int32_t* len_in, int B, int32_t* len_out, hipStream_t stream);
int launch_add(const float* a, const float* b, float* y, size_t n, hipStream_t stream);
int launch_binary_bcast(const float* a, const float* b, float* y, const int64_t* shape, const int64_t* sa,
                        const int64_t* sb, int nd, int op, hipStream_t stream);
int launch_unary(const float* x, float* y, size_t n, int act, hipStream_t stream);
int launch_permute(const float* x, float* y, const int64_t* out_shape, const int64_t* in_strides, int nd,
                   hipStream_t stream);
int launch_concat_last(const float* a, int da, const float* b, int db, float* y, size_t rows, hipStream_t stream);
int launch_softmax_lastdim(const float* x, float* y, size_t rows, int n, hipStream_t stream);
int launch_bmm(const float* a, const float* b, float* c, int batch, int M, int N, int K, int64_t sa, int64_t sb,
               int trans_b, hipStream_t stream);

int launch_relpos_attention(const float* qkv, int ldq, const float* pmat, int ldp, const float* pos_u,
                            const float* pos_v, const int32_t* row_len, int B, int T, int H, int dk, float scale,
                            float* out, int ldo, hipStream_t stream, int out_bf16 = 0, const int32_t* row0 = nullptr,
                            int chunk = 0, int left_chunks = -1);
struct AttArgs {
  const float* qkv = nullptr; int ldq = 0; const float* pmat = nullptr; int ldp = 0; const float *pos_u = nullptr, *pos_v = nullptr;
  const int32_t* row_len = nullptr; int B = 0, T = 0, H = 0, dk = 0; float scale = 1.f; float* out = nullptr; int ldo = 0, out_bf16 = 0;
  const int32_t* row0 = nullptr; int chunk = 0, left_chunks = 0;
};
int launch_relpos_attention_args(const AttArgs& a, hipStream_t stream);
bool relpos_attention_dual_fusable(const AttArgs& a, const AttArgs& b);
int launch_relpos_attention_dual(const AttArgs& a, const AttArgs& b, hipStream_t stream);
int launch_relpos_attention_stream(const float* qkv, int ldq, float* hist, int cap, const float* pmat, int ldp, const float* pos_u,
                                   const float* pos_v, const int32_t* chunk_len, const int32_t* step, int B, int C, int H, int dk,
                                   float scale, float* out, int ldo, int left_chunks, hipStream_t stream,
                                   int slot_max_chunks = -1);

bool relpos_attention_bf16_supports(int T, int dk);
int init_relpos_attention_bf16_kernels();
int launch_relpos_attention_bf16(const void* qkv, int ldq, const float* pmat, int ldp, const float* pos_u, const float* pos_v,
                                 const int32_t* row_len, int B, int T, int H, int dk, float scale, void* out, int ldo,
                                 hipStream_t stream, const int32_t* row0 = nullptr, int chunk = 0, int left_chunks = -1);

int launch_dwconv_ln_silu(const float* z, const float* w_kc, const float* bias, const float* gamma,
                          const float* beta, float eps, int B, int T, int D, int K, float* out, hipStream_t stream,
                          int out_bf16 = 0, const int32_t* pad_of = nullptr, const int32_t* row0 = nullptr,
                          const int32_t* row_len = nullptr, const float* causal_left_fill = nullptr);
int launch_pad2d(const float* x, size_t outer, int H, int W, int pre_h, int post_h, int pre_w, int post_w, float* y, hipStream_t stream);
int launch_advance_counter(int32_t* counter, int by, hipStream_t stream);
int launch_fill_rows(const float* row, int D, float* out, size_t rows, hipStream_t stream);
int launch_advance_slots(int32_t* pos, int32_t* status, int32_t* frames, const int32_t* chunk_len, int B, int C, int max_chunks,
                         hipStream_t stream);
constexpr int kMaxStreamBlocks = 64;
struct SlotResetArgs {
  int32_t *pos = nullptr, *status = nullptr, *frames = nullptr;
  const int32_t* slots = nullptr; int n = 0;
  int B = 0, K = 0, D = 0, n_blocks = 0;
  float* conv[kMaxStreamBlocks];
  const float* fill[kMaxStreamBlocks];
};
int launch_reset_slots(const SlotResetArgs& a, hipStream_t stream);
int launch_slot_positions(const int32_t* status, const int32_t* frames, int B, int32_t* out, hipStream_t stream);
struct DwArgs {
  const float *z = nullptr, *w_kc = nullptr, *bias = nullptr, *gamma = nullptr, *beta = nullptr; float eps = 1e-5f;
  int B = 0, T = 0, D = 0, K = 0; float* out = nullptr; int out_bf16 = 0;
  const int32_t *pad_of = nullptr, *row0 = nullptr, *row_len = nullptr; const float* causal_left_fill = nullptr;
  int glu_ldz = 0;
};
int launch_dwconv_ln_silu_args(const DwArgs& a, hipStream_t stream);
bool dwconv_glu_in_supports(int D, int K, bool causal_or_stream, int out_bf16, int ldz);
bool dwconv_dual_fusable(const DwArgs& a, const DwArgs& b);
int launch_dwconv_ln_silu_dual(const DwArgs& a, const DwArgs& b, hipStream_t stream);
int launch_dwconv_ln_silu_stream(const float* z, const float* w_kc, const float* bias, const float* gamma, const float* beta,
                                 float eps, int B, int T, int D, int K, float* out, float* cache_pair, const int32_t* step,
                                 const int32_t* chunk_len, hipStream_t stream, int out_bf16 = 0,
                                 int slot_max_chunks = -1);
int launch_pack_plan(int32_t* len, int B, int T, int32_t* row0, int32_t* pad_of, hipStream_t stream,
                     const int32_t* feat_len = nullptr);
int launch_unpack_rows(const float* in, const int32_t* row0, int B, int T, int n, float* out, hipStream_t stream);
int launch_conv1_relu(const float* feat, const float* w9c, const float* bias, const float* cmvn_mean,
                      const float* cmvn_istd, int B, int T, int idim, int C, float* out, hipStream_t stream, int relu = 1,
                      int out_bf16 = 0, const int32_t* feat_len = nullptr, int32_t* lens_out = nullptr);
struct Conv1Args {
  const float *feat = nullptr, *w9c = nullptr, *bias = nullptr, *cmvn_mean = nullptr, *cmvn_istd = nullptr;
  int B = 0, T = 0, idim = 0, C = 0; float* out = nullptr; int relu = 1, out_bf16 = 0;
  const int32_t* feat_len = nullptr; int32_t* lens_out = nullptr;
};
int launch_conv1_relu_args(const Conv1Args& a, hipStream_t stream);
bool conv1_dual_fusable(const Conv1Args& a, const Conv1Args& b);
int launch_conv1_relu_dual(const Conv1Args& a, const Conv1Args& b, hipStream_t stream);
int launch_cmvn(const float* x, const int32_t* len, const float* mean, const float* istd, int B, int T, int D,
                float* y, hipStream_t stream);
int launch_log_softmax_bias(const float* x, const float* bias, float* y, size_t rows, int n, hipStream_t stream);
int launch_ctc_greedy(const float* logits, const int32_t* len, int B, int T, int V, int blank, int32_t* frame_ids,
                      int32_t* tokens, int32_t* n_tokens, hipStream_t stream);
int launch_ctc_topk(const float* logits, size_t rows, int V, int k, float* top_logp, int32_t* top_idx, hipStream_t stream);
int ctc_prefix_beam_search_host(const float* top_logp, const int32_t* top_idx, int T, int k, int beam, int blank,
                                int32_t* hyp_tokens, int32_t* hyp_len, float* hyp_score, int32_t* n_hyps);
int launch_ctc_argmax(const float* logits, size_t rows, int V, int32_t* ids, hipStream_t stream);
size_t ctc_beam_state_size(const m3_ctc_beam_desc* d);
int launch_ctc_beam_reset(const m3_ctc_beam_desc* d, void* state, size_t bytes, hipStream_t stream,
                          const int32_t* slots = nullptr, int n = 0);
int launch_ctc_beam_advance(const m3_ctc_beam_desc* d, void* state, size_t bytes, const float* top_logp, const int32_t* top_idx,
                            int T_chunk, const int32_t* n_frames, hipStream_t stream);
int launch_ctc_beam_nbest(const m3_ctc_beam_desc* d, const void* state, size_t bytes, int32_t* hyp_tokens, int32_t* hyp_len,
                          float* hyp_score, int32_t* n_hyps, hipStream_t stream);
size_t ctc_align_workspace_size(const m3_ctc_align_desc* d);
int launch_ctc_align_emit(const m3_ctc_align_desc* d, const float* logits, int ldl, const int32_t* row0, const int32_t* n_frames,
                          const int32_t* tokens, const int32_t* tok0, float* emit, hipStream_t stream);
int launch_ctc_align_path(const m3_ctc_align_desc* d, const float* emit, const int32_t* n_frames, const int32_t* tokens,
                          const int32_t* tok0, void* workspace, size_t ws_bytes, float* score, int32_t* status, int32_t* state,
                          int32_t* tok_start, int32_t* tok_end, int32_t* tok_peak, float* tok_logp, hipStream_t stream);
constexpr int32_t kCtxMagic = 0x5843334d;
constexpr int kCtxMaxGraphs = 1024, kCtxMaxStates = 65536;
constexpr size_t kCtxMaxBytes = (size_t)64 << 20;
enum { CTX_MAGIC = 0, CTX_G = 1, CTX_V = 2, CTX_WORDS = 3, CTX_HDR_WORDS = 4 };
enum { CTXG_STATES = 0, CTXG_A = 1, CTXG_CLS = 2, CTXG_NEXT = 3, CTXG_DELTA = 4, CTXG_POT = 5, CTXG_WORDS = 8 };
struct CtxGraph {
  const int32_t* cls;
  const int32_t* next;
  const float* delta;
  const float* pot;
  int n_states, A, V;
};
__host__ __device__ inline bool ctx_graph_view(const int32_t* image, long long words, int g, CtxGraph* out) {
  if (image == nullptr || words < CTX_HDR_WORDS || image[CTX_MAGIC] != kCtxMagic) return false;
  const long long G = image[CTX_G], V = image[CTX_V];
  if (G < 0 || G > kCtxMaxGraphs || V < 1 || CTX_HDR_WORDS + G * CTXG_WORDS > words || g < 0 || g >= G) return false;
  const int32_t* h = image + CTX_HDR_WORDS + (long long)g * CTXG_WORDS;
  const long long ns = h[CTXG_STATES], A = h[CTXG_A], first = CTX_HDR_WORDS + G * CTXG_WORDS;
  if (ns < 1 || ns > kCtxMaxStates || A < 1 || A > V + 1 || A > kCtxMaxStates) return false;
  const long long off[4] = {h[CTXG_CLS], h[CTXG_NEXT], h[CTXG_DELTA], h[CTXG_POT]};
  const long long len[4] = {V, ns * A, ns * A, ns};
  for (int i = 0; i < 4; ++i)
    if (off[i] < first || off[i] > words || len[i] > words - off[i]) return false;
  out->cls = image + off[0];
  out->next = image + off[1];
  out->delta = (const float*)(image + off[2]);
  out->pot = (const float*)(image + off[3]);
  out->n_states = (int)ns;
  out->A = (int)A;
  out->V = (int)V;
  return true;
}
int ctc_context_validate(const void* image, size_t bytes, int V);
int ctc_prefix_beam_search_ctx_host(const float* top_logp, const int32_t* top_idx, int T, int k, int beam, int blank,
                                    const void* image, size_t image_bytes, int graph, int32_t* hyp_tokens, int32_t* hyp_len,
                                    float* hyp_score, float* hyp_bonus, int32_t* hyp_state, int32_t* n_hyps);
size_t ctc_beam_ctx_state_size(const m3_ctc_beam_desc* d);
int launch_ctc_beam_ctx_reset(const m3_ctc_beam_desc* d, void* state, size_t bytes, hipStream_t stream,
                              const int32_t* slots = nullptr, int n = 0);
int launch_ctc_beam_ctx_advance(const m3_ctc_beam_desc* d, void* state, size_t bytes, const void* image, size_t image_bytes,
                                const int32_t* graph_of, const float* top_logp, const int32_t* top_idx, int T_chunk,
                                const int32_t* n_frames, hipStream_t stream);
int launch_ctc_beam_ctx_nbest(const m3_ctc_beam_desc* d, const void* state, size_t bytes, const void* image, size_t image_bytes,
                              const int32_t* graph_of, int32_t* hyp_tokens, int32_t* hyp_len, float* hyp_score,
                              float* hyp_bonus, int32_t* n_hyps, hipStream_t stream);
constexpr int32_t kLmMagic = 0x4d4c334d;
constexpr int32_t kLmVersion = 1;
constexpr int kLmMaxOrder = 8, kLmMaxStates = 1 << 26;
constexpr size_t kLmMaxBytes = (size_t)1 << 30;
enum { LM_MAGIC = 0, LM_VERSION = 1, LM_V = 2, LM_ORDER = 3, LM_STATES = 4, LM_ARCS = 5, LM_START = 6, LM_UNK = 7, LM_TABLES = 8,
       LM_WORDS = 17, LM_HDR_WORDS = 20 };
enum { LMT_UNI_LOGP = 0, LMT_UNI_NEXT, LMT_ARC_BEGIN, LMT_ARC_TOK, LMT_ARC_NEXT, LMT_ARC_LOGP, LMT_BO_STATE, LMT_BO_WEIGHT,
       LMT_FINAL, LMT_COUNT };
struct LmView {
  const float* uni_logp;
  const int32_t* uni_next;
  const int32_t* arc_begin;
  const int32_t* arc_tok;
  const int32_t* arc_next;
  const float* arc_logp;
  const int32_t* bo_state;
  const float* bo_weight;
  const float* fin;
  int V, order, n_states, n_arcs, start;
  float unk_logp;
};
__host__ __device__ inline bool lm_view(const int32_t* image, long long words, LmView* out) {
  if (image == nullptr || words < LM_HDR_WORDS || image[LM_MAGIC] != kLmMagic || image[LM_VERSION] != kLmVersion) return false;
  const long long V = image[LM_V], order = image[LM_ORDER], ns = image[LM_STATES], na = image[LM_ARCS], start = image[LM_START];
  if (V < 1 || order < 1 || order > kLmMaxOrder || ns < 1 || ns > kLmMaxStates || na < 0 || start < 0 || start >= ns) return false;
  const long long len[LMT_COUNT] = {V, V, ns + 1, na, na, na, ns, ns, ns};
  for (int i = 0; i < LMT_COUNT; ++i) {
    const long long off = image[LM_TABLES + i];
    if (off < LM_HDR_WORDS || off > words || len[i] > words - off) return false;
  }
  out->uni_logp = (const float*)(image + image[LM_TABLES + LMT_UNI_LOGP]);
  out->uni_next = image + image[LM_TABLES + LMT_UNI_NEXT];
  out->arc_begin = image + image[LM_TABLES + LMT_ARC_BEGIN];
  out->arc_tok = image + image[LM_TABLES + LMT_ARC_TOK];
  out->arc_next = image + image[LM_TABLES + LMT_ARC_NEXT];
  out->arc_logp = (const float*)(image + image[LM_TABLES + LMT_ARC_LOGP]);
  out->bo_state = image + image[LM_TABLES + LMT_BO_STATE];
  out->bo_weight = (const float*)(image + image[LM_TABLES + LMT_BO_WEIGHT]);
  out->fin = (const float*)(image + image[LM_TABLES + LMT_FINAL]);
  out->V = (int)V;
  out->order = (int)order;
  out->n_states = (int)ns;
  out->n_arcs = (int)na;
  out->start = (int)start;
  out->unk_logp = ((const float*)image)[LM_UNK];
  return true;
}
__host__ __device__ inline int lm_in_range(int v, int n) { return (unsigned)v < (unsigned)n ? v : 0; }
__host__ __device__ inline int lm_find(const LmView& m, int lo, int hi, int tok) {
  while (lo < hi) {
    const int mid = (lo + hi) >> 1, t = m.arc_tok[mid];
    if (t == tok) return mid;
    if (t < tok) lo = mid + 1;
    else hi = mid;
  }
  return -1;
}
__host__ __device__ inline void lm_arcs(const LmView& m, int st, int* lo, int* hi) {
  *lo = m.arc_begin[st];
  *hi = m.arc_begin[st + 1];
  if (*lo < 0 || *hi > m.n_arcs || *lo > *hi) *lo = *hi = 0;
}
__host__ __device__ inline double lm_step_root(const LmView& m, double w, int tok, int* next) {
// ... 72 lines not shown
```

Baseline: 155,000 frames/s.

## Precompute router embed-half products for all layers and fold GLU sigmoid into GEMM epilogue

```diff
diff --git a/3m-asr-inference_amd/csrc/conv.hip b/3m-asr-inference_amd/csrc/conv.hip
--- a/3m-asr-inference_amd/csrc/conv.hip
+++ b/3m-asr-inference_amd/csrc/conv.hip
@@ -13,7 +13,7 @@
   int max_chunks = 0;
 };
 
-template <int KT, bool CAUSAL, bool SLOTS = false, bool GLU_IN = false>
+template <int KT, bool CAUSAL, bool SLOTS = false, int GLU_IN = 0>
 __device__ __forceinline__ void dwconv_ln_silu_body(const float* __restrict__ z, const float* __restrict__ w_kc,
                                                     const float* __restrict__ bias, const float* __restrict__ gamma,
                                                     const float* __restrict__ beta, float eps, int T, int D, int K,
@@ -85,7 +85,14 @@
         if (GLU_IN) gg[kk] = ldg4(src + D + c);
         ww[kk] = ldg4(w_kc + (size_t)k * D + c);
       }
-      if (GLU_IN) {
+      if (GLU_IN == 2) {
+        __builtin_amdgcn_sched_barrier(0);
+#pragma unroll
+        for (int kk = 0; kk < KT; ++kk)
+#pragma unroll
+          for (int j = 0; j < 4; ++j) zz[kk][j] = zz[kk][j] * gg[kk][j];
+      }
+      if (GLU_IN == 1) {
         __builtin_amdgcn_sched_barrier(0);
 #pragma unroll
         for (int kk = 0; kk < KT; ++kk)
@@ -140,7 +147,7 @@
   }
 }
 
-template <int KT, bool CAUSAL, bool SLOTS = false, bool GLU_IN = false>
+template <int KT, bool CAUSAL, bool SLOTS = false, int GLU_IN = 0>
 __global__ __launch_bounds__(GLU_IN ? 256 : 1024) void dwconv_ln_silu_kernel(const float* __restrict__ z, const float* __restrict__ w_kc,
                                                               const float* __restrict__ bias,
                                                               const float* __restrict__ gamma,
@@ -156,7 +163,7 @@
   const float *z, *w_kc, *bias, *gamma, *beta; float eps; int T, D, K; float* out; int out_bf16;
   const int32_t *pad_of, *row0, *row_len; int n_rows; DwCausal cs; int ldz;
 };
-template <int KT, bool CAUSAL, bool GLU_IN = false>
+template <int KT, bool CAUSAL, int GLU_IN = 0>
 __global__ __launch_bounds__(GLU_IN ? 256 : 1024) void dwconv_ln_silu_dual_kernel(const DwKernArgs a, const DwKernArgs b) {
   if ((int)blockIdx.x < a.n_rows)
     dwconv_ln_silu_body<KT, CAUSAL, false, GLU_IN>(a.z, a.w_kc, a.bias, a.gamma, a.beta, a.eps, a.T, a.D, a.K, a.out, a.out_bf16, a.pad_of, a.row0,
@@ -168,7 +175,8 @@
 
 static int launch_dwconv_impl(const float* z, const float* w_kc, const float* bias, const float* gamma, const float* beta, float eps,
                               int B, int T, int D, int K, float* out, hipStream_t stream, int out_bf16, const int32_t* pad_of,
-                              const int32_t* row0, const int32_t* row_len, const DwCausal& cs, bool slots = false, int glu_ldz = 0) {
+                              const int32_t* row0, const int32_t* row_len, const DwCausal& cs, bool slots = false, int glu_ldz = 0,
+                              int glu_sig = 0) {
   M3_REQUIRE(glu_ldz == 0 || dwconv_glu_in_supports(D, K, cs.causal != 0 || slots, out_bf16, glu_ldz),
              "dwconv (GLU on load): needs the symmetric fp32 conv, K <= 15, 256 <= channels <= 1024, ldz=%d a multiple of 4 and >= %d", glu_ldz, 2 * D);
   M3_REQUIRE(!slots || (cs.causal && cs.step != nullptr && cs.max_chunks > 0), "dwconv (slot mode): needs the streaming causal form");
@@ -185,8 +193,12 @@
 #define M3_DW_SLOTS(KT_)                                                                                                        \
   hipLaunchKernelGGL((dwconv_ln_silu_kernel<KT_, true, true>), dim3(grid), dim3(threads), 0, stream, z, w_kc, bias, gamma, beta, eps, \
                      T, D, K, out, out_bf16, pad_of, row0, row_len, rows, cs, 0)
-  if (glu_ldz)
-    hipLaunchKernelGGL((dwconv_ln_silu_kernel<15, false, false, true>), dim3(grid), dim3(threads), 0, stream, z, w_kc, bias, gamma, beta, eps, T,
+  M3_REQUIRE(!glu_sig || glu_ldz, "dwconv: sigmoided gate columns belong to the GLU-on-load form");
+  if (glu_ldz && glu_sig)
+    hipLaunchKernelGGL((dwconv_ln_silu_kernel<15, false, false, 2>), dim3(grid), dim3(threads), 0, stream, z, w_kc, bias, gamma, beta, eps, T,
+                       D, K, out, out_bf16, pad_of, row0, row_len, rows, cs, glu_ldz);
+  else if (glu_ldz)
+    hipLaunchKernelGGL((dwconv_ln_silu_kernel<15, false, false, 1>), dim3(grid), dim3(threads), 0, stream, z, w_kc, bias, gamma, beta, eps, T,
                        D, K, out, out_bf16, pad_of, row0, row_len, rows, cs, glu_ldz);
   else if (slots) { if (K <= 15) M3_DW_SLOTS(15); else M3_DW_SLOTS(8); }
   else if (K <= 15) { if (cs.causal) M3_DW_CASE(15, true); else M3_DW_CASE(15, false); }
@@ -213,13 +225,13 @@
   if (a.glu_ldz) {
     M3_REQUIRE(a.causal_left_fill == nullptr, "dwconv (GLU on load): the symmetric conv only");
     return launch_dwconv_impl(a.z, a.w_kc, a.bias, a.gamma, a.beta, a.eps, a.B, a.T, a.D, a.K, a.out, stream, a.out_bf16, a.pad_of, a.row0, a.row_len,
-                              DwCausal{}, false, a.glu_ldz);
+                              DwCausal{}, false, a.glu_ldz, a.glu_sig);
   }
   return launch_dwconv_ln_silu(a.z, a.w_kc, a.bias, a.gamma, a.beta, a.eps, a.B, a.T, a.D, a.K, a.out, stream, a.out_bf16, a.pad_of, a.row0,
                                a.row_len, a.causal_left_fill);
 }
 bool dwconv_dual_fusable(const DwArgs& a, const DwArgs& b) {
-  if ((a.glu_ldz != 0) != (b.glu_ldz != 0)) return false;
+  if ((a.glu_ldz != 0) != (b.glu_ldz != 0) || (a.glu_sig != 0) != (b.glu_sig != 0)) return false;
   if (a.glu_ldz && !(dwconv_glu_in_supports(a.D, a.K, a.causal_left_fill != nullptr, a.out_bf16, a.glu_ldz) &&
                      dwconv_glu_in_supports(b.D, b.K, b.causal_left_fill != nullptr, b.out_bf16, b.glu_ldz)))
     return false;
@@ -240,7 +252,8 @@
   const int threads = (int)align_up(a.D / 4, 64), grid = ka.n_rows + kb.n_rows;
   const bool causal = a.causal_left_fill != nullptr;
 #define M3_DWD_CASE(KT_, C_) hipLaunchKernelGGL((dwconv_ln_silu_dual_kernel<KT_, C_>), dim3(grid), dim3(threads), 0, stream, ka, kb)
-  if (a.glu_ldz) hipLaunchKernelGGL((dwconv_ln_silu_dual_kernel<15, false, true>), dim3(grid), dim3(threads), 0, stream, ka, kb);
+  if (a.glu_ldz && a.glu_sig) hipLaunchKernelGGL((dwconv_ln_silu_dual_kernel<15, false, 2>), dim3(grid), dim3(threads), 0, stream, ka, kb);
+  else if (a.glu_ldz) hipLaunchKernelGGL((dwconv_ln_silu_dual_kernel<15, false, 1>), dim3(grid), dim3(threads), 0, stream, ka, kb);
   else if (a.K <= 15) { if (causal) M3_DWD_CASE(15, true); else M3_DWD_CASE(15, false); }
   else { if (causal) M3_DWD_CASE(8, true); else M3_DWD_CASE(8, false); }
 #undef M3_DWD_CASE
diff --git a/3m-asr-inference_amd/csrc/engine.hip b/3m-asr-inference_amd/csrc/engine.hip
--- a/3m-asr-inference_amd/csrc/engine.hip
+++ b/3m-asr-inference_amd/csrc/engine.hip
@@ -54,6 +54,7 @@
   Conv1Args c1;
   DwArgs dw;
   AttArgs att;
+  std::function<int(hipStream_t)> refresh_prefix;
 };
 
 m3_stage_info stage_info(const char* kernel, int launches, double bytes, double flops, bool per_row = true) {
@@ -103,6 +104,7 @@
     bool packed = false;
     bool xn_skipped = false;
     int fork_first = -1, fork_mid = -1, join_at = -1;
+    int prefix_stage = -1;
     std::shared_ptr<float> pfold;
     std::vector<Stage> stages;
     std::unordered_map<std::string, Buf> buffers;
@@ -134,6 +136,8 @@
   bool fused8_adapt;
   bool glu_defer;
   bool front_pair;
+  bool router_prefix;
+  bool glu_sig_epi;
 };
 const Switches& switches() {
   static const Switches sw = [] {
@@ -148,6 +152,8 @@
     w.fused8_adapt = num("M3_FUSED8_ADAPT", 0) != 0;
     w.glu_defer = num("M3_GLU_DEFER", 1) != 0;
     w.front_pair = num("M3_FRONT_PAIR", 1) != 0;
+    w.router_prefix = num("M3_ROUTER_PREFIX", 1) != 0;
+    w.glu_sig_epi = num("M3_GLU_SIG_EPI", 1) != 0;
     return w;
   }();
   return sw;
@@ -278,6 +284,7 @@
 struct Plan {
   int32_t* lens;
   float *c1, *c2, *x, *emb, *h1, *qkv, *pbuf, *ctx, *glu, *dw, *xn, *rl, *eall;
+  float* rprefix; size_t rprefix_layer;
   void* xb;
   int32_t* moe_fs;
   unsigned char* xq; float* xq_scale;
@@ -305,6 +312,8 @@
   return switches().hfuse && !c.debug_taps && c.weight_dtype == M3_F32 && c.embed_blocks > 0 && c.num_blocks > 0 && S <= 128 && c.fork_embed <= 0 &&
          !use_packed_rows(c, B);
 }
+
+size_t router_prefix_layer_floats(const m3_engine_config& c, int S, const Plan& pl);
 
 Plan make_plan(const m3_engine_config& c, void* base, int B, int T, int ep_capacity = 0) {
   Plan p;
@@ -400,6 +409,8 @@
       p.e_xbpad = cv.take<uint16_t>((size_t)S * D);
     }
   }
+  p.rprefix_layer = router_prefix_layer_floats(c, S, p);
+  p.rprefix = p.rprefix_layer ? cv.take<float>(p.rprefix_layer * (size_t)c.num_blocks) : nullptr;
   p.bytes = cv.off;
   return p;
 }
@@ -490,6 +501,27 @@
   r.fs_dev = sw.fused8_adapt && fused8 && pl.moe_fs != nullptr && !c.debug_taps;
   r.needs_e_all = r.norm_in_expert();
   return r;
+}
+
+GemmParams router_concat_gemm(const m3_engine_config& c, int S, const float* emb, const float* x) {
+  const int world = c.ep_world_size > 0 ? c.ep_world_size : 1;
+  const int D = c.attention_dim, De = c.embed_dim, Etot = c.num_experts * world;
+  GemmParams g;
+  g.ldy = Etot; g.M = S; g.N = Etot;
+  g.mode = GEMM_A_CONCAT2; g.A = emb; g.lda = De; g.K1 = De; g.A2 = x; g.lda2 = D; g.K = De + D;
+  g.ln_on_a2 = 1; g.ld_ln_out = D;
+  return g;
+}
+size_t router_prefix_layer_floats(const m3_engine_config& c, int S, const Plan& pl) {
+  if (!switches().router_prefix || c.weight_dtype != M3_F32 || c.embed_dim < 256 || S > 128 || c.num_blocks < 1 ||
+      c.num_blocks > kRouterPrefixMaxLayers)
+    return 0;
+  if (choose_moe_route(c, S, BlockW(), pl).router != RouterForm::Gemm) return 0;
+  static const float some = 0.f;
+  GemmParams g = router_concat_gemm(c, S, &some, &some);
+  g.W = &some; g.Y = const_cast<float*>(&some); g.ln_gamma = g.ln_beta = &some; g.acc_init = &some;
+  const GemmPlan plan = plan_gemm(g, 0);
+  return plan.launches == 1 ? router_prefix_floats(plan) : 0;
 }
 
 struct StageBuilder {
@@ -687,6 +719,7 @@
   const int32_t *lens, *live_len; int live_rpb;
   const int32_t* pdev;
   const float* eall; int ld_eall;
+  int layer;
   void* xb_out; float* xstats_out;
   void* ws; MoeWorkspace mw;
 };
@@ -718,11 +751,25 @@
       g.A = m.x; g.lda = D; g.W = w.router_x.w; g.bias = w.router_x.b; g.ln_wsum = w.router_x.wsum; g.ln_eps = m.eps; g.K = D;
       g.resid = m.eall; g.ldr = m.ld_eall;
     } else {
-      g.mode = GEMM_A_CONCAT2; g.A = pl.emb; g.lda = De; g.K1 = De; g.A2 = m.x; g.lda2 = D; g.K = De + D;
+      g = router_concat_gemm(sb.eng.cfg, S, pl.emb, m.x);
+      g.Y = m.rl; g.m_dev = m.pdev;
       g.W = w.router.w; g.bias = w.router.b;
-      g.ln_gamma = w.n_ff.g; g.ln_beta = w.n_ff.b; g.ln_eps = m.eps; g.ln_on_a2 = 1; g.ln_out = m.xn; g.ld_ln_out = D;
+      g.ln_gamma = w.n_ff.g; g.ln_beta = w.n_ff.b; g.ln_eps = m.eps; g.ln_out = m.xn;
+      if (pl.rprefix != nullptr) g.acc_init = pl.rprefix + (size_t)m.layer * pl.rprefix_layer;
     }
     add_gemm(sb, m.pfx + "moe_router", g, true);
+    if (g.acc_init != nullptr) {
+      Stage& st = sb.bd.stages.back();
+      st.info.alg_bytes += 4.0 * pl.rprefix_layer - 4.0 * De * (Etot + S);
+      st.info.flops -= 2.0 * S * Etot * De;
+      const GemmPlan plan = st.gemm_plan;
+      float* prefix = pl.rprefix; const int layer = m.layer;
+      st.refresh_prefix = [plan, g, prefix, layer](hipStream_t s) {
+        const float* wt[kRouterPrefixMaxLayers] = {};
+        wt[layer] = g.W;
+        return launch_router_embed_prefix(plan, g, wt, layer, 1, prefix, s);
+      };
+    }
   }
   sb.bd.stages.back().reads_embed = true;
 }
@@ -931,6 +978,8 @@
       const GemmPlan rp = plan_gemm(r, 0);
       if (rp.launches == 1 && rp.kernel == GemmKernel::SkinnyF32 && rp.mt == 1) { g = r; glu_deferred = true; }
     }
+    const bool glu_sig = glu_deferred && switches().glu_sig_epi && (D & 15) == 0;
+    if (glu_sig) g.sig_col0 = D;
     add_gemm(sb, pfx + "conv.pw1_glu", g);
     const float* glu = pl.glu; float* dw = pl.dw;
     const float* dww = w.dw_w; const float* dwb = w.dw_b;
@@ -946,7 +995,7 @@
       DwArgs da;
       da.z = glu; da.w_kc = dww; da.bias = dwb; da.gamma = ng; da.beta = nb; da.eps = 1e-5f; da.B = B; da.T = Tp; da.D = D; da.K = K;
       da.out = dw; da.out_bf16 = a16; da.pad_of = pad_of; da.row0 = row0; da.row_len = lens; da.causal_left_fill = lfill;
-      da.glu_ldz = glu_deferred ? 2 * D : 0;
+      da.glu_ldz = glu_deferred ? 2 * D : 0; da.glu_sig = glu_sig;
       add_stage(sb, pfx + "conv.dw_ln_silu", 1, [da](hipStream_t s) { return launch_dwconv_ln_silu_args(da, s); },
                 stage_info("dwconv_ln_silu_kernel", 1, (double)S * D * ((glu_deferred ? 8 : 4) + (a16 ? 2 : 4)) + (double)K * D * 4, 2.0 * K * D * S));
       sb.bd.stages.back().fuse_kind = FuseKind::Dwconv;
@@ -985,7 +1034,7 @@
     m.gidx = pl.gate_idx + (size_t)layer * S; m.gval = pl.gate_val + (size_t)layer * S;
     m.gv = c.keep_expert_output ? nullptr : m.gval;
     m.lens = lens; m.live_len = live_len; m.live_rpb = live_rpb; m.pdev = pdev;
-    m.eall = pl.eall + (size_t)layer * m.E; m.ld_eall = c.num_blocks * m.E;
+    m.eall = pl.eall + (size_t)layer * m.E; m.ld_eall = c.num_blocks * m.E; m.layer = layer;
     m.xb_out = a16 ? xb : nullptr; m.xstats_out = dma ? xstats : nullptr;
     m.ws = (char*)pl.moe_ws + (c.debug_taps ? (size_t)layer * pl.moe_ws_bytes : 0);
     m.mw = carve_moe_workspace(m.ws, S, m.E, D, F);
@@ -1233,6 +1282,20 @@
     add_gemm(sb, "router_e_all", g, true);
     bd.stages.back().reads_embed = true;
   }
+  if (pl.rprefix != nullptr) {
+    GemmParams g = router_concat_gemm(c, S, pl.emb, pl.x);
+    g.W = e->mblocks[0].router.w; g.Y = pl.rl; g.ln_gamma = e->mblocks[0].n_ff.g; g.ln_beta = e->mblocks[0].n_ff.b; g.acc_init = pl.rprefix;
+    if (bd.packed) g.m_dev = pl.row0 + B;
+    const GemmPlan plan = plan_gemm(g, 0);
+    M3_REQUIRE(plan.launches == 1 && router_prefix_floats(plan) == pl.rprefix_layer, "engine_prepare: router prefix: %s", plan.reason);
+    std::vector<const float*> wt(kRouterPrefixMaxLayers, nullptr);
+    for (int i = 0; i < c.num_blocks; ++i) wt[i] = e->mblocks[i].router.w;
+    float* prefix = pl.rprefix; const int L = c.num_blocks;
+    const double Etot = g.N;
+    add_stage(sb, "router_e_prefix", 1, [plan, g, wt, prefix, L](hipStream_t s) { return launch_router_embed_prefix(plan, g, wt.data(), 0, L, prefix, s); },
+              stage_info("router_embed_prefix_kernel", 1, 4.0 * De * (L * Etot + S) + 4.0 * L * pl.rprefix_layer, 2.0 * S * Etot * De * L));
+    bd.stages.back().reads_embed = true;
+  }
   const int main_start = (int)bd.stages.size();
   build_subsample(sb, "subsample.", e->sub_m, D, pl, pl.x);
   for (int i = 0; i < c.num_blocks; ++i)
@@ -1281,6 +1344,8 @@
     add_stage(sb, "stream.advance", 1, [=](hipStream_t s) { return launch_advance_counter(step, 1, s); },
               stage_info("advance_counter_kernel", 1, 8.0, 0.0, false));
   }
+  for (int i = 0; i < (int)bd.stages.size(); ++i)
+    if (bd.stages[i].name == "router_e_prefix") bd.prefix_stage = i;
   bd.buffers["x"] = Buf{pl.x, (size_t)S * D * 4};
   bd.buffers["dw"] = Buf{pl.dw, (size_t)S * D * 4};
   if (!bd.xn_skipped) bd.buffers["xn"] = Buf{pl.xn, (size_t)S * D * 4};
@@ -1383,13 +1448,22 @@
 }
 int m3_engine_num_kernels(const m3_engine* engine) { return engine ? engine->cur.n_kernels : 0; }
 
+static int run_stage_range(m3_engine* engine, int first_stage, int last_stage, hipStream_t stream, bool whole) {
+  const int ps = engine->cur.prefix_stage;
+  for (int i = first_stage; i < last_stage; ++i) {
+    const Stage& st = engine->cur.stages[i];
+    if (st.refresh_prefix && !whole && !(ps >= first_stage && ps < i))
+      if (int rc = st.refresh_prefix(stream)) return rc;
+    if (int rc = st.run(stream)) return rc;
+  }
+  return 0;
+}
+
 int m3_engine_run(m3_engine* engine, int first_stage, int last_stage, m3_stream stream) {
   M3_REQUIRE(engine && !engine->cur.stages.empty(), "engine_run: engine not prepared");
   M3_REQUIRE(first_stage >= 0 && last_stage <= (int)engine->cur.stages.size() && first_stage <= last_stage,
              "engine_run: bad stage range [%d,%d)", first_stage, last_stage);
-  for (int i = first_stage; i < last_stage; ++i)
-    if (int rc = engine->cur.stages[i].run((hipStream_t)stream)) return rc;
-  return 0;
+  return run_stage_range(engine, first_stage, last_stage, (hipStream_t)stream, false);
 }
 
 int m3_engine_buffer(const m3_engine* engine, const char* name, void** ptr, size_t* bytes) {
@@ -1409,7 +1483,6 @@
     b.graph_exec = nullptr;
   }
   hipGraph_t graph = nullptr;
-  const m3_stream stream_ = (m3_stream)stream;
   const int n_st = (int)b.stages.size();
   const bool fork = b.fork_first >= 0 && b.fork_mid > b.fork_first && b.join_at > b.fork_mid;
   if (fork && e->side == nullptr) {
@@ -1420,17 +1493,17 @@
   M3_CHECK_HIP(hipStreamBeginCapture(stream, hipStreamCaptureModeThreadLocal));
   int rc = 0;
   if (!fork) {
-    rc = m3_engine_run(e, 0, n_st, stream_);
+    rc = run_stage_range(e, 0, n_st, stream, true);
   } else {
     hipError_t he = hipSuccess;
-    rc = m3_engine_run(e, 0, b.fork_first, stream_);
+    rc = run_stage_range(e, 0, b.fork_first, stream, true);
     if (!rc && (he = hipEventRecord(e->ev_fork, stream)) != hipSuccess) rc = -1;
     if (!rc && (he = hipStreamWaitEvent(e->side, e->ev_fork, 0)) != hipSuccess) rc = -1;
-    if (!rc) rc = m3_engine_run(e, b.fork_first, b.fork_mid, (m3_stream)e->side);
-    if (!rc) rc = m3_engine_run(e, b.fork_mid, b.join_at, stream_);
+    if (!rc) rc = run_stage_range(e, b.fork_first, b.fork_mid, e->side, true);
+    if (!rc) rc = run_stage_range(e, b.fork_mid, b.join_at, stream, true);
     if (!rc && (he = hipEventRecord(e->ev_join, e->side)) != hipSuccess) rc = -1;
     if (!rc && (he = hipStreamWaitEvent(stream, e->ev_join, 0)) != hipSuccess) rc = -1;
-    if (!rc) rc = m3_engine_run(e, b.join_at, n_st, stream_);
+    if (!rc) rc = run_stage_range(e, b.join_at, n_st, stream, true);
     if (he != hipSuccess) set_error("%s: forked capture failed: %s", who, hipGetErrorString(he));
   }
   hipError_t ce = hipStreamEndCapture(stream, &graph);
diff --git a/3m-asr-inference_amd/csrc/gemm.hip b/3m-asr-inference_amd/csrc/gemm.hip
--- a/3m-asr-inference_amd/csrc/gemm.hip
+++ b/3m-asr-inference_amd/csrc/gemm.hip
@@ -14,10 +14,12 @@
 
 enum { LN_NONE = GEMM_LN_NONE, LN_EPI = GEMM_LN_EPI, LN_PRO = GEMM_LN_PRO };
 
-template <int MT, bool GLU, int NW, bool CONV, int LN, int NBUF>
+template <int MT, bool GLU, int NW, bool CONV, int LN, int NBUF, bool ACCI = false>
 __device__ __forceinline__ void gemm_f32_body(const GemmParams& p, const int bid) {
   constexpr int NT = GLU ? 2 : 1;
   constexpr int G = gemm_group_steps(MT, NT, NW);
+  constexpr int I0 = ACCI ? G / 2 : 0;
+  static_assert(!ACCI || (MT == 1 && !GLU && !CONV && NBUF == 1 && G % 2 == 0), "acc_init: the one-group 16-row concat form only");
   constexpr int RW = (16 * MT) / NW;
   static_assert(RW >= 1, "more waves than rows");
   __shared__ float red[NW][MT * NT][256];
@@ -28,7 +30,8 @@
   M3_GDIAG(unsigned long long dg[8]; dg[0] = __builtin_amdgcn_s_memtime();)
   asm volatile("" ::"s"(p.A), "s"(p.lda), "s"(p.W), "s"(p.bias), "s"(p.Y), "s"(p.ldy), "s"(p.M), "s"(p.N), "s"(p.K), "s"(p.mode),
                "s"(p.n_tiles), "s"(p.m_tiles), "s"(p.xcd_swizzle), "s"(p.m_dev), "s"(p.resid), "s"(p.ldr), "s"(p.act), "s"(p.alpha),
-               "s"(p.mask_in), "s"(p.mask_out), "s"(p.row_len), "s"(p.rows_per_batch));
+               "s"(p.mask_in), "s"(p.mask_out), "s"(p.row_len), "s"(p.rows_per_batch), "s"(p.sig_col0));
+  if (ACCI) asm volatile("" ::"s"(p.acc_init));
   if (LN == LN_EPI) asm volatile("" ::"s"(p.ln_wsum), "s"(p.ln_wbeta), "s"(p.ln_eps));
   if (LN == LN_PRO) asm volatile("" ::"s"(p.ln_gamma), "s"(p.ln_beta), "s"(p.ln_eps), "s"(p.ln_out), "s"(p.ld_ln_out), "s"(p.ln_on_a2));
   if (!CONV) asm volatile("" ::"s"(p.A2), "s"(p.lda2), "s"(p.K1));
@@ -104,12 +107,12 @@
   f32x4 wbuf[NBUF][G][NT], abuf[NBUF][G][MT];
   auto load_group = [&](int g, int buf) {
 #pragma unroll
-    for (int i = 0; i < G; ++i) {
+    for (int i = I0; i < G; ++i) {
       const int s = min(wave + NW * (G * g + i), nsteps - 1);
       const int k = s << 4;
 #pragma unroll
       for (int t = 0; t < NT; ++t) wbuf[buf][i][t] = ldg4_w(wrow[t] + k);
-      const bool second = !CONV && p.mode == GEMM_A_CONCAT2 && k >= p.K1;
+      const bool second = ACCI || (!CONV && p.mode == GEMM_A_CONCAT2 && k >= p.K1);
       const int off = second ? (k - p.K1) : a_offset(k);
 #pragma unroll
       for (int mt = 0; mt < MT; ++mt) abuf[buf][i][mt] = ldg4((second ? arow2[mt] : arow[mt]) + off);
@@ -118,7 +121,29 @@
 
   const int ngroups = (nsteps + NW * G - 1) / (NW * G);
   M3_GDIAG(dg[1] = __builtin_amdgcn_s_memtime();)
+  f32x4 ln_v[16];
+  auto load_stat_rows = [&](int c) {
+    const int l16 = lane & 15;
+    const int rloc = wave * RW + 4 * c + (lane >> 4);
+    const int m = min(m0 + min(rloc, 16 * MT - 1), p.M - 1);
+    const float* row = (p.ln_on_a2 ? p.A2 : p.A) + (size_t)m * (p.ln_on_a2 ? p.lda2 : p.lda);
+#pragma unroll
+    for (int j = 0; j < 8; ++j) ln_v[j] = ldg4(row + min(4 * (l16 + 16 * j), Kl - 4));
+    if (Kl > 512) {
+#pragma unroll
+      for (int j = 8; j < 16; ++j) ln_v[j] = ldg4(row + min(4 * (l16 + 16 * j), Kl - 4));
+    } else {
+#pragma unroll
+      for (int j = 8; j < 16; ++j) ln_v[j] = f32x4{0.f, 0.f, 0.f, 0.f};
+    }
+  };
+  if (LN == LN_PRO && ACCI) load_stat_rows(0);
   load_group(0, 0);
+  if (ACCI) {
+    const float* pre = p.acc_init + ((size_t)((m_tile * p.n_tiles + n_tile) * NW + wave) * 2) * 256 + 4 * lane;
+    acc[0][0] = ldg4(pre);
+    acc2[0][0] = ldg4(pre + 256);
+  }
   M3_GDIAG(dg[2] = __builtin_amdgcn_s_memtime();)
   const int ep_mt = wave;
   const bool is_ep = wave < MT;
@@ -164,8 +189,6 @@
     ln_out_row[mt] = nullptr;
   }
   if (LN == LN_PRO) {
-    const float* lnA = p.ln_on_a2 ? p.A2 : p.A;
-    const int ldl = p.ln_on_a2 ? p.lda2 : p.lda;
     for (int k = threadIdx.x * 4; k < Kl; k += 256 * NW) {
       *reinterpret_cast<f32x4*>(&ln_g[k]) = ldg4(p.ln_gamma + k);
       *reinterpret_cast<f32x4*>(&ln_b[k]) = ldg4(p.ln_beta + k);
@@ -175,13 +198,12 @@
     for (int c = 0; c < (RW + 3) / 4; ++c) {
       const int rloc = wave * RW + 4 * c + q;
       const bool row_on = (4 * c + q) < RW;
-      const int m = min(m0 + min(rloc, 16 * MT - 1), p.M - 1);
-      const float* row = lnA + (size_t)m * ldl;
       f32x4 v[16];
+      if (!(ACCI && c == 0)) load_stat_rows(c);
 #pragma unroll
       for (int j = 0; j < 16; ++j) {
         const int k = 4 * (l16 + 16 * j);
-        const f32x4 t = ldg4(row + min(k, Kl - 4));
+        const f32x4 t = ln_v[j];
         const bool in = j < nj && k < Kl;
         v[j] = f32x4{in ? t[0] : 0.f, in ? t[1] : 0.f, in ? t[2] : 0.f, in ? t[3] : 0.f};
       }
@@ -218,7 +240,7 @@
 
   auto compute_group = [&](int g, int buf) {
 #pragma unroll
-    for (int i = 0; i < G; ++i) {
+    for (int i = I0; i < G; ++i) {
       const int s = wave + NW * (G * g + i);
       if (s < nsteps) {
         const int k = s << 4;
@@ -335,8 +357,9 @@
           }
           ln_mean_rstd(t1, t2, Kl, p.ln_eps, mean, rstd);
         }
-        p.Y[(size_t)m * p.ldy + ep_n] =
-            gemm_epilogue<GLU, LN == LN_EPI>(y0, y1, bias0, bias1, wsum0, wsum1, wbeta0, wbeta1, mean, rstd, pad, res[r], p);
+        float y = gemm_epilogue<GLU, LN == LN_EPI>(y0, y1, bias0, bias1, wsum0, wsum1, wbeta0, wbeta1, mean, rstd, pad, res[r], p);
+        if (!GLU && p.sig_col0 >= 0 && n0 >= p.sig_col0) y = sigmoidf(y);
+        p.Y[(size_t)m * p.ldy + ep_n] = y;
       }
     }
   }
@@ -351,9 +374,79 @@
            })
 }
 
-template <int MT, bool GLU, int NW, bool CONV, int LN, int NBUF>
+template <int MT, bool GLU, int NW, bool CONV, int LN, int NBUF, bool ACCI = false>
 __global__ __launch_bounds__(64 * NW) void gemm_f32_kernel(const GemmParams p) {
-  gemm_f32_body<MT, GLU, NW, CONV, LN, NBUF>(p, (int)blockIdx.x);
+  gemm_f32_body<MT, GLU, NW, CONV, LN, NBUF, ACCI>(p, (int)blockIdx.x);
+}
+
+struct RouterPrefixArgs {
+  const float* A; int lda; int M, N, K;
+  int n_tiles, m_tiles, xcd_swizzle;
+  const int32_t* m_dev;
+  float* prefix; long layer_floats; int layer0;
+  const float* w[kRouterPrefixMaxLayers];
+};
+template <int NW>
+__global__ __launch_bounds__(64 * NW) void router_embed_prefix_kernel(const RouterPrefixArgs a) {
+  constexpr int H = gemm_group_steps(1, 1, NW) / 2;
+  asm volatile("" ::"s"(a.A), "s"(a.lda), "s"(a.M), "s"(a.N), "s"(a.K), "s"(a.n_tiles), "s"(a.m_tiles), "s"(a.xcd_swizzle), "s"(a.m_dev),
+               "s"(a.prefix), "s"(a.layer_floats), "s"(a.layer0));
+  const int lane = threadIdx.x & 63, wave = threadIdx.x >> 6;
+  const int col = lane & 15, kq = lane >> 4;
+  const int layer = a.layer0 + (int)blockIdx.y;
+  int n_tile, m_tile;
+  {
+    const int id = (int)blockIdx.x;
+    if (a.xcd_swizzle) {
+      const int j = id >> 3;
+      m_tile = j % a.m_tiles;
+      n_tile = (j / a.m_tiles) * 8 + (id & 7);
+    } else {
+      n_tile = id % a.n_tiles;
+      m_tile = id / a.n_tiles;
+    }
+  }
+  const int n0 = n_tile * 16, m0 = m_tile * 16;
+  if (a.m_dev != nullptr && m0 > *a.m_dev) return;
+  const float* arow = a.A + (size_t)min(m0 + col, a.M - 1) * a.lda + 4 * kq;
+  const float* wrow = a.w[layer] + (size_t)min(n0 + col, a.N - 1) * a.K + 4 * kq;
+  f32x4 wb[H], ab[H];
+#pragma unroll
+  for (int i = 0; i < H; ++i) {
+    const int k = (wave + NW * i) << 4;
+    wb[i] = ldg4_w(wrow + k);
+    ab[i] = ldg4(arow + k);
+  }
+  f32x4 acc = f32x4{0.f, 0.f, 0.f, 0.f}, acc2 = f32x4{0.f, 0.f, 0.f, 0.f};
+#pragma unroll
+  for (int i = 0; i < H; ++i)
+#pragma unroll
+    for (int j = 0; j < 4; j += 2) {
+      acc = mfma16(ab[i][j], wb[i][j], acc);
+      acc2 = mfma16(ab[i][j + 1], wb[i][j + 1], acc2);
+    }
+  float* o = a.prefix + (size_t)layer * a.layer_floats + ((size_t)((m_tile * a.n_tiles + n_tile) * NW + wave) * 2) * 256 + 4 * lane;
+  stg4(o, acc);
+  stg4(o + 256, acc2);
+}
+
+size_t router_prefix_floats(const GemmPlan& plan) { return (size_t)plan.m_tiles * plan.n_tiles * plan.nw * 2 * 256; }
+
+int launch_router_embed_prefix(const GemmPlan& plan, const GemmParams& p, const float* const* w, int layer0, int n_layers, float* prefix,
+                               hipStream_t stream) {
+  M3_REQUIRE(plan.launches == 1 && plan.kernel == GemmKernel::SkinnyF32 && p.acc_init != nullptr && (plan.nw == 4 || plan.nw == 8),
+             "router prefix: the consumer's plan does not take an accumulator prefix");
+  M3_REQUIRE(layer0 >= 0 && n_layers > 0 && layer0 + n_layers <= kRouterPrefixMaxLayers && prefix != nullptr, "router prefix: bad layer range");
+  RouterPrefixArgs a;
+  a.A = p.A; a.lda = p.lda; a.M = p.M; a.N = p.N; a.K = p.K;
+  a.n_tiles = plan.n_tiles; a.m_tiles = plan.m_tiles; a.xcd_swizzle = plan.xcd_swizzle;
+  a.m_dev = p.m_dev; a.prefix = prefix; a.layer_floats = (long)router_prefix_floats(plan); a.layer0 = layer0;
+  for (int l = 0; l < kRouterPrefixMaxLayers; ++l) a.w[l] = (l >= layer0 && l < layer0 + n_layers) ? w[l] : nullptr;
+  const dim3 grid(plan.n_tiles * plan.m_tiles, n_layers);
+  if (plan.nw == 8) hipLaunchKernelGGL((router_embed_prefix_kernel<8>), grid, dim3(512), 0, stream, a);
+  else hipLaunchKernelGGL((router_embed_prefix_kernel<4>), grid, dim3(256), 0, stream, a);
+  M3_LAUNCH_CHECK();
+  return 0;
 }
 template <int MT, bool GLU, int NW, int LN>
 __global__ __launch_bounds__(64 * NW) void gemm_f32_dual_kernel(const GemmParams p0, const GemmParams p1, const int n0) {
@@ -392,6 +485,12 @@
   p.n_tiles = plan.n_tiles; p.m_tiles = plan.m_tiles; p.xcd_swizzle = plan.xcd_swizzle;
   dim3 grid(p.n_tiles * p.m_tiles);
   const int mt = plan.mt, nw = plan.nw, ln = plan.ln;
+  if (p.acc_init != nullptr) {
+    if (nw == 8) hipLaunchKernelGGL((gemm_f32_kernel<1, false, 8, false, LN_PRO, 1, true>), grid, dim3(512), 0, stream, p);
+    else hipLaunchKernelGGL((gemm_f32_kernel<1, false, 4, false, LN_PRO, 1, true>), grid, dim3(256), 0, stream, p);
+    M3_LAUNCH_CHECK();
+    return 0;
+  }
 
 #define M3_GEMM_LAUNCH(MT_, GLU_, NW_, CONV_, LN_)                                                              \
   do {                                                                                                          \
diff --git a/3m-asr-inference_amd/csrc/gemm_plan.hip b/3m-asr-inference_amd/csrc/gemm_plan.hip
--- a/3m-asr-inference_amd/csrc/gemm_plan.hip
+++ b/3m-asr-inference_amd/csrc/gemm_plan.hip
@@ -137,7 +137,24 @@
   plan.kernel = GemmKernel::SkinnyF32; plan.label = "gemm_f32_kernel";
   skinny_grid(p, plan, Nout);
   plan.dual_ok = plan.mt == 1 && (plan.nw == 4 || plan.nw == 8) && plan.nbuf == 1 && p.mode == GEMM_A_PLAIN &&
-                 plan.ln != GEMM_LN_PRO && p.m_dev == nullptr;
+                 plan.ln != GEMM_LN_PRO && p.m_dev == nullptr && p.acc_init == nullptr;
+  return true;
+}
+
+static bool extras_ok(const GemmParams& p, GemmPlan& plan) {
+  if (p.sig_col0 >= 0) {
+    M3_PLAN_REQUIRE(plan.kernel == GemmKernel::SkinnyF32 && !plan.glu, "gemm: sig_col0 needs the skinny fp32 kernel with a plain epilogue (M=%d N=%d K=%d)",
+                    p.M, p.N, p.K);
+    M3_PLAN_REQUIRE((p.sig_col0 & 15) == 0, "gemm: sig_col0=%d must be a multiple of 16", p.sig_col0);
+  }
+  if (p.acc_init != nullptr) {
+    M3_PLAN_REQUIRE(plan.kernel == GemmKernel::SkinnyF32 && plan.mt == 1 && !plan.glu && p.mode == GEMM_A_CONCAT2 && (p.K1 & 15) == 0,
+                    "gemm: acc_init needs the skinny fp32 kernel, 16-row tiles, concat operands with K1 %% 16 == 0");
+    M3_PLAN_REQUIRE(plan.ln == GEMM_LN_PRO && p.ln_on_a2 && (plan.nw == 4 || plan.nw == 8) && plan.nbuf == 1 && 2 * p.K1 == p.K &&
+                    p.K == 16 * plan.nw * gemm_group_steps(1, 1, plan.nw),
+                    "gemm: acc_init is built for K1 = K / 2 = %d with the LayerNorm prologue on the A2 half (K1=%d K=%d)",
+                    8 * plan.nw * gemm_group_steps(1, 1, plan.nw), p.K1, p.K);
+  }
   return true;
 }
 
@@ -147,7 +164,7 @@
   plan.label = "";
   plan.glu = p.act == ACT_GLU; plan.conv = p.mode == GEMM_A_CONV3X3S2;
   plan.ln = p.ln_wsum ? GEMM_LN_EPI : (p.ln_gamma ? GEMM_LN_PRO : GEMM_LN_NONE);
-  if (operands_ok(p, p.w_bf16 ? "gemm_bf16w" : "gemm", plan) && choose_form(p, workspace_bytes_available, plan))
+  if (operands_ok(p, p.w_bf16 ? "gemm_bf16w" : "gemm", plan) && choose_form(p, workspace_bytes_available, plan) && extras_ok(p, plan))
     plan.launches = plan.kernel == GemmKernel::SplitKF32 ? 2 : 1;
   return plan;
 }
diff --git a/3m-asr-inference_amd/csrc/kernels.h b/3m-asr-inference_amd/csrc/kernels.h
--- a/3m-asr-inference_amd/csrc/kernels.h
+++ b/3m-asr-inference_amd/csrc/kernels.h
@@ -35,6 +35,8 @@
   const int32_t* m_dev = nullptr;
   const int32_t* y_rows = nullptr;
   const int32_t* conv_len = nullptr;
+  int sig_col0 = -1;
+  const float* acc_init = nullptr;
   int n_tiles = 0, m_tiles = 0, xcd_swizzle = 0;
 };
 enum { GEMM_LN_NONE = 0, GEMM_LN_EPI = 1, GEMM_LN_PRO = 2 };
@@ -56,6 +58,10 @@
 int launch_gemm(const GemmPlan& plan, const GemmParams& p, float* ws, hipStream_t stream);
 bool gemm_dual_fusable(const GemmPlan& a, const GemmPlan& b);
 int launch_gemm_f32_dual(const GemmPlan& pa, const GemmParams& a, const GemmPlan& pb, const GemmParams& b, hipStream_t stream);
+constexpr int kRouterPrefixMaxLayers = 64;
+size_t router_prefix_floats(const GemmPlan& plan);
+int launch_router_embed_prefix(const GemmPlan& plan, const GemmParams& p, const float* const* w, int layer0, int n_layers, float* prefix,
+                               hipStream_t stream);
 constexpr int gemm_group_steps(int MT, int NT, int NW) {
   if (NW == 16) return MT == 1 ? (NT == 1 ? 4 : 2) : (MT == 2 ? 2 : 1);
   if (NW == 8) return MT == 1 ? 8 : (MT == 2 ? (NT == 1 ? 6 : 4) : (NT == 1 ? 3 : 2));
@@ -244,6 +250,7 @@
   int B = 0, T = 0, D = 0, K = 0; float* out = nullptr; int out_bf16 = 0;
   const int32_t *pad_of = nullptr, *row0 = nullptr, *row_len = nullptr; const float* causal_left_fill = nullptr;
   int glu_ldz = 0;
+  int glu_sig = 0;
 };
 int launch_dwconv_ln_silu_args(const DwArgs& a, hipStream_t stream);
 bool dwconv_glu_in_supports(int D, int K, bool causal_or_stream, int out_bf16, int ldz);
```

New measurement: 158,200 frames/s (median of 6 runs). 1.02x the previous value.
